# MartijnAB/guacamole

Measured on AMD Instinct MI355X. Metric: pileup loci/sec at 30x WGS; achieved HBM GB/s vs roofline, higher is better.
Workload: dtype u8; 1 GPU; germline-threshold, synthetic 30x chr20-length shard per GPU (configs[1]); genome_loci=63025519, visited_loci_per_gpu=63025483, reads_per_gpu=12612887, contigs_per_gpu=1, read_len=150, threshold=8, parallelism=loci-sharded x1

## Files before the change

guacamole_amd/csrc/gq_germline_common.h:

```cpp
#pragma once

#include "gq_kernels.h"


__device__ __forceinline__ int64_t xcd_tile(int64_t b, int64_t n) {
  const int64_t q = n >> 3, rem = n & 7;
  const int64_t x = b & 7, j = b >> 3;
  return x * q + (x < rem ? x : rem) + j;
}

struct LdsOut {
  unsigned *lds;
  unsigned long long base[2], cap[2];
  __device__ __forceinline__ unsigned long long reserve(int which, unsigned n) {
    return wave_reserve_lds(lds + which, n);
  }
};
struct GlobalOut {
  Counters *ctr;
  int part;
  unsigned long long base[2], cap[2];
  __device__ __forceinline__ unsigned long long reserve(int which, unsigned n) {
    return wave_reserve(&ctr->part[which][part], n);
  }
};

template <int T, bool ZERO = false, class Out>
__device__ __forceinline__ void germline_decide(const uint32_t *cnt, const Tile &tl, int64_t tile_id, bool wide,
                                                int n_samples, int threshold, int emit_ref, int emit_no_call,
                                                CallRec *__restrict__ recs, ComplexItem *__restrict__ cplx,
                                                Out &out, unsigned &visited, unsigned &amb, unsigned &ties,
                                                const uint32_t *reg = nullptr) {
  constexpr int S = T + 2 * kGuard;
  const int32_t L0 = tl.L0;
  const bool multi_sample = n_samples > 1;
  const int nloci = tl.L1 - L0;
  const int64_t thr1 = (int64_t)threshold + 1;
  const bool narrow = thr1 >= 0 && thr1 <= 1001;
  const uint32_t thr1u = (uint32_t)thr1;
  auto passes = [=](uint32_t count, uint32_t depth) {
    return narrow ? count * 100u >= thr1u * depth : (int64_t)count * 100 >= thr1 * (int64_t)depth;
  };
  constexpr uint64_t kAltSym = ((uint64_t)'<' << 8) | ((uint64_t)'A' << 16) | ((uint64_t)'L' << 24) |
                               ((uint64_t)'T' << 32) | ((uint64_t)'>' << 40);
  for (int i0 = 0; i0 < nloci; i0 += blockDim.x) {
    const int i = i0 + threadIdx.x;
    const bool in = i < nloci;
    uint32_t wac = 0, wtg = 0, wox = 0, wnn = 0, eac = 0, etg = 0;
    if (in) {
      wac = cnt[W_AC * S + kGuard + i];
      wtg = cnt[W_TG * S + kGuard + i];
      wox = cnt[W_OX * S + kGuard + i];
      wnn = cnt[W_NN * S + kGuard + i];
      eac = cnt[W_EAC * S + kGuard + i];
      etg = cnt[W_ETG * S + kGuard + i];
    }
    if (ZERO && i < T) {
      uint32_t *z = const_cast<uint32_t *>(cnt) + kGuard + i;
#pragma unroll
      for (int w = 0; w < W_N; ++w) z[w * S] = 0u;
    }
    uint32_t c[5] = {wac & 0xFFFFu, wac >> 16, wtg & 0xFFFFu, wtg >> 16, wnn >> 16};
    if (reg) {
#pragma unroll
      for (int k = 0; k < 5; ++k) c[k] += in ? reg[k] : 0u;
    }
    const uint32_t cx = (wox & 0xFFFFu) + (wox >> 16);
    const uint32_t depth = c[0] + c[1] + c[2] + c[3] + c[4] + cx;
    const uint32_t mask = (wnn & 0xFu) | (c[0] > (eac & 0xFFFFu) ? 1u : 0u) | (c[1] > (eac >> 16) ? 2u : 0u) |
                          (c[2] > (etg & 0xFFFFu) ? 4u : 0u) | (c[3] > (etg >> 16) ? 8u : 0u);
    const bool live = in && depth > 0;
    const bool ambiguous = (mask & (mask - 1)) != 0;
    const uint32_t low = mask & (0u - mask);
    const uint32_t c_ref = low == 1u ? c[0] : low == 2u ? c[1] : low == 4u ? c[2] : low == 8u ? c[3] : c[4];
    const bool cgn = low == 2u && c[3] > 0 && c[4] > 0;
    const bool to_complex = (wide && in) || (live && (ambiguous || cx > 0 || multi_sample || cgn));
    const bool homref = live && !to_complex && !passes(depth - c_ref, depth);
    const bool ref_pass = c_ref > 0 && passes(c_ref, depth);
    const bool emit_hr = homref && (ref_pass ? emit_ref : emit_no_call);
    const bool general = live && !to_complex && !homref;
    visited += (live && !(wide && in)) ? 1u : 0u;
    amb += (live && ambiguous && !wide) ? 1u : 0u;
    if (__ballot(to_complex || emit_hr || general) == 0) continue;
    CallRec out0, out1;
    unsigned nout = 0;
    const uint8_t ref = mask ? bit_base(mask) : (uint8_t)'N';
    const int32_t pos = L0 + i;
    const uint64_t ord = (uint64_t)(tl.ordinal0 + i);
    auto push = [&](const CallRec &rr) {
      if (nout == 0) out0 = rr;
      else out1 = rr;
      ++nout;
    };
    if (emit_hr) {
      CallRec rr;
      rr.key = ord << 12;
      rr.contig = tl.contig;
      rr.pos = pos;
      rr.sample = 0;
      rr.gt0 = rr.gt1 = ref_pass ? GQ_GT_REF : GQ_GT_NOCALL;
      rr.flags = 0;
      rr.ref_len = 1;
      rr.alt_len = 5;
      rr.allele = (uint64_t)ref | kAltSym;
      push(rr);
    }
    if (general) {
      CallRec rr;
      rr.key = ord << 12;
      rr.contig = tl.contig;
      rr.pos = pos;
      rr.sample = 0;
      rr.gt0 = ref;
      rr.gt1 = 0;
      rr.flags = kCandidate;
      rr.ref_len = (uint16_t)c[4];
      rr.alt_len = 0;
      rr.allele = (uint64_t)c[0] | ((uint64_t)c[1] << 16) | ((uint64_t)c[2] << 32) | ((uint64_t)c[3] << 48);
      push(rr);
      rr.flags = kCandidateSlot;
      push(rr);
    }
    const unsigned long long base = out.reserve(0, nout);
    CallRec *prec = recs + out.base[0];
    if (nout > 0 && base < out.cap[0]) prec[base] = out0;
    if (nout > 1 && base + 1 < out.cap[0]) prec[base + 1] = out1;
    const unsigned long long cb = out.reserve(1, to_complex ? 1u : 0u);
    if (to_complex && cb < out.cap[1])
      cplx[out.base[1] + cb] = ComplexItem{(int32_t)tile_id, L0 + i, wide ? 1 : 0};
  }
}

__global__ void germline_expand(CallRec *__restrict__ recs, Counters *ctr, OutGeom og, int threshold,
                                int emit_ref, int emit_no_call, uint64_t dead_key) {
  const unsigned long long n = ctr->n_rec;
  const int64_t thr1 = (int64_t)threshold + 1;
  auto passes = [=](uint32_t count, uint32_t depth) { return (int64_t)count * 100 >= thr1 * (int64_t)depth; };
  constexpr uint64_t kAltSym = ((uint64_t)'<' << 8) | ((uint64_t)'A' << 16) | ((uint64_t)'L' << 24) |
                               ((uint64_t)'T' << 32) | ((uint64_t)'>' << 40);
  unsigned dead = 0, ties = 0;
  (void)n;
  for (int p = blockIdx.x; p < kParts; p += gridDim.x) {
   const unsigned long long cnt = ctr->part_off[0][p + 1] - ctr->part_off[0][p];
   for (unsigned long long k = threadIdx.x; k < cnt; k += blockDim.x) {
    const unsigned long long slot = og.slot(0, p, k);
    const CallRec cand = recs[slot];
    if (cand.flags != kCandidate) continue;
    constexpr int NC = 6;
    const uint32_t c[NC] = {(uint32_t)(cand.allele & 0xFFFFu), (uint32_t)((cand.allele >> 16) & 0xFFFFu),
                            (uint32_t)((cand.allele >> 32) & 0xFFFFu), (uint32_t)(cand.allele >> 48), cand.ref_len,
                            cand.alt_len};
    const uint32_t depth = c[0] + c[1] + c[2] + c[3] + c[4] + c[5];
    const uint8_t ref = cand.gt0;
    int npres = 0;
#pragma unroll
    for (int cat = 0; cat < NC; ++cat) npres += c[cat] > 0 ? 1 : 0;
    uint64_t sk[NC];
#pragma unroll
    for (int cat = 0; cat < NC; ++cat) {
      scala::SeqHasher hr, ha;
      hr.add_byte(ref);
      if (cat < 5) ha.add_byte(cat_base(cat));
      const uint32_t h = scala::allele_hash(hr.result(), ha.result());
      sk[cat] = npres <= 4 ? (uint64_t)(15u - scala::mutable_bucket(h, 4)) : scala::trie_key(h);
    }
    uint32_t k0 = 0, k1 = 0, k2 = 0;
    int npass = 0;
#pragma unroll
    for (int cat = 0; cat < NC; ++cat) {
      const uint32_t cc = c[cat];
      if (cc == 0 || !passes(cc, depth)) continue;
      ++npass;
      int rank = 0;
#pragma unroll
      for (int o = 0; o < NC; ++o)
        if (o != cat && c[o] > 0 && (sk[o] < sk[cat] || (sk[o] == sk[cat] && o < cat))) ++rank;
      uint32_t key = (cc << 16) | ((uint32_t)(255 - rank) << 8) | (uint32_t)cat;
      if (key > k0) { const uint32_t t = k0; k0 = key; key = t; }
      if (key > k1) { const uint32_t t = k1; k1 = key; key = t; }
      if (key > k2) { k2 = key; }
    }
    const bool tie = npass >= 2 && ((k0 >> 16) == (k1 >> 16) || (npass >= 3 && (k1 >> 16) == (k2 >> 16)));
    if (tie) ++ties;
    const uint8_t fl = tie ? GQ_FLAG_TIE : 0;
    const int t0 = (int)(k0 & 0xFFu), t1 = (int)(k1 & 0xFFu);
    auto is_var = [&](int cat) { return cat == 5 || cat_base(cat) != ref; };
    int nout = 0, aa = 0, ab = 0;
    uint8_t ga0 = 0, ga1 = 0, gb0 = 0, gb1 = 0;
    bool syma = false;
    if (npass == 0) {
      if (emit_no_call) nout = 1, ga0 = ga1 = GQ_GT_NOCALL, syma = true;
    } else if (npass == 1 && !is_var(t0)) {
      if (emit_ref) nout = 1, ga0 = ga1 = GQ_GT_REF, syma = true;
    } else if (npass == 1) {
      nout = 1, ga0 = ga1 = GQ_GT_ALT, aa = t0;
    } else {
      const bool v1 = is_var(t0), v2 = is_var(t1);
      if ((!v1 || !v2) && ((t0 == 5) != (t1 == 5))) {
      } else if (v1 != v2) {
        nout = 1, ga0 = GQ_GT_REF, ga1 = GQ_GT_ALT, aa = v1 ? t0 : t1;
      } else if (v1 && v2) {
        nout = 2, ga0 = gb0 = GQ_GT_ALT, ga1 = gb1 = GQ_GT_OTHERALT, aa = t0, ab = t1;
      }
    }
    auto put = [&](unsigned long long at, bool live, int sub, uint8_t g0, uint8_t g1, int cat, bool sym) {
      const uint64_t key = live ? (cand.key | (uint64_t)sub) : dead_key;
      const uint32_t alt_len = sym ? 5u : cat == 5 ? 0u : 1u;
      const uint64_t allele = sym ? ((uint64_t)ref | kAltSym)
                                  : ((uint64_t)ref | (cat == 5 ? 0ull : (uint64_t)cat_base(cat) << 8));
      const uint32_t w3 = (uint32_t)cand.sample | ((uint32_t)g0 << 8) | ((uint32_t)g1 << 16) |
                          ((uint32_t)(live ? fl : 0) << 24);
      const uint32_t w4 = 1u | (alt_len << 16);
      uint4 *d = reinterpret_cast<uint4 *>(recs + at);
      d[0] = make_uint4((uint32_t)key, (uint32_t)(key >> 32), (uint32_t)cand.contig, (uint32_t)cand.pos);
      d[1] = make_uint4(w3, w4, (uint32_t)allele, (uint32_t)(allele >> 32));
    };
    put(slot, nout > 0, 0, ga0, ga1, aa, syma);
    put(slot + 1, nout > 1, 1, gb0, gb1, ab, false);
    dead += nout > 1 ? 0u : nout > 0 ? 1u : 2u;
   }
  }
  for (int d = 32; d >= 1; d >>= 1) {
    dead += __shfl_xor(dead, d, 64);
    ties += __shfl_xor(ties, d, 64);
  }
  if ((threadIdx.x & 63) == 0) {
    const int sl = (int)((blockIdx.x * (blockDim.x >> 6) + (threadIdx.x >> 6)) & (kSpread - 1));
    if (dead) atomicAdd(&ctr->spread[3][sl], (unsigned long long)dead);
    if (ties) atomicAdd(&ctr->spread[2][sl], (unsigned long long)ties);
  }
}

__device__ __forceinline__ void add_run_counters(Counters *ctr, unsigned visited, unsigned amb, unsigned ties,
                                                 int slot) {
  __shared__ unsigned red[3];
  if (threadIdx.x < 3) red[threadIdx.x] = 0;
  __syncthreads();
  if (visited) atomicAdd(&red[0], visited);
  if (amb) atomicAdd(&red[1], amb);
  if (ties) atomicAdd(&red[2], ties);
  __syncthreads();
  if (threadIdx.x == 0) {
    const int sl = slot & (kSpread - 1);
    if (red[0]) atomicAdd(&ctr->spread[0][sl], (unsigned long long)red[0]);
    if (red[1]) atomicAdd(&ctr->spread[1][sl], (unsigned long long)red[1]);
    if (red[2]) atomicAdd(&ctr->spread[2][sl], (unsigned long long)red[2]);
  }
}

template <int T>
__global__ __launch_bounds__(kBlock) __attribute__((amdgpu_waves_per_eu(4))) void germline_walk(const Tile *__restrict__ tiles, const int32_t *__restrict__ slow,
                                                        DevReads R, int threshold, int emit_ref, int emit_no_call,
                                                        CallRec *__restrict__ recs, ComplexItem *__restrict__ cplx,
                                                        OutGeom og,
                                                        Counters *ctr) {
  constexpr int S = T + 2 * kGuard;
  __shared__ __attribute__((aligned(16))) uint32_t cnt[W_N * S];
  const int64_t n = (int64_t)ctr->n_slow;
  const int part = kPartsCols + (int)((blockIdx.x * (blockDim.x >> 6) + (threadIdx.x >> 6)) & (kPartsWalk - 1));
  GlobalOut out{ctr, part, {og.slot(0, part, 0), og.slot(1, part, 0)}, {og.capB[0], og.capB[1]}};
  unsigned visited = 0, amb = 0, ties = 0;
  for (int64_t q = blockIdx.x; q < n; q += gridDim.x) {
    const int64_t tid_tile = slow[q];
    const Tile tl = tiles[tid_tile];
    const bool wide = (tl.re - tl.rb) >= 65535;
    uint4 *c4 = reinterpret_cast<uint4 *>(cnt);
    for (int i = threadIdx.x; i < W_N * S / 4; i += blockDim.x) c4[i] = make_uint4(0u, 0u, 0u, 0u);
    __syncthreads();
    if (!wide) {
      GermSink<T, 0> sink{cnt, tl.L0, &ctr->err, &ctr->err_pos};
      for (int64_t r = tl.rb + threadIdx.x; r < tl.re; r += blockDim.x) walk_read_lane(R, r, tl.L0, tl.L1, sink);
    }
    __syncthreads();
    germline_decide<T>(cnt, tl, tid_tile, wide, R.n_samples, threshold, emit_ref, emit_no_call, recs, cplx, out,
                       visited, amb, ties);
    __syncthreads();
  }
  add_run_counters(ctr, visited, amb, ties, (int)blockIdx.x);
}
```

guacamole_amd/csrc/gq_host.h:

```cpp
#pragma once
#include <hip/hip_runtime.h>

#include <algorithm>
#include <cstddef>
#include <cstring>
#include <condition_variable>
#include <mutex>
#include <thread>
#include <cstdarg>
#include <cstdio>
#include <string>
#include <utility>
#include <vector>

#include "../../include/gqpileup.h"
#include "gq_kernels.h"

namespace gq {

gq_status set_err(gq_status s, const char *fmt, ...);

#define HIP_TRY(expr)                                                                         \
  do {                                                                                        \
    hipError_t _e = (expr);                                                                   \
// ... 688 lines not shown
    if (len && !keep(m)) len = 0;
    {
      const int64_t q0 = m.qoff + (pr.col0 >> 4);
      const int32_t npc = len ? ((pr.col1 - 1) >> 4) - (pr.col0 >> 4) + 1 : 0;
      int64_t g[kReadPieces];
      piece_grows(R, rr, q0, npc < kReadPieces ? npc : kReadPieces, g);
#pragma unroll
      for (int j = 0; j < kReadPieces; ++j) m.grow[j] = g[j];
    }
    if (len) meta[lane] = m;
    const uint32_t incl = wave_incl_scan(len), ex = incl - len;
    const uint32_t tot = (uint32_t)__builtin_amdgcn_readlane((int)incl, 63);
    for (uint32_t w0 = 0; w0 < tot; w0 += 64) {
      owner[lane] = 0;
      __builtin_amdgcn_wave_barrier();
      __builtin_amdgcn_fence(__ATOMIC_SEQ_CST, "wavefront");
      if (len > 0 && ex > w0 && ex < w0 + 64) owner[ex - w0] = (uint32_t)lane + 1;
      __builtin_amdgcn_wave_barrier();
      __builtin_amdgcn_fence(__ATOMIC_SEQ_CST, "wavefront");
      const uint32_t w = w0 + (uint32_t)lane;
      const unsigned long long run = __ballot(len > 0 && ex <= w0);
      const uint32_t k_at = run ? 64u - (uint32_t)__clzll((long long)run) : 0u;
      const uint32_t k1 = max(wave_incl_max(owner[lane]), k_at);
      const bool au = w < tot;
      const int k = au ? (int)k1 - 1 : 0;
      const uint4 *rec = reinterpret_cast<const uint4 *>(meta + k);
      const uint4 a = rec[0], bq = rec[1], c = rec[2], dq = rec[3], eq = rec[4];
      ReadMeta mm;
      mm.p0 = (int64_t)((uint64_t)a.x | ((uint64_t)a.y << 32));
      mm.s = (int32_t)a.z;
      mm.e = (int32_t)a.w;
      mm.info = bq.x;
      mm.mq = bq.y;
      mm.col0 = (int32_t)bq.z;
      mm.evin = bq.w;
      mm.ev01 = eq.z;
      mm.ev23 = eq.w;
      mm.md_off = (int64_t)((uint64_t)c.x | ((uint64_t)c.y << 32));
      mm.qoff = (int64_t)((uint64_t)c.z | ((uint64_t)c.w << 32));
      const int64_t g0 = (int64_t)((uint64_t)dq.x | ((uint64_t)dq.y << 32));
      const int64_t g1 = (int64_t)((uint64_t)dq.z | ((uint64_t)dq.w << 32));
      const int64_t g2 = (int64_t)((uint64_t)eq.x | ((uint64_t)eq.y << 32));
      const uint32_t kex = (uint32_t)__shfl((int)ex, k, 64);
      const int32_t col = mm.col0 + (int32_t)(w - kex);
      const int32_t col1 = (mm.e + 7) >> 3;
      bool act = au && col < col1;
      const int32_t pj = (col >> 4) - (mm.col0 >> 4);
      const int64_t slot = mm.qoff + (col >> 4);
      int64_t grow = pj == 0 ? g0 : pj == 1 ? g1 : pj == 2 ? g2 : -2;
      if (act && grow == -2) grow = piece_grow(R, 64 * b + k, slot);
      act = act && grow >= 0;
      const int64_t pa = mm.p0 + 8 * (int64_t)col;
      const bool fast = src != nullptr && act && (mm.info & kColEligible) && pa >= 0 && pa + 8 <= R.seq_cap;
      const uint64_t pre = src != nullptr && R.seq_cap >= 8 && !(dbg & 1)
                               ? *reinterpret_cast<const gq_u64u *>(src + (fast ? pa : 0))
                               : 0ull;
      decltype(fetch((int64_t)0, mm, (int32_t)0, 0ull, false)) raw{};
      if (act && !(dbg & 1)) raw = fetch(64 * b + k, mm, col, pre, fast);
      emit(act && !(dbg & 2), raw, 64 * b + k, mm, col, grow, slot);
    }
    __builtin_amdgcn_wave_barrier();
    __builtin_amdgcn_fence(__ATOMIC_SEQ_CST, "wavefront");
  }
}

__device__ __forceinline__ unsigned wave_reserve_lds(unsigned *ctr, unsigned n) {
  const uint64_t b1 = __ballot(n & 1u), b2 = __ballot(n & 2u);
  if ((b1 | b2) == 0) return 0;
  const uint64_t lt = __builtin_amdgcn_read_exec() & ((1ull << (threadIdx.x & 63)) - 1ull);
  const unsigned pre = (unsigned)__popcll(b1 & lt) + 2u * (unsigned)__popcll(b2 & lt);
  const unsigned total = (unsigned)__popcll(b1) + 2u * (unsigned)__popcll(b2);
  unsigned base = 0;
  if (lt == 0) base = atomicAdd(ctr, total);
  base = (unsigned)__builtin_amdgcn_readfirstlane((int)base);
  return base + pre;
}

struct Plan {
  int64_t n_tiles = 0;
  int64_t n_loci = 0;
  int T = 0;
  bool aligned = false;
  std::vector<int32_t> rc, rwin;
  std::vector<int64_t> rs, re, rt, rtask;
  struct Win {
    int32_t contig;
    int64_t r0, r1;
  };
  std::vector<Win> wins;
  const int64_t *d_rs = nullptr, *d_re = nullptr, *d_wroff = nullptr;
  const int32_t *d_rwin = nullptr, *d_wcontig = nullptr;
  int64_t range_of_tile(int64_t t) const {
    return (int64_t)(std::upper_bound(rt.begin(), rt.end(), t) - rt.begin()) - 1;
  }
  int64_t tiles_of(int64_t r) const {
    const int64_t s = rs[(size_t)r], e = re[(size_t)r];
    return aligned ? (e - 1) / T - s / T + 1 : (e - s + T - 1) / T;
  }
};

struct AmbItem {
  int32_t tile, pos;
  int64_t item;
};

}

namespace gq {
struct DevBuf {
  void *p = nullptr;
  size_t n = 0;
  hipError_t ensure(size_t bytes) {
    if (bytes <= n) return hipSuccess;
    if (p) (void)hipFree(p);
    p = nullptr;
    n = 0;
    size_t want = std::max(bytes, (size_t)256);
    hipError_t e = hipMalloc(&p, want);
    if (e == hipSuccess) n = want;
    return e;
  }
  void release() {
    if (p) (void)hipFree(p);
    p = nullptr;
    n = 0;
  }
};
}

struct gq_ctx {
  int device = 0;
  hipStream_t stream = nullptr;
  hipEvent_t ev[6] = {};
  hipEvent_t dev_ev[4] = {};
  hipStream_t side = nullptr;
  hipEvent_t side_ev[4] = {};
  gq_timings timings{};
  int germ_tile = gq::kGermT;
  int n_cu = 0;
  int proj_wg_per_cu = 0;
  int dir_wg_per_cu = 0;
  int som_wg_per_cu = 0;
  int somd_wg_per_cu = 0;
  gq::DevBuf mtab;
  int mtab_key = -1;
  int call_wg_per_cu = 0;
  gq::DevBuf ranges, tiles, recs, recs_sorted, keys, keys_sorted, idx, idx_sorted, cplx, pool, counters, sort_tmp, image, tiles2, srecs;
  gq::DevBuf c_depth, c_pos, c_base, c_indel, c_ref, c_rb, c_amb, slow, deep_tiles;
  gq::DevBuf amb, amb_ref, heap_off, heap_reads;
  gq::DevBuf win_meta, win_grp;
  gq::DevBuf deep_list, deep_scratch;
  gq::DevBuf cands;
  gq::DevBuf win_bound;
  gq::DevBuf bkt;
  void *stage[2] = {nullptr, nullptr};
  hipEvent_t stage_done[2] = {};
  bool stage_used[2] = {false, false};
  std::mutex stage_m;
  std::condition_variable stage_cv;
  bool stage_ready = false;
  hipError_t stage_err = hipSuccess;
  std::thread prep;
  hipError_t wait_stage() {
    std::unique_lock<std::mutex> lk(stage_m);
    stage_cv.wait(lk, [this] { return stage_ready; });
    return stage_err;
  }
  void *pin = nullptr;
  size_t pin_n = 0;
  hipError_t pinned(size_t bytes) {
    if (bytes <= pin_n) return hipSuccess;
    if (pin) (void)hipHostFree(pin);
    pin = nullptr;
    pin_n = 0;
    const size_t want = std::max(bytes, (size_t)65536);
    hipError_t e = hipHostMalloc(&pin, want, hipHostMallocDefault);
    if (e == hipSuccess) pin_n = want;
    return e;
  }
};

struct DerivedPool {
  std::vector<std::pair<void *, size_t>> live, spare;
  hipError_t get(void **p, size_t bytes) {
    bytes = std::max(bytes, (size_t)16);
    size_t best = spare.size();
    for (size_t i = 0; i < spare.size(); ++i)
      if (spare[i].second >= bytes && spare[i].second <= bytes + bytes / 4 + 65536 &&
          (best == spare.size() || spare[i].second < spare[best].second))
        best = i;
    if (best < spare.size()) {
      *p = spare[best].first;
      live.push_back(spare[best]);
      spare.erase(spare.begin() + (long)best);
      return hipSuccess;
    }
    *p = nullptr;
    const hipError_t e = hipMalloc(p, bytes);
    if (e == hipSuccess) live.emplace_back(*p, bytes);
    return e;
  }
  void put(void *p) {
    for (size_t i = 0; i < live.size(); ++i)
      if (live[i].first == p) {
        spare.push_back(live[i]);
        live.erase(live.begin() + (long)i);
        return;
      }
  }
  void release_all() {
    spare.insert(spare.end(), live.begin(), live.end());
    live.clear();
  }
  void free_all() {
    for (auto &x : live) (void)hipFree(x.first);
    for (auto &x : spare) (void)hipFree(x.first);
    live.clear();
    spare.clear();
  }
};

struct gq_dev_reads {
  gq_ctx *ctx = nullptr;
  gq::DevReads d{};
  std::vector<int64_t> contig_read_begin;
  std::vector<void *> owned;
  mutable DerivedPool dp;
  int64_t seq_bytes = 0;
  int64_t proj_bytes = 0, pev_count = 0, proj_reads = 0;
  int64_t n_slices = 0;
  int64_t n_rows = 0;
  float h2d_ms = 0, derive_ms = 0;
  bool columns = false;
  bool ev_bases = false;
  bool projected = false;
  void *nnb = nullptr;
  float proj_ms = 0;
  float fill_ms = 0;
  float proj_dev_ms = 0;
  float derive_dev_ms = 0;
  hipEvent_t tev[6] = {};
  unsigned pending = 0;
  unsigned long long *nok = nullptr;
  mutable void *mproj = nullptr;
  mutable int mproj_mapq = -1;
  mutable void *mnb = nullptr;
};

namespace gq {
struct H2DStager {
  static constexpr size_t kChunk = size_t(64) << 20;
  gq_ctx *c;
  hipStream_t stream;
  void **buf = nullptr;
  hipEvent_t *done = nullptr;
  bool *used = nullptr;
  int slot = 0;
  unsigned threads = 1;
  explicit H2DStager(gq_ctx *ctx) : c(ctx), stream(ctx->stream) {
    const unsigned hw = std::max(1u, std::thread::hardware_concurrency());
    threads = std::min(16u, hw);
  }
  ~H2DStager() {
    for (int i = 0; done && i < 2; ++i)
      if (used[i]) (void)hipEventSynchronize(done[i]);
  }
  hipError_t init() {
    const hipError_t e = c->wait_stage();
    if (e != hipSuccess) return e;
    buf = c->stage;
    done = c->stage_done;
    used = c->stage_used;
    return hipSuccess;
  }
  template <class F>
  void fill(uint8_t *out, size_t o, size_t k, const F &src_range) const {
    const unsigned t = (unsigned)std::min<size_t>(threads, std::max<size_t>(1, k >> 22));
    if (t <= 1) {
      src_range(out, o, k);
      return;
    }
    std::vector<std::thread> th;
    const size_t per = (k + t - 1) / t;
    for (unsigned i = 0; i < t; ++i) {
      const size_t a = (size_t)i * per;
      if (a >= k) break;
      th.emplace_back([&, a] { src_range(out + a, o + a, std::min(per, k - a)); });
    }
    for (auto &x : th) x.join();
  }
  template <class F, class G>
  hipError_t copy_from(void *dst, size_t bytes, const F &src_range, const G &landed) {
    for (size_t o = 0; o < bytes; o += kChunk) {
      const size_t k = std::min(kChunk, bytes - o);
      if (used[slot]) {
        hipError_t e = hipEventSynchronize(done[slot]);
        if (e != hipSuccess) return e;
      }
      fill((uint8_t *)buf[slot], o, k, src_range);
      hipError_t e = hipMemcpyAsync((char *)dst + o, buf[slot], k, hipMemcpyHostToDevice, stream);
      if (e == hipSuccess) e = hipEventRecord(done[slot], stream);
      if (e != hipSuccess) return e;
      used[slot] = true;
      slot ^= 1;
      e = landed(o + k);
      if (e != hipSuccess) return e;
    }
    return hipSuccess;
  }
  template <class F>
  hipError_t copy_from(void *dst, size_t bytes, const F &src_range) {
    return copy_from(dst, bytes, src_range, [](size_t) { return hipSuccess; });
  }
  hipError_t copy(void *dst, const void *src, size_t bytes) {
    return copy_from(dst, bytes, [src](uint8_t *out, size_t o, size_t k) { memcpy(out, (const uint8_t *)src + o, k); });
  }
};

gq_status derive_shape(gq_ctx *c, gq_dev_reads *d, int64_t md_len);
gq_status ensure_columns(gq_ctx *c, const gq_dev_reads *d);
gq_status ensure_ev_bases(gq_ctx *c, const gq_dev_reads *d);
gq_status ensure_projection(gq_ctx *c, const gq_dev_reads *d);
hipError_t warm_pileup(hipStream_t s);
hipError_t warm_somatic(hipStream_t s);
hipError_t warm_heapref(hipStream_t s);
hipError_t warm_bamdev(hipStream_t s);

gq_status plan(gq_ctx *c, const gq_dev_reads *rd, const gq_loci *loci, int T, Plan &pl, DevBuf &tiles,
               int stage_cap = 0, int meta_cap = 0, int ev_cap = 0, bool aligned = false);
gq_status check_device_error(gq_ctx *c, const Counters &h);
gq_status heap_ref_bases(gq_ctx *c, const Plan &pl, const DevBuf &tiles_buf,
                         const std::vector<const gq_dev_reads *> &sets, const std::vector<AmbItem> &items,
                         uint8_t *out_ref);

gq_status reads_overlap(gq_ctx *c, const gq_dev_reads *set, int32_t contig,
                        const std::vector<std::pair<int64_t, int64_t>> &ranges, std::vector<char> &out);
}
```

guacamole_amd/csrc/gq_pileup.hip:

```cpp
#include <hip/hip_runtime.h>
#include <hipcub/hipcub.hpp>

#include <algorithm>
#include <chrono>
#include <cstdarg>
#include <cstdlib>
#include <cstdio>
#include <cstring>
#include <string>
#include <thread>
#include <vector>

#include "../../include/gqpileup.h"
#include "gq_host.h"
#include "gq_alleles.h"

using namespace gq;

namespace {
constexpr int kScanT = 256, kScanV = 16, kScanTile = kScanT * kScanV;

__device__ __forceinline__ void scan_load16(const uint32_t *__restrict__ in, int64_t n, int64_t i0, uint32_t (&v)[kScanV]) {
  if (i0 + kScanV <= n) {
    const uint4 *p = reinterpret_cast<const uint4 *>(in + i0);
// ... 1309 lines not shown
      if (((valid4 >> j) & 1u) && i + j >= 0 && i + j < T) elem_i(i + j, K_SNV, (uint8_t)(w >> (8 * j)), 0, false, fl);
  }
  __device__ __forceinline__ void event_i(int i, uint8_t b, uint8_t m, uint8_t) {
    const int bc = base_cat(b);
    if (bc < 4) atomicAdd(&cnt[(K2_EVA + bc) * T + i], 1u);
    const uint32_t bit = std_bit(m);
    if (bit) atomicOr(&cnt[K2_MASK * T + i], bit);
  }
  __device__ __forceinline__ void elem_i(int i, int kind, uint8_t base, uint8_t mdb, bool ev, uint8_t fl) {
    int c;
    switch (kind) {
      case K_SNV: c = base_cat(base); break;
      case K_INS: c = K2_INS; break;
      case K_DEL: c = K2_DEL; break;
      case K_MID: c = K2_MID; break;
      default: c = K2_CLIP; break;
    }
    atomicAdd(&cnt[c * T + i], 1u);
    if (!(fl & 1)) atomicAdd(&cnt[K2_POS * T + i], 1u);
    const uint32_t b = std_bit(mdb);
    if (kind == K_SNV && !ev) return;
    if (kind == K_SNV && ev) {
      const int bc = base_cat(base);
      if (bc < 4) atomicAdd(&cnt[(K2_EVA + bc) * T + i], 1u);
    }
    if (b) atomicOr(&cnt[K2_MASK * T + i], b);
  }
  __device__ __forceinline__ void clip_run(int i0, int i1, uint8_t fl) {
    for (int i = i0; i < i1; ++i) elem_i(i, K_CLIP, 0, (uint8_t)'N', false, fl);
  }
  __device__ __forceinline__ void error(int code, int64_t where) { raise_error(err, (int64_t *)err_pos, code, where); }
};

template <int T>
__global__ __launch_bounds__(kBlock) void counts_tile(const Tile *__restrict__ tiles, DevReads R,
                                                      int32_t *__restrict__ depth, int32_t *__restrict__ pos_depth,
                                                      int32_t *__restrict__ base_counts,
                                                      int32_t *__restrict__ indel_counts,
                                                      int32_t *__restrict__ ref_depth, uint8_t *__restrict__ ref_base,
                                                      uint8_t *__restrict__ ambiguous, Counters *ctr) {
  __shared__ uint32_t cnt[K2_NCAT * T];
  const Tile tl = tiles[blockIdx.x];
  const int32_t L0 = tl.L0, L1 = tl.L1;
  for (int i = threadIdx.x; i < K2_NCAT * T; i += blockDim.x) cnt[i] = 0u;
  __syncthreads();
  CountSink<T> sink{cnt, L0, &ctr->err, &ctr->err_pos};
  for (int64_t r = tl.rb + threadIdx.x; r < tl.re; r += blockDim.x) walk_read_lane(R, r, L0, L1, sink);
  __syncthreads();
  for (int i = threadIdx.x; i < L1 - L0; i += blockDim.x) {
    const int64_t o = tl.ordinal0 + i;
    uint32_t dsum = 0;
    for (int k = 0; k <= K2_CLIP; ++k) dsum += cnt[k * T + i];
    uint32_t mask = cnt[K2_MASK * T + i];
    for (int k = 0; k < 4; ++k)
      if (cnt[k * T + i] > cnt[(K2_EVA + k) * T + i]) mask |= 1u << k;
    const uint8_t rb = mask ? bit_base(mask) : (uint8_t)'N';
    depth[o] = (int32_t)dsum;
    pos_depth[o] = (int32_t)cnt[K2_POS * T + i];
    const int out_order[6] = {K2_A, K2_C, K2_G, K2_T, K2_N, K2_O};
    for (int k = 0; k < 6; ++k) base_counts[o * 6 + k] = (int32_t)cnt[out_order[k] * T + i];
    for (int k = 0; k < 4; ++k) indel_counts[o * 4 + k] = (int32_t)cnt[(K2_INS + k) * T + i];
    ref_depth[o] = (int32_t)cnt[base_cat(rb) * T + i];
    ref_base[o] = rb;
    ambiguous[o] = __popc(mask) > 1 ? 1 : 0;
  }
}

struct VafAmb {
  int32_t depth, base[6];
};
template <int T>
__global__ __launch_bounds__(kBlock) void vaf_tile(const Tile *__restrict__ tiles, DevReads R, int bins,
                                                   int min_depth, int min_vaf, unsigned long long *__restrict__ hist,
                                                   AmbItem *__restrict__ amb, VafAmb *__restrict__ amb_cnt,
                                                   unsigned long long amb_cap, Counters *ctr) {
  __shared__ uint32_t cnt[K2_NCAT * T];
  __shared__ uint32_t h[101];
  const Tile tl = tiles[blockIdx.x];
  const int32_t L0 = tl.L0, L1 = tl.L1;
  for (int i = threadIdx.x; i < K2_NCAT * T; i += blockDim.x) cnt[i] = 0u;
  for (int i = threadIdx.x; i < 101; i += blockDim.x) h[i] = 0u;
  __syncthreads();
  CountSink<T> sink{cnt, L0, &ctr->err, &ctr->err_pos};
  for (int64_t r = tl.rb + threadIdx.x; r < tl.re; r += blockDim.x) walk_read_lane(R, r, L0, L1, sink);
  __syncthreads();
  const int bin_size = 100 / bins;
  unsigned visited = 0, variant = 0;
  for (int i = threadIdx.x; i < L1 - L0; i += blockDim.x) {
    uint32_t dsum = 0;
    for (int k = 0; k <= K2_CLIP; ++k) dsum += cnt[k * T + i];
    if (dsum == 0) continue;
    ++visited;
    uint32_t mask = cnt[K2_MASK * T + i];
    for (int k = 0; k < 4; ++k)
      if (cnt[k * T + i] > cnt[(K2_EVA + k) * T + i]) mask |= 1u << k;
    if (__popc(mask) > 1) {
      const unsigned long long k = atomicAdd(&ctr->n_amb, 1ull);
      if (k < amb_cap) {
        amb[k] = AmbItem{(int32_t)blockIdx.x, L0 + i, (int64_t)k};
        VafAmb v;
        v.depth = (int32_t)dsum;
        const int out_order[6] = {K2_A, K2_C, K2_G, K2_T, K2_N, K2_O};
        for (int q = 0; q < 6; ++q) v.base[q] = (int32_t)cnt[out_order[q] * T + i];
        amb_cnt[k] = v;
      }
      continue;
    }
    const uint8_t rb = mask ? bit_base(mask) : (uint8_t)'N';
    const uint32_t ref = cnt[base_cat(rb) * T + i];
    if (ref == dsum) continue;
    const float vaf = (float)(int32_t)(dsum - ref) / (float)(int32_t)dsum;
    if (!((int32_t)dsum >= min_depth) || !((double)vaf >= (double)min_vaf / 100.0)) continue;
    ++variant;
    const int pct = (int)(vaf * 100.0f);
    atomicAdd(&h[pct - pct % bin_size], 1u);
  }
  __syncthreads();
  unsigned long long *hh = hist + (size_t)(blockIdx.x & 63) * 101;
  for (int i = threadIdx.x; i < 101; i += blockDim.x)
    if (h[i]) atomicAdd(&hh[i], (unsigned long long)h[i]);
  for (int d = 32; d >= 1; d >>= 1) {
    visited += __shfl_xor(visited, d, 64);
    variant += __shfl_xor(variant, d, 64);
  }
  if ((threadIdx.x & 63) == 0) {
    if (visited) atomicAdd(&ctr->spread[0][blockIdx.x & (kSpread - 1)], (unsigned long long)visited);
    if (variant) atomicAdd(&ctr->spread[1][blockIdx.x & (kSpread - 1)], (unsigned long long)variant);
  }
}

struct CallsLayout {
  size_t contig, pos, ref_off, alt_off, ref_len, alt_len, sample, gt0, gt1, flags, pool, bytes;
};
__host__ __device__ inline CallsLayout calls_layout(int64_t n, int64_t dev_pool_used) {
  auto al = [](size_t x) { return (x + 63) & ~(size_t)63; };
  const size_t N = (size_t)n;
  CallsLayout L;
  L.contig = 64;
  L.pos = al(L.contig + 4 * N);
  L.ref_off = al(L.pos + 8 * N);
  L.alt_off = al(L.ref_off + 8 * N);
  L.ref_len = al(L.alt_off + 8 * N);
  L.alt_len = al(L.ref_len + 4 * N);
  L.sample = al(L.alt_len + 4 * N);
  L.gt0 = al(L.sample + N);
  L.gt1 = al(L.gt0 + N);
  L.flags = al(L.gt1 + N);
  L.pool = al(L.flags + N);
  L.bytes = al(L.pool + 8 * N + (size_t)dev_pool_used + 1);
  return L;
}

__global__ __launch_bounds__(1024) void part_scan(Counters *ctr, int which, OutGeom og) {
  constexpr int PER = kParts / 1024;
  __shared__ unsigned long long s[1024];
  __shared__ unsigned long long mx;
  const int t = threadIdx.x;
  unsigned long long v[PER], sum = 0, m = 0;
#pragma unroll
  for (int j = 0; j < PER; ++j) {
    const unsigned long long x = ctr->part[which][t * PER + j];
    const unsigned long long cap = og.cap(which, t * PER + j);
    m = x > cap && x - cap > m ? x - cap : m;
    v[j] = x < cap ? x : cap;
    sum += v[j];
  }
  if (t == 0) mx = 0;
  s[t] = sum;
  __syncthreads();
  if (m) atomicMax(&mx, m);
  for (int d = 1; d < 1024; d <<= 1) {
    const unsigned long long y = t >= d ? s[t - d] : 0ull;
    __syncthreads();
    s[t] += y;
    __syncthreads();
  }
  unsigned long long o = s[t] - sum;
#pragma unroll
  for (int j = 0; j < PER; ++j) {
    ctr->part_off[which][t * PER + j] = o;
    o += v[j];
  }
  if (t == 1023) {
    ctr->part_off[which][kParts] = s[t];
    if (which == 0) ctr->n_rec = s[t];
    else ctr->n_complex = s[t];
    ctr->part_max[which] = mx;
  }
}

__global__ void gather_keys(const CallRec *__restrict__ recs, const Counters *__restrict__ ctr, OutGeom og,
                            int64_t n, uint64_t *__restrict__ keys,
                            int32_t *__restrict__ slot) {
  const int64_t k = (int64_t)blockIdx.x * blockDim.x + threadIdx.x;
  if (k >= n) return;
  const unsigned long long src = part_slot(ctr->part_off[0], (unsigned long long)k, og, 0);
  keys[k] = recs[src].key;
  slot[k] = (int32_t)src;
}

constexpr int kFinBlocks = 1024;
constexpr int kImgBlocks = 512;
__global__ __launch_bounds__(kBlock) void bucket_count(const CallRec *__restrict__ recs, Counters *__restrict__ ctr,
                                                        OutGeom og, uint64_t dead_key, int bshift, int64_t nbk,
                                                        uint64_t *__restrict__ keys, int32_t *__restrict__ slot,
                                                        int64_t *__restrict__ bkt, uint32_t *__restrict__ cnt) {
  const int64_t n_all = (int64_t)ctr->n_rec;
  for (int64_t k = (int64_t)blockIdx.x * blockDim.x + threadIdx.x; k < n_all; k += (int64_t)gridDim.x * blockDim.x) {
    const unsigned long long src = part_slot(ctr->part_off[0], (unsigned long long)k, og, 0);
    const uint64_t key = recs[src].key;
    keys[k] = key;
    slot[k] = (int32_t)src;
    int64_t b = key == dead_key ? -1 : (int64_t)(key >> (12 + bshift));
    if (b >= nbk) {
      if (atomicCAS(&ctr->err, 0, 1 ) == 0) {
        const CallRec r = recs[src];
        ctr->err_pos = (long long)src;
        ctr->prof[0] = key;
        ctr->prof[1] = ((unsigned long long)(uint32_t)r.contig << 32) | (uint32_t)r.pos;
        ctr->prof[2] = ((unsigned long long)r.flags << 24) | ((unsigned long long)r.gt1 << 16) | ((unsigned long long)r.gt0 << 8) | r.sample;
        ctr->prof[3] = (unsigned long long)k;
        ctr->prof[4] = ctr->n_rec;
      }
      b = -1;
    }
    bkt[k] = b;
    if (b >= 0) atomicAdd(&cnt[b], 1u);
  }
}

__global__ void bucket_scatter(const Counters *__restrict__ ctr, const int64_t *__restrict__ bkt,
                               const uint32_t *__restrict__ off, uint32_t *__restrict__ fill,
                               int32_t *__restrict__ members) {
  const int64_t n_all = (int64_t)ctr->n_rec;
  for (int64_t k = (int64_t)blockIdx.x * blockDim.x + threadIdx.x; k < n_all; k += (int64_t)gridDim.x * blockDim.x) {
    const int64_t b = bkt[k];
    if (b >= 0) members[off[b] + atomicAdd(&fill[b], 1u)] = (int32_t)k;
  }
}

__global__ void bucket_rank(int64_t nbk, const uint32_t *__restrict__ off, const int32_t *__restrict__ members,
                            const uint64_t *__restrict__ keys, const int32_t *__restrict__ slot,
                            const int64_t *__restrict__ bkt, int32_t *__restrict__ order) {
  const int64_t n = off[nbk];
  for (int64_t p = (int64_t)blockIdx.x * blockDim.x + threadIdx.x; p < n; p += (int64_t)gridDim.x * blockDim.x) {
    const int32_t k = members[p];
    const int64_t b = bkt[k];
    const uint32_t lo = off[b], hi = off[b + 1];
    const uint64_t key = keys[k];
    uint32_t rank = 0;
    for (uint32_t q = lo; q < hi; ++q) rank += keys[members[q]] < key ? 1u : 0u;
    order[lo + rank] = slot[k];
  }
}

__global__ void zero_u32(uint32_t *__restrict__ v, int64_t n) {
  for (int64_t i = (int64_t)blockIdx.x * blockDim.x + threadIdx.x; i < n; i += (int64_t)gridDim.x * blockDim.x) v[i] = 0u;
}

__global__ void iota_i32(int32_t *__restrict__ v, int64_t n) {
  const int64_t i = (int64_t)blockIdx.x * blockDim.x + threadIdx.x;
  if (i < n) v[i] = (int32_t)i;
}

__device__ __forceinline__ void img_chunk(int64_t n, int64_t &a, int64_t &b) {
  const int64_t per = (n + kImgBlocks - 1) / kImgBlocks;
  a = min(n, (int64_t)blockIdx.x * per);
  b = min(n, a + per);
}
__device__ __forceinline__ uint32_t rec_len(const CallRec &r) { return (uint32_t)r.ref_len + (uint32_t)r.alt_len; }

__global__ __launch_bounds__(kBlock) void img_sums(const CallRec *__restrict__ recs, const int32_t *__restrict__ order,
                                                    const uint32_t *__restrict__ off, int64_t nbk,
                                                    int64_t *__restrict__ bsum) {
  __shared__ unsigned long long red;
  if (threadIdx.x == 0) red = 0;
  __syncthreads();
  int64_t a, b;
  img_chunk((int64_t)off[nbk], a, b);
  unsigned long long s = 0;
  for (int64_t k = a + threadIdx.x; k < b; k += blockDim.x) s += rec_len(recs[order[k]]);
  for (int d = 32; d >= 1; d >>= 1) s += __shfl_xor(s, d, 64);
  if ((threadIdx.x & 63) == 0 && s) atomicAdd(&red, s);
  __syncthreads();
  if (threadIdx.x == 0) bsum[blockIdx.x] = (int64_t)red;
}

__global__ __launch_bounds__(kImgBlocks) void img_scan(int64_t *__restrict__ bsum) {
  __shared__ int64_t s[kImgBlocks];
  const int t = threadIdx.x;
  const int64_t v = bsum[t];
  s[t] = v;
  __syncthreads();
  for (int d = 1; d < kImgBlocks; d <<= 1) {
    const int64_t y = t >= d ? s[t - d] : 0;
    __syncthreads();
    s[t] += y;
    __syncthreads();
  }
  bsum[t] = s[t] - v;
  if (t == kImgBlocks - 1) bsum[kImgBlocks] = s[t];
}

__global__ __launch_bounds__(kBlock) void calls_image(const CallRec *__restrict__ recs, const int32_t *__restrict__ order,
                                                       const uint32_t *__restrict__ off, int64_t nbk,
                                                       const int64_t *__restrict__ bsum, const uint8_t *__restrict__ dpool,
                                                       Counters *__restrict__ ctr, uint8_t *__restrict__ img) {
  __shared__ uint32_t wsum[kBlock / 64];
  const int64_t n = (int64_t)off[nbk];
  const CallsLayout L = calls_layout(n, 0);
  int64_t a, b;
  img_chunk(n, a, b);
  int64_t prefix = bsum[blockIdx.x];
  const int lane = threadIdx.x & 63, wv = threadIdx.x >> 6;
  for (int64_t base = a; base < b; base += blockDim.x) {
    const int64_t k = base + threadIdx.x;
    CallRec r{};
    if (k < b) r = recs[order[k]];
    const uint32_t tot = k < b ? rec_len(r) : 0u;
    const uint32_t inc = wave_incl_scan(tot);
    if (lane == 63) wsum[wv] = inc;
    __syncthreads();
    uint32_t before = 0, all = 0;
#pragma unroll
    for (int w = 0; w < kBlock / 64; ++w) {
      before += w < wv ? wsum[w] : 0u;
      all += wsum[w];
    }
    __syncthreads();
    if (k < b) {
      const int64_t o = prefix + before + inc - tot;
      reinterpret_cast<int32_t *>(img + L.contig)[k] = r.contig;
      reinterpret_cast<int64_t *>(img + L.pos)[k] = r.pos;
      reinterpret_cast<int64_t *>(img + L.ref_off)[k] = o;
      reinterpret_cast<int64_t *>(img + L.alt_off)[k] = o + r.ref_len;
      reinterpret_cast<int32_t *>(img + L.ref_len)[k] = r.ref_len;
      reinterpret_cast<int32_t *>(img + L.alt_len)[k] = r.alt_len;
      img[L.sample + k] = r.sample;
      img[L.gt0 + k] = r.gt0;
      img[L.gt1 + k] = r.gt1;
      img[L.flags + k] = r.flags;
      uint8_t *dst = img + L.pool + o;
      if (tot <= 8) {
        for (uint32_t i = 0; i < tot; ++i) dst[i] = (uint8_t)(r.allele >> (8 * i));
      } else {
        for (uint32_t i = 0; i < tot; ++i) dst[i] = dpool[r.allele + i];
      }
    }
    prefix += all;
  }
  if (blockIdx.x == 0 && threadIdx.x == 0) {
    const int64_t pool_len = bsum[kImgBlocks];
    reinterpret_cast<int64_t *>(img)[0] = pool_len;
    reinterpret_cast<int64_t *>(img)[1] = n;
    ctr->n_out = (unsigned long long)n;
    ctr->out_pool = (unsigned long long)pool_len;
  }
}

}

namespace {
__global__ void warm_k() {}
}
hipError_t gq::warm_pileup(hipStream_t s) {
  hipLaunchKernelGGL(warm_k, dim3(1), dim3(64), 0, s);
  return hipGetLastError();
}

extern "C" {

const char *gq_version(void) { return "guacamole-amd gqpileup 0.1 (gfx950)"; }
const char *gq_last_error(void) { return g_err.c_str(); }

gq_status gq_open(int device, gq_ctx **out) {
  if (!out) return set_err(GQ_E_ARG, "gq_open: null out");
  int n = 0;
  HIP_TRY(hipGetDeviceCount(&n));
  if (device < 0 || device >= n) return set_err(GQ_E_ARG, "gq_open: device %d out of range (%d devices)", device, n);
  HIP_TRY(hipSetDevice(device));
  gq_ctx *c = new gq_ctx();
  c->device = device;
  HIP_TRY(hipStreamCreateWithFlags(&c->stream, hipStreamNonBlocking));
  HIP_TRY(hipStreamCreateWithFlags(&c->side, hipStreamNonBlocking));
  for (auto &e : c->ev) HIP_TRY(hipEventCreate(&e));
  for (auto &e : c->dev_ev) HIP_TRY(hipEventCreate(&e));
  for (auto &e : c->side_ev) HIP_TRY(hipEventCreateWithFlags(&e, hipEventDisableTiming));
  c->prep = std::thread([c] {
    hipError_t e = hipSetDevice(c->device);
    for (int i = 0; i < 2 && e == hipSuccess; ++i) {
      e = hipHostMalloc(&c->stage[i], H2DStager::kChunk, hipHostMallocDefault);
      if (e == hipSuccess) e = hipEventCreateWithFlags(&c->stage_done[i], hipEventDisableTiming);
    }
    {
      std::lock_guard<std::mutex> lk(c->stage_m);
      c->stage_err = e;
      c->stage_ready = true;
    }
    c->stage_cv.notify_all();
    if (e == hipSuccess) e = gq::warm_pileup(c->stream);
    if (e == hipSuccess) e = gq::warm_somatic(c->stream);
    if (e == hipSuccess) e = gq::warm_heapref(c->stream);
    if (e == hipSuccess) e = gq::warm_bamdev(c->stream);
    (void)e;
  });
  *out = c;
  return GQ_OK;
}


void gq_close(gq_ctx *c) {
  if (!c) return;
  if (c->prep.joinable()) c->prep.join();
  (void)hipSetDevice(c->device);
  (void)hipStreamSynchronize(c->stream);
  for (int i = 0; i < 2; ++i) {
    if (c->stage_done[i]) (void)hipEventDestroy(c->stage_done[i]);
    if (c->stage[i]) (void)hipHostFree(c->stage[i]);
  }
  for (DevBuf *b : {&c->ranges, &c->tiles, &c->recs, &c->recs_sorted, &c->keys, &c->keys_sorted, &c->idx,
                    &c->idx_sorted, &c->cplx, &c->pool, &c->counters, &c->sort_tmp, &c->image, &c->tiles2, &c->srecs, &c->c_depth, &c->c_pos,
                    &c->c_base, &c->c_indel, &c->c_ref, &c->c_rb, &c->c_amb, &c->slow, &c->amb, &c->amb_ref,
                    &c->heap_off, &c->heap_reads, &c->win_meta, &c->win_grp, &c->bkt})
    b->release();
  for (auto &e : c->ev) (void)hipEventDestroy(e);
  for (auto &e : c->dev_ev) (void)hipEventDestroy(e);
  for (auto &e : c->side_ev) (void)hipEventDestroy(e);
  if (c->side) {
    (void)hipStreamSynchronize(c->side);
    (void)hipStreamDestroy(c->side);
  }
  if (c->pin) (void)hipHostFree(c->pin);
  (void)hipStreamDestroy(c->stream);
  delete c;
}

gq_status gq_get_timings(const gq_ctx *c, gq_timings *out) {
  if (!c || !out) return set_err(GQ_E_ARG, "gq_get_timings: null argument");
  *out = c->timings;
  return GQ_OK;
}

gq_status gq_set_tile(gq_ctx *c, int32_t t) {
  if (!c) return set_err(GQ_E_ARG, "null ctx");
  if (t == 0) t = kGermT;
  if (t != 512) return set_err(GQ_E_ARG, "tile must be 512 (the germline column kernel's geometry)");
  c->germ_tile = t;
  return GQ_OK;
}

static gq_status validate_reads(const gq_reads *h) {
  if (!h) return set_err(GQ_E_ARG, "null read set");
  if (h->n_reads < 0 || h->n_contigs <= 0) return set_err(GQ_E_ARG, "bad read-set sizes");
  if (h->n_samples < 1 || h->n_samples > 8) return set_err(GQ_E_ARG, "n_samples must be in [1, 8]");
  return GQ_OK;
}

static gq_status settle_stats(gq_dev_reads *d) {
  if (d->pending & 1) {
    HIP_TRY(hipEventSynchronize(d->tev[1]));
    (void)hipEventElapsedTime(&d->derive_dev_ms, d->tev[0], d->tev[1]);
  }
  if (d->pending & 2) {
    HIP_TRY(hipEventSynchronize(d->tev[5]));
    (void)hipEventElapsedTime(&d->fill_ms, d->tev[3], d->tev[4]);
    (void)hipEventElapsedTime(&d->proj_dev_ms, d->tev[2], d->tev[5]);
    std::vector<unsigned long long> hk(kOkSpread);
    HIP_TRY(hipMemcpy(hk.data(), d->nok, sizeof(unsigned long long) * kOkSpread, hipMemcpyDeviceToHost));
    d->proj_reads = 0;
    for (unsigned long long x : hk) d->proj_reads += (int64_t)x;
    d->dp.put(d->nok);
    d->nok = nullptr;
  }
  d->pending = 0;
  return GQ_OK;
}

static gq_status derive_shape_impl(gq_ctx *c, gq_dev_reads *d, int64_t md_len, bool lazy = false) {
  for (hipEvent_t &e : d->tev)
    if (!e) HIP_TRY(hipEventCreate(&e));
  HIP_TRY(hipEventRecord(d->tev[0], c->stream));
  {
    const auto &b = d->contig_read_begin;
    bool ok = !b.empty() && b.front() == 0 && b.back() == d->d.n_reads;
    for (size_t i = 1; i < b.size() && ok; ++i) ok = b[i] >= b[i - 1];
    if (!ok) return set_err(GQ_E_UNSORTED, "contig_read_begin must run from 0 to n_reads, non-decreasing");
  }
  void *p = nullptr;
  HIP_TRY(d->dp.get(&p, sizeof(int16_t) * (size_t)std::max<int64_t>(d->d.n_reads, 1)));
  d->d.lead = (const int16_t *)p;
  d->d.ev_rb = nullptr;
  d->ev_bases = false;
  int unordered = 0;
  const int nc = d->d.n_contigs;
  std::vector<int32_t> last((size_t)nc, 0);
  if (d->d.n_reads > 0) {
    void *flag = nullptr;
    HIP_TRY(d->dp.get(&flag, sizeof(int)));
    HIP_TRY(hipMemsetAsync(flag, 0, sizeof(int), c->stream));
    const unsigned nb = (unsigned)((d->d.n_reads + kBlock - 1) / kBlock);
    hipLaunchKernelGGL(read_prep, dim3(nb), dim3(kBlock), 0, c->stream, d->d, (int *)flag, (int16_t *)p);
    HIP_TRY(hipGetLastError());
    int bad = 0;
    HIP_TRY(hipMemcpyAsync(&bad, flag, sizeof(int), hipMemcpyDeviceToHost, c->stream));
    const auto &crb = d->contig_read_begin;
    for (int k = 0; k < nc; ++k)
      if (crb[(size_t)k + 1] > crb[(size_t)k])
        HIP_TRY(hipMemcpyAsync(&last[(size_t)k], d->d.pmax_end + (crb[(size_t)k + 1] - 1), sizeof(int32_t),
                               hipMemcpyDeviceToHost, c->stream));
    HIP_TRY(hipStreamSynchronize(c->stream));
    if (bad & 1)
      return set_err(GQ_E_UNSORTED, "Regions must be sorted by start locus: reads are not sorted by (contig, start), "
                                    "or pmax_end is not the running maximum of end within each contig");
    if (bad & 2)
      return set_err(GQ_E_ARG, "read set: an offset or length lies outside its pool, or a sample slot >= n_samples");
    unordered = (bad & 4) ? 1 : 0;
  }
  {
    std::vector<int64_t> qoff((size_t)nc + 1, 0);
    for (int k = 0; k < nc; ++k) {
      const int64_t col1 = ((int64_t)std::max(last[(size_t)k], 0) + 7) >> 3;
      qoff[(size_t)k + 1] = qoff[(size_t)k] + 4 * ((col1 + 63) >> 6);
    }
    void *qo = nullptr;
    HIP_TRY(d->dp.get(&qo, sizeof(int64_t) * ((size_t)nc + 1)));
    HIP_TRY(hipMemcpyAsync(qo, qoff.data(), sizeof(int64_t) * ((size_t)nc + 1), hipMemcpyHostToDevice, c->stream));
    d->d.qoff = (const int64_t *)qo;
    d->n_slices = qoff[(size_t)nc];
    const int64_t n_blk = qoff[(size_t)nc] / 4;
    void *bi = nullptr;
    HIP_TRY(d->dp.get(&bi, sizeof(int64_t) * 2 * (size_t)std::max<int64_t>(n_blk, 1)));
    int64_t *brb = (int64_t *)bi, *brs = brb + std::max<int64_t>(n_blk, 1);
    if (n_blk > 0) {
      hipLaunchKernelGGL(block_index, dim3((unsigned)((n_blk + kBlock - 1) / kBlock)), dim3(kBlock), 0, c->stream, d->d,
                         n_blk, brb, brs);
      HIP_TRY(hipGetLastError());
    }
    d->d.blk_rb = brb;
    d->d.blk_rs = brs;
  }
  HIP_TRY(hipEventRecord(d->tev[1], c->stream));
  d->d.pool_ordered = unordered ? 0 : 1;
  if (lazy) {
    d->pending |= 1;
    return GQ_OK;
  }
  HIP_TRY(hipStreamSynchronize(c->stream));
  (void)hipEventElapsedTime(&d->derive_dev_ms, d->tev[0], d->tev[1]);
  return GQ_OK;
}


gq_status gq_reads_upload(gq_ctx *c, const gq_reads *h, gq_dev_reads **out) {
  if (!c || !out) return set_err(GQ_E_ARG, "gq_reads_upload: null argument");
  gq_status st = validate_reads(h);
  if (st) return st;
  HIP_TRY(hipSetDevice(c->device));
  gq_dev_reads *d = new gq_dev_reads();
  d->ctx = c;
  const int64_t n = h->n_reads;
  const auto t0 = std::chrono::steady_clock::now();
  H2DStager stager(c);
  {
    hipError_t e = stager.init();
    if (e != hipSuccess) {
      delete d;
      return set_err(GQ_E_HIP, "upload: pinned staging: %s", hipGetErrorString(e));
    }
  }
  auto up_from = [&](size_t bytes, void **dst, size_t pad, const auto &src_range) -> hipError_t {
    *dst = nullptr;
    hipError_t e = hipMalloc(dst, std::max(bytes + pad, (size_t)16));
    if (e != hipSuccess) return e;
    d->owned.push_back(*dst);
    if (bytes) e = stager.copy_from(*dst, bytes, src_range);
    if (e == hipSuccess && pad) e = hipMemsetAsync((char *)*dst + bytes, 0, pad, c->stream);
    return e;
  };
  auto up = [&](const void *src, size_t bytes, void **dst, size_t pad) -> hipError_t {
    if (bytes >= (size_t(1) << 20) || (!src && bytes))
      return up_from(bytes, dst, pad, [src](uint8_t *out, size_t o, size_t k) {
        if (src) memcpy(out, (const uint8_t *)src + o, k);
        else memset(out, 0, k);
      });
    *dst = nullptr;
    hipError_t e = hipMalloc(dst, std::max(bytes + pad, (size_t)16));
    if (e != hipSuccess) return e;
    d->owned.push_back(*dst);
    if (bytes) e = hipMemcpyAsync(*dst, src, bytes, hipMemcpyHostToDevice, c->stream);
    if (e == hipSuccess && pad) e = hipMemsetAsync((char *)*dst + bytes, 0, pad, c->stream);
    return e;
  };
  void *p;
#define UP_CHECK(field, T, expr)                                                \
  do {                                                                          \
    hipError_t _e = (expr);                                                     \
    if (_e != hipSuccess) {                                                     \
      gq_reads_free(d);                                                         \
      return set_err(GQ_E_HIP, "upload %s: %s", #field, hipGetErrorString(_e)); \
    }                                                                           \
    d->d.field = (const T *)p;                                                  \
  } while (0)
#define UP(field, count, T) UP_CHECK(field, T, up(h->field, (size_t)(count) * sizeof(T), &p, pad_##field))
  enum : size_t { pad_contig_read_begin = 0, pad_start = 0, pad_end = 0, pad_pmax_end = 0, pad_mapq = 0, pad_flags = 0,
                  pad_sample = 0, pad_seq_off = 0, pad_seq_len = 0, pad_cigar_off = 0, pad_n_cigar = 0, pad_md_off = 0,
                  pad_n_md = 0, pad_n_mismatch = 0, pad_seq = kSeqPad, pad_qual = kSeqPad, pad_cigar = 0,
                  pad_md_ev = 0 };
  const gq_reads *h0 = h;
  gq_reads hh = *h;
  std::vector<int64_t> off2;
  bool ordered = true;
  for (int64_t r = 1; r < n && ordered; ++r) ordered = h->seq_off[r] >= h->seq_off[r - 1] + h->seq_len[r - 1];
  if (!ordered) {
    off2.resize((size_t)n);
    int64_t o = 0;
    for (int64_t r = 0; r < n; ++r) {
      off2[(size_t)r] = o;
      o += h->seq_len[r];
    }
    hh.seq_off = off2.data();
    hh.seq_bytes = o;
  }
  auto gather = [&](const uint8_t *src) {
    return [&, src](uint8_t *out, size_t o, size_t k) {
      if (!src) {
        memset(out, 0, k);
        return;
      }
      int64_t r = (int64_t)(std::upper_bound(off2.begin(), off2.end(), (int64_t)o) - off2.begin()) - 1;
      size_t done = 0;
      while (done < k) {
        const size_t a = o + done - (size_t)off2[(size_t)r];
        const size_t m = std::min((size_t)h0->seq_len[r] - a, k - done);
        memcpy(out + done, src + h0->seq_off[r] + a, m);
        done += m;
        ++r;
      }
    };
  };
  h = &hh;
  UP(contig_read_begin, h->n_contigs + 1, int64_t);
  UP(start, n, int32_t);
  UP(end, n, int32_t);
  UP(pmax_end, n, int32_t);
  UP(mapq, n, uint8_t);
  UP(flags, n, uint8_t);
  UP(sample, n, uint8_t);
  UP(seq_off, n, int64_t);
  UP(seq_len, n, int32_t);
  UP(cigar_off, n, int64_t);
  UP(n_cigar, n, int32_t);
  UP(md_off, n, int64_t);
  UP(n_md, n, int32_t);
  UP(n_mismatch, n, uint16_t);
  if (ordered) {
    UP(seq, h->seq_bytes, uint8_t);
    UP(qual, h->seq_bytes, uint8_t);
  } else {
    UP_CHECK(seq, uint8_t, up_from((size_t)h->seq_bytes, &p, pad_seq, gather(h0->seq)));
    UP_CHECK(qual, uint8_t, up_from((size_t)h->seq_bytes, &p, pad_qual, gather(h0->qual)));
  }
  UP(cigar, h->cigar_len, uint32_t);
  UP(md_ev, h->md_len, uint32_t);
#undef UP
#undef UP_CHECK
  d->d.n_reads = n;
  d->d.seq_bytes = h->seq_bytes;
  d->d.seq_cap = h->seq_bytes + kSeqPad;
  d->d.cigar_len = h->cigar_len;
  d->d.md_len = h->md_len;
  d->d.n_contigs = h->n_contigs;
  d->d.n_samples = h->n_samples;
  if (h->sample_hash && h->n_samples > 0) {
    void *sh = nullptr;
    if (hipMalloc(&sh, sizeof(uint32_t) * (size_t)h->n_samples) != hipSuccess ||
        hipMemcpy(sh, h->sample_hash, sizeof(uint32_t) * (size_t)h->n_samples, hipMemcpyHostToDevice) != hipSuccess) {
      if (sh) (void)hipFree(sh);
      gq_reads_free(d);
      return set_err(GQ_E_HIP, "gq_reads_upload: sample hashes");
    }
    d->owned.push_back(sh);
    d->d.sample_hash = (const uint32_t *)sh;
  }
  d->contig_read_begin.assign(h->contig_read_begin, h->contig_read_begin + h->n_contigs + 1);
  d->seq_bytes = h->seq_bytes;
  if (hipStreamSynchronize(c->stream) != hipSuccess) {
    gq_reads_free(d);
    return set_err(GQ_E_HIP, "gq_reads_upload: copies");
  }
  const auto t1 = std::chrono::steady_clock::now();
  d->h2d_ms = std::chrono::duration<float, std::milli>(t1 - t0).count();
  gq_status st2 = derive_shape_impl(c, d, h->md_len);
  d->derive_ms = std::chrono::duration<float, std::milli>(std::chrono::steady_clock::now() - t1).count();
  if (st2) {
    gq_reads_free(d);
    return st2;
  }
  *out = d;
  return GQ_OK;
}

gq_status gq_reads_wrap_device(gq_ctx *c, const gq_reads *h, gq_dev_reads **out) {
  if (!c || !out) return set_err(GQ_E_ARG, "gq_reads_wrap_device: null argument");
  gq_status st = validate_reads(h);
  if (st) return st;
  gq_dev_reads *d = new gq_dev_reads();
  d->ctx = c;
  d->d.n_reads = h->n_reads;
  d->d.seq_bytes = h->seq_bytes;
  d->d.seq_cap = h->seq_bytes;
  d->d.cigar_len = h->cigar_len;
  d->d.md_len = h->md_len;
  d->d.n_contigs = h->n_contigs;
  d->d.n_samples = h->n_samples;
  d->d.contig_read_begin = h->contig_read_begin;
  d->d.start = h->start;
  d->d.end = h->end;
  d->d.pmax_end = h->pmax_end;
  d->d.mapq = h->mapq;
  d->d.flags = h->flags;
  d->d.sample = h->sample;
  d->d.seq_off = h->seq_off;
  d->d.seq_len = h->seq_len;
  d->d.cigar_off = h->cigar_off;
  d->d.n_cigar = h->n_cigar;
  d->d.md_off = h->md_off;
  d->d.n_md = h->n_md;
  d->d.n_mismatch = h->n_mismatch;
  d->d.seq = h->seq;
  d->d.qual = h->qual;
  d->d.cigar = h->cigar;
  d->d.md_ev = h->md_ev;
  d->d.sample_hash = h->sample_hash;
  d->contig_read_begin.resize((size_t)h->n_contigs + 1);
  hipError_t e = hipMemcpy(d->contig_read_begin.data(), h->contig_read_begin,
                           sizeof(int64_t) * ((size_t)h->n_contigs + 1), hipMemcpyDeviceToHost);
  if (e != hipSuccess) {
    delete d;
    return set_err(GQ_E_HIP, "wrap: contig_read_begin D2H: %s", hipGetErrorString(e));
  }
  d->seq_bytes = h->seq_bytes;
  const auto t1 = std::chrono::steady_clock::now();
  gq_status st2 = derive_shape_impl(c, d, h->md_len);
  d->derive_ms = std::chrono::duration<float, std::milli>(std::chrono::steady_clock::now() - t1).count();
  if (st2) {
    gq_reads_free(d);
    return st2;
  }
  *out = d;
  return GQ_OK;
}

gq_status gq_reads_rederive(gq_ctx *c, gq_dev_reads *d) {
  if (!c || !d) return set_err(GQ_E_ARG, "gq_reads_rederive: null argument");
  if (d->ctx != c) return set_err(GQ_E_ARG, "gq_reads_rederive: the read set belongs to another context");
  HIP_TRY(hipSetDevice(c->device));
  HIP_TRY(hipStreamSynchronize(c->stream));
  HIP_TRY(hipStreamSynchronize(c->side));
  d->nok = nullptr;
  d->pending = 0;
  d->dp.release_all();
  DevReads &R = d->d;
  R.lead = nullptr;
  R.ev_rb = R.clean = nullptr;
  R.pool_ordered = 0;
  R.cdesc = nullptr;
  R.cev = nullptr;
  R.caux_off = R.qoff = R.srow = R.pev_off = R.sra = R.soff = R.blk_rb = R.blk_rs = nullptr;
  R.prec = nullptr;
  R.proj = R.pbad = nullptr;
  R.pev = nullptr;
  R.prow = nullptr;
  d->projected = false;
  d->columns = false;
  d->ev_bases = false;
  d->nnb = d->mproj = d->mnb = nullptr;
  d->mproj_mapq = -1;
  d->proj_bytes = d->pev_count = d->proj_reads = d->n_rows = d->n_slices = 0;
  d->proj_ms = d->fill_ms = d->proj_dev_ms = 0;
  const auto t1 = std::chrono::steady_clock::now();
  const gq_status st = derive_shape_impl(c, d, R.md_len, true);
  d->derive_ms = std::chrono::duration<float, std::milli>(std::chrono::steady_clock::now() - t1).count();
  return st;
}

gq_status gq_reads_get_info(const gq_dev_reads *dc, gq_reads_info *out) {
  if (!dc || !out) return set_err(GQ_E_ARG, "gq_reads_get_info: null argument");
  gq_dev_reads *d = const_cast<gq_dev_reads *>(dc);
  if (d->pending) {
    HIP_TRY(hipSetDevice(d->ctx->device));
    const gq_status s0 = settle_stats(d);
    if (s0) return s0;
  }
  out->n_reads = d->d.n_reads;
  out->seq_bytes = d->seq_bytes;
  out->proj_bytes = d->proj_bytes;
  out->pev_count = d->pev_count;
  out->n_rows = d->n_rows;
  out->proj_reads = d->proj_reads;
  out->h2d_ms = d->h2d_ms;
  out->derive_ms = d->derive_ms;
  out->cigar_len = d->d.cigar_len;
  out->md_len = d->d.md_len;
  out->n_contigs = d->d.n_contigs;
  out->n_samples = d->d.n_samples;
  out->proj_ms = d->proj_ms;
  out->projected = d->projected ? 1 : 0;
  out->fill_ms = d->fill_ms;
  out->proj_dev_ms = d->proj_dev_ms;
  out->derive_dev_ms = d->derive_dev_ms;
  return GQ_OK;
}

void gq_reads_free(gq_dev_reads *d) {
  if (!d) return;
  if (d->ctx) (void)hipSetDevice(d->ctx->device);
  for (hipEvent_t e : d->tev)
    if (e) {
      (void)hipEventSynchronize(e);
      (void)hipEventDestroy(e);
    }
  for (void *p : d->owned) (void)hipFree(p);
  d->dp.free_all();
  delete d;
}

}

static int gq_dbg() {
  static const int d = getenv("GQ_DBG") ? atoi(getenv("GQ_DBG")) : 0;
  return d;
}

gq_status gq::plan(gq_ctx *c, const gq_dev_reads *rd, const gq_loci *loci, int T, Plan &pl, DevBuf &tiles_buf,
                   int stage_cap, int meta_cap, int ev_cap, bool aligned) {
  if (!loci || loci->n_ranges < 0) return set_err(GQ_E_ARG, "bad loci");
  const int64_t R = loci->n_ranges;
  pl = Plan{};
  pl.T = T;
  pl.aligned = aligned;
  std::vector<int32_t> &rc = pl.rc;
  std::vector<int64_t> &rs = pl.rs, &re = pl.re, &rt = pl.rt, ro;
  int64_t ord = 0, tiles = 0;
  for (int64_t i = 0; i < R; ++i) {
    const int32_t cc = loci->contig[i];
    const int64_t s = loci->start[i], e = loci->end[i];
    if (cc < 0 || cc >= rd->d.n_contigs) return set_err(GQ_E_ARG, "loci range %lld: contig %d out of range", (long long)i, cc);
    if (s < 0 || e < s || e > INT32_MAX) return set_err(GQ_E_ARG, "loci range %lld: bad interval", (long long)i);
    if (e == s) continue;
    const int64_t task = loci->task ? loci->task[i] : 0;
    if (pl.wins.empty() || pl.rtask.back() != task || rc.back() != cc) {
      pl.wins.push_back(Plan::Win{cc, (int64_t)rc.size(), (int64_t)rc.size()});
    } else if (s < re.back()) {
      return set_err(GQ_E_ARG, "loci range %lld: ranges of one task and contig must be sorted and disjoint",
                     (long long)i);
    }
    pl.wins.back().r1 = (int64_t)rc.size() + 1;
    pl.rwin.push_back((int32_t)(pl.wins.size() - 1));
    pl.rtask.push_back(task);
    rc.push_back(cc);
    rs.push_back(s);
    re.push_back(e);
    ro.push_back(ord);
    rt.push_back(tiles);
    ord += e - s;
    tiles += aligned ? (e - 1) / T - s / T + 1 : (e - s + T - 1) / T;
  }
  pl.n_tiles = tiles;
  pl.n_loci = ord;
  if (tiles == 0) return GQ_OK;
  const size_t nr = rc.size(), nw = pl.wins.size();
  const size_t o_rs = (nr * 4 + 15) & ~(size_t)15, o_wroff = o_rs + 4 * 8 * nr, o_rwin = o_wroff + 8 * (nw + 1),
               o_wc = o_rwin + ((4 * nr + 15) & ~(size_t)15), bytes = o_wc + 4 * nw;
  HIP_TRY(c->ranges.ensure(bytes + 64));
  char *base = (char *)c->ranges.p;
  int32_t *d_rc = (int32_t *)base;
  int64_t *d_rs = (int64_t *)(base + o_rs);
  int64_t *d_re = d_rs + nr, *d_ro = d_re + nr, *d_rt = d_ro + nr;
  {
    HIP_TRY(c->pinned(bytes));
    char *hb = (char *)c->pin;
    memcpy(hb, rc.data(), nr * 4);
    memcpy(hb + o_rs, rs.data(), nr * 8);
    memcpy(hb + o_rs + 8 * nr, re.data(), nr * 8);
    memcpy(hb + o_rs + 16 * nr, ro.data(), nr * 8);
    memcpy(hb + o_rs + 24 * nr, rt.data(), nr * 8);
    int64_t *wroff = (int64_t *)(hb + o_wroff);
    int32_t *wc = (int32_t *)(hb + o_wc);
    for (size_t w = 0; w < nw; ++w) {
      wroff[w] = pl.wins[w].r0;
      wc[w] = pl.wins[w].contig;
    }
    wroff[nw] = (int64_t)nr;
    memcpy(hb + o_rwin, pl.rwin.data(), nr * 4);
    HIP_TRY(hipMemcpyAsync(base, hb, bytes, hipMemcpyHostToDevice, c->stream));
  }
  pl.d_rs = d_rs;
  pl.d_re = d_re;
  pl.d_wroff = (const int64_t *)(base + o_wroff);
  pl.d_rwin = (const int32_t *)(base + o_rwin);
  pl.d_wcontig = (const int32_t *)(base + o_wc);
  const bool with_x = aligned && T == 512 && rd->d.srow != nullptr;
  HIP_TRY(tiles_buf.ensure((size_t)tiles * (sizeof(Tile) + (with_x ? sizeof(TileX) : 0))));
  const int nb = (int)((tiles + kBlock - 1) / kBlock);
  hipLaunchKernelGGL(plan_tiles, dim3(nb), dim3(kBlock), 0, c->stream, d_rc, d_rs, d_re, d_ro, d_rt, (int64_t)nr,
                     tiles, T, rd->d, (Tile *)tiles_buf.p, stage_cap, meta_cap, ev_cap, aligned ? 1 : 0,
                     with_x ? (TileX *)((Tile *)tiles_buf.p + tiles) : (TileX *)nullptr);
  HIP_TRY(hipGetLastError());
  return GQ_OK;
}

gq_status gq::check_device_error(gq_ctx *c, const Counters &h) {
  if (h.err == 1 && h.prof[4])
    fprintf(stderr, "gq: record slot %lld (k %llu of %llu): key %llx contig %d pos %d flags/gt %llx\n",
            (long long)h.err_pos, h.prof[3], h.prof[4], h.prof[0], (int)(h.prof[1] >> 32), (int)(uint32_t)h.prof[1],
            h.prof[2]);
  if (h.err) {
    static const char *names[] = {"ok", "assertion", "invalid cigar element", "CIGAR / MD tag mismatch",
                                  "read without MD tag", "multiple reference bases", "unsorted", "argument", "hip",
                                  "nomem", "allele table capacity"};
    const char *nm = (h.err >= 0 && h.err <= 10) ? names[h.err] : "?";
    return set_err((gq_status)h.err, "device error: %s near position %lld", nm, (long long)h.err_pos);
  }
  return GQ_OK;
}

extern "C" {

static bool germline_direct_mode(const DevReads &R) {
  static const char *m = getenv("GQ_GERM");
  static const bool proj = m && strcmp(m, "proj") == 0;
  return !proj && R.seq_cap >= 8;
}

static unsigned germline_grid(gq_ctx *c, int64_t tiles, bool direct) {
  if (c->n_cu <= 0 && hipDeviceGetAttribute(&c->n_cu, hipDeviceAttributeMultiprocessorCount, c->device) != hipSuccess)
    c->n_cu = 256;
  int &per_cu = direct ? c->dir_wg_per_cu : c->proj_wg_per_cu;
  if (per_cu <= 0) {
    int nb = 0;
    const hipError_t e = direct ? hipOccupancyMaxActiveBlocksPerMultiprocessor(&nb, germline_direct<false>, DirCfg::kThreads, 0)
                                : hipOccupancyMaxActiveBlocksPerMultiprocessor(&nb, germline_proj, ProjCfg::kThreads, 0);
    if (e != hipSuccess || nb <= 0) nb = 2;
    per_cu = nb;
  }
  const int64_t want = (tiles + ProjCfg::kWaves - 1) / ProjCfg::kWaves;
  return (unsigned)std::max<int64_t>(1, std::min<int64_t>({want, (int64_t)per_cu * c->n_cu, (int64_t)kPartsCols}));
}

static gq_status launch_germline(gq_ctx *c, int64_t tiles, const DevReads &R, const gq_germline_params *p,
                                 CallRec *recs, ComplexItem *cplx, const OutGeom &og, Counters *ctr, bool direct) {
  static const int dbg = getenv("GQ_DBG") ? atoi(getenv("GQ_DBG")) : 0;
  HIP_TRY(c->slow.ensure((size_t)tiles * sizeof(int32_t)));
  if (tiles >= (int64_t)1 << 24) return set_err(GQ_E_ARG, "%lld tiles in one call (at most 2^24)", (long long)tiles);
  if (direct) {
    HIP_TRY(c->deep_tiles.ensure((size_t)tiles * sizeof(int32_t)));
    hipLaunchKernelGGL(germline_direct<false>, dim3((unsigned)og.ncols), dim3(DirCfg::kThreads), 0, c->stream,
                       (const Tile *)c->tiles.p, tiles, R, p->threshold, p->emit_ref, p->emit_no_call, recs, cplx, og, ctr,
                       (int32_t *)c->slow.p, (int32_t *)c->deep_tiles.p, dbg);
    HIP_TRY(hipGetLastError());
    hipLaunchKernelGGL(germline_direct<true>, dim3((unsigned)std::min<int64_t>((tiles + DirCfg::kWaves - 1) / DirCfg::kWaves, 512)),
                       dim3(DirCfg::kThreads), 0, c->stream, (const Tile *)c->tiles.p, tiles, R, p->threshold,
                       p->emit_ref, p->emit_no_call, recs, cplx, og, ctr, (int32_t *)c->slow.p,
                       (int32_t *)c->deep_tiles.p, dbg);
  } else {
    hipLaunchKernelGGL(germline_proj, dim3((unsigned)og.ncols), dim3(ProjCfg::kThreads), 0, c->stream,
                       (const Tile *)c->tiles.p, (const TileX *)((const Tile *)c->tiles.p + tiles), tiles, R.proj,
                       R.pev, R.n_samples,
                       p->threshold, p->emit_ref, p->emit_no_call, recs, cplx, og, ctr, (int32_t *)c->slow.p, dbg);
  }
  HIP_TRY(hipGetLastError());
  HIP_TRY(hipEventRecord(c->ev[5], c->stream));
  const unsigned wblocks = (unsigned)std::min<int64_t>(tiles, 2048);
  hipLaunchKernelGGL((germline_walk<ProjCfg::kT>), dim3(wblocks), dim3(kBlock), 0, c->stream,
                     (const Tile *)c->tiles.p, (const int32_t *)c->slow.p, R, p->threshold, p->emit_ref,
                     p->emit_no_call, recs, cplx, og, ctr);
  HIP_TRY(hipGetLastError());
  return GQ_OK;
}

static gq_status germline_run(gq_ctx *c, const gq_dev_reads *rd, const gq_loci *loci, const gq_germline_params *p,
                              gq_calls **out, gq_calls_device *dev) {
  if (!c || !rd || !loci || !p || !out) return set_err(GQ_E_ARG, "gq_germline_threshold: null argument");
  HIP_TRY(hipSetDevice(c->device));
  const int T = c->germ_tile;
  c->timings = gq_timings{};
  const auto h0 = std::chrono::steady_clock::now();
  HIP_TRY(hipEventRecord(c->ev[0], c->stream));
  Plan pl;
  const bool direct = germline_direct_mode(rd->d);
  gq_status st = direct ? GQ_OK : ensure_projection(c, rd);
  if (st) return st;
  st = plan(c, rd, loci, T, pl, c->tiles, 0, 0, 0, true);
  if (st) return st;
  HIP_TRY(hipEventRecord(c->ev[1], c->stream));
  gq_calls *res = (gq_calls *)calloc(1, sizeof(gq_calls));
  if (!res) return set_err(GQ_E_NOMEM, "calloc");
  if (pl.n_tiles == 0) {
    *out = res;
    return GQ_OK;
  }
  const int ns = rd->d.n_samples;
  OutGeom og{};
  og.ncols = (int)germline_grid(c, pl.n_tiles, direct);
  const bool dense = p->emit_ref || p->emit_no_call;
  const unsigned long long wg_loci = (unsigned long long)((pl.n_tiles + og.ncols - 1) / og.ncols) * T;
  og.capA[0] = dense ? 2ull * ns * wg_loci + 64 : wg_loci / 32 + 256;
  og.capA[1] = wg_loci / 32 + 256;
  og.capB[0] = dense ? 2ull * ns * (unsigned long long)pl.n_loci / 8192 + 256 : (unsigned long long)pl.n_loci / 16384 + 256;
  og.capB[1] = (unsigned long long)pl.n_loci / 16384 + 256;
  unsigned long long pool_cap = 1 << 22, amb_cap = 4096;
  unsigned long long gdeep_cap = 1024;
  Counters hc{};
  const int bshift = dense ? 0 : 9;
  const uint64_t dead_key = ((uint64_t)pl.n_loci << 12) | 0xFFFu;
  const int64_t nbk = (pl.n_loci >> bshift) + 1;
  size_t scan_tmp = 0;
  HIP_TRY(hipcub::DeviceScan::ExclusiveSum(nullptr, scan_tmp, (const uint32_t *)nullptr, (uint32_t *)nullptr,
                                           (int)(nbk + 1), c->stream));
  auto finalize = [&](Counters *ctr, size_t cap_rec) -> gq_status {
    uint32_t *cnt = (uint32_t *)c->bkt.p, *off = cnt + (nbk + 1), *fill = off + (nbk + 1);
    hipLaunchKernelGGL(zero_u32, dim3((unsigned)std::min<int64_t>((3 * (nbk + 1) + kBlock - 1) / kBlock, 1024)),
                       dim3(kBlock), 0, c->stream, cnt, 3 * (nbk + 1));
    const unsigned gb = (unsigned)std::max<int64_t>(1, std::min<int64_t>(((int64_t)cap_rec + kBlock - 1) / kBlock, kFinBlocks));
    hipLaunchKernelGGL(bucket_count, dim3(gb), dim3(kBlock), 0, c->stream, (const CallRec *)c->recs.p,
                       ctr, og, dead_key, bshift, nbk, (uint64_t *)c->keys.p, (int32_t *)c->idx_sorted.p,
                       (int64_t *)c->idx.p, cnt);
    HIP_TRY(hipGetLastError());
    HIP_TRY(hipcub::DeviceScan::ExclusiveSum(c->sort_tmp.p, scan_tmp, cnt, off, (int)(nbk + 1), c->stream));
    hipLaunchKernelGGL(bucket_scatter, dim3(gb), dim3(kBlock), 0, c->stream, (const Counters *)ctr,
                       (const int64_t *)c->idx.p, (const uint32_t *)off, fill, (int32_t *)c->keys_sorted.p);
    HIP_TRY(hipGetLastError());
    hipLaunchKernelGGL(bucket_rank, dim3(gb), dim3(kBlock), 0, c->stream, nbk, (const uint32_t *)off,
                       (const int32_t *)c->keys_sorted.p, (const uint64_t *)c->keys.p, (const int32_t *)c->idx_sorted.p,
                       (const int64_t *)c->idx.p, (int32_t *)c->recs_sorted.p);
    HIP_TRY(hipGetLastError());
    int64_t *bsum = (int64_t *)c->keys_sorted.p + (cap_rec + 1) / 2 + 1;
    hipLaunchKernelGGL(img_sums, dim3(kImgBlocks), dim3(kBlock), 0, c->stream, (const CallRec *)c->recs.p,
                       (const int32_t *)c->recs_sorted.p, (const uint32_t *)off, nbk, bsum);
    hipLaunchKernelGGL(img_scan, dim3(1), dim3(kImgBlocks), 0, c->stream, bsum);
    hipLaunchKernelGGL(calls_image, dim3(kImgBlocks), dim3(kBlock), 0, c->stream, (const CallRec *)c->recs.p,
                       (const int32_t *)c->recs_sorted.p, (const uint32_t *)off, nbk, (const int64_t *)bsum,
                       (const uint8_t *)c->pool.p, ctr, (uint8_t *)c->image.p);
    HIP_TRY(hipGetLastError());
    return GQ_OK;
  };
  auto read_counters = [&](Counters *ctr) -> gq_status {
    HIP_TRY(c->pinned(kCountersHead));
    HIP_TRY(hipMemcpyAsync(c->pin, ctr, kCountersHead, hipMemcpyDeviceToHost, c->stream));
    HIP_TRY(hipStreamSynchronize(c->stream));
    memcpy(&hc, c->pin, kCountersHead);
    return GQ_OK;
  };
  for (int attempt = 0; attempt < 3; ++attempt) {
    HIP_TRY(c->amb.ensure(2 * amb_cap * sizeof(AmbItem)));
    const size_t cap_rec = (size_t)og.total(0);
    HIP_TRY(c->recs.ensure(cap_rec * sizeof(CallRec)));
    HIP_TRY(c->cplx.ensure(og.total(1) * sizeof(ComplexItem)));
    HIP_TRY(c->pool.ensure(pool_cap));
    HIP_TRY(c->counters.ensure(sizeof(Counters)));
    HIP_TRY(c->keys.ensure((cap_rec + 1) * 8));
    HIP_TRY(c->keys_sorted.ensure((cap_rec + 1) * 4 + 8 * (kImgBlocks + 2) + 16));
    HIP_TRY(c->idx.ensure((cap_rec + 1) * 8));
    HIP_TRY(c->idx_sorted.ensure((cap_rec + 1) * 4));
    HIP_TRY(c->recs_sorted.ensure((cap_rec + 1) * 4));
    HIP_TRY(c->bkt.ensure(sizeof(uint32_t) * (size_t)(3 * (nbk + 1))));
    HIP_TRY(c->sort_tmp.ensure(std::max<size_t>(scan_tmp, 16)));
    HIP_TRY(c->image.ensure(calls_layout((int64_t)cap_rec, (int64_t)pool_cap).bytes));
    Counters *ctr = (Counters *)c->counters.p;
    HIP_TRY(hipMemsetAsync(ctr, 0, sizeof(Counters), c->stream));
    if (attempt == 0) HIP_TRY(hipEventRecord(c->ev[1], c->stream));
    st = launch_germline(c, pl.n_tiles, rd->d, p, (CallRec *)c->recs.p, (ComplexItem *)c->cplx.p, og, ctr, direct);
    if (st) {
      free(res);
      return st;
    }
    HIP_TRY(hipEventRecord(c->ev[2], c->stream));
#ifndef GQ_CPLX_BLOCKS
#define GQ_CPLX_BLOCKS 4096
#endif
    const int cblocks = (int)std::min<int64_t>(std::max<int64_t>(pl.n_tiles, 1), GQ_CPLX_BLOCKS);
    SomWin wb{};
    st = window_bounds(c, pl, rd, wb);
    if (st) {
      free(res);
      return st;
    }
    hipLaunchKernelGGL(part_scan, dim3(1), dim3(1024), 0, c->stream, ctr, 1, og);
    HIP_TRY(c->deep_list.ensure(3 * sizeof(int64_t) * (size_t)gdeep_cap));
    auto complex_pair = [&](int blocks, int which, AmbItem *amb_out, unsigned long long acap, const AmbItem *amb_in,
                            const uint8_t *amb_ref, int64_t n_amb_in, const SomWin &sw_) -> gq_status {
      int64_t *region = (int64_t *)c->deep_list.p + (size_t)which * gdeep_cap;
      const DeepList fast{region, &ctr->n_gdeep[which], nullptr, nullptr, gdeep_cap};
      const DeepList wide{nullptr, nullptr, region, &ctr->n_gdeep[which], gdeep_cap};
      hipLaunchKernelGGL(germline_complex<2>, dim3(blocks), dim3(kBlock), 0, c->stream, (const Tile *)c->tiles.p,
                         (const ComplexItem *)c->cplx.p, rd->d, p->threshold, p->emit_ref, p->emit_no_call,
                         (CallRec *)c->recs.p, og, (uint8_t *)c->pool.p, pool_cap, ctr, amb_out, acap, amb_in, amb_ref,
                         n_amb_in, gq_dbg(), sw_, fast);
      HIP_TRY(hipGetLastError());
      hipLaunchKernelGGL(germline_complex<16>, dim3(64), dim3(kBlock), 0, c->stream, (const Tile *)c->tiles.p,
                         (const ComplexItem *)c->cplx.p, rd->d, p->threshold, p->emit_ref, p->emit_no_call,
                         (CallRec *)c->recs.p, og, (uint8_t *)c->pool.p, pool_cap, ctr, amb_out, acap, amb_in, amb_ref,
                         n_amb_in, gq_dbg(), sw_, wide);
      HIP_TRY(hipGetLastError());
      return GQ_OK;
    };
    st = complex_pair(cblocks, 0, (AmbItem *)c->amb.p, amb_cap, (const AmbItem *)nullptr, (const uint8_t *)nullptr,
                      (int64_t)0, wb);
    if (st) {
      free(res);
      return st;
    }
    hipLaunchKernelGGL(part_scan, dim3(1), dim3(1024), 0, c->stream, ctr, 0, og);
    {
#ifndef GQ_EXPAND_BLOCKS
#define GQ_EXPAND_BLOCKS 1024
#endif
      hipLaunchKernelGGL(germline_expand, dim3(GQ_EXPAND_BLOCKS), dim3(kBlock), 0, c->stream, (CallRec *)c->recs.p, ctr, og,
                         p->threshold, p->emit_ref, p->emit_no_call, dead_key);
      HIP_TRY(hipGetLastError());
    }
    HIP_TRY(hipEventRecord(c->ev[3], c->stream));
    st = finalize(ctr, cap_rec);
    if (st) {
      free(res);
      return st;
    }
    HIP_TRY(hipEventRecord(c->ev[4], c->stream));
    st = read_counters(ctr);
    if (st) {
      free(res);
      return st;
    }
    bool retry = false;
    for (int w = 0; w < 2; ++w)
      if (hc.part_max[w]) {
        og.capA[w] += hc.part_max[w] + 64;
        og.capB[w] += hc.part_max[w] + 64;
        retry = true;
      }
    if (hc.pool_used > pool_cap) {
      pool_cap = hc.pool_used + 4096;
      retry = true;
    }
    if (hc.n_amb > amb_cap || hc.n_ord > amb_cap) {
      amb_cap = std::max(hc.n_amb, hc.n_ord) + 1024;
      retry = true;
    }
    if (hc.n_gdeep[0] > gdeep_cap) {
      gdeep_cap = hc.n_gdeep[0] + 1024;
      retry = true;
    }
    SomWin sw{};
    const bool rerun = !retry && (hc.n_amb > 0 || hc.n_ord > 0) && !hc.err;
    if (rerun) {
      st = build_somwin(c, pl, rd, rd, sw);
      if (st) {
        free(res);
        return st;
      }
    }
    if (rerun && hc.n_ord > 0) {
      const int oblocks = (int)std::min<int64_t>(((int64_t)hc.n_ord + 3) / 4, 4096);
      st = complex_pair(oblocks, 1, (AmbItem *)nullptr, (unsigned long long)0, (const AmbItem *)c->amb.p + amb_cap,
                        (const uint8_t *)nullptr, (int64_t)hc.n_ord, sw);
      if (st) {
        free(res);
        return st;
      }
      hipLaunchKernelGGL(part_scan, dim3(1), dim3(1024), 0, c->stream, ctr, 0, og);
    }
    if (rerun && hc.n_amb > 0) {
      std::vector<AmbItem> amb((size_t)hc.n_amb);
      HIP_TRY(hipMemcpyAsync(amb.data(), c->amb.p, amb.size() * sizeof(AmbItem), hipMemcpyDeviceToHost, c->stream));
      HIP_TRY(hipStreamSynchronize(c->stream));
      HIP_TRY(c->amb_ref.ensure(amb.size()));
      st = heap_ref_bases(c, pl, c->tiles, {rd}, amb, (uint8_t *)c->amb_ref.p);
      if (st) {
        free(res);
        return st;
      }
      const int ablocks = (int)std::min<int64_t>(((int64_t)amb.size() + 3) / 4, 4096);
      st = complex_pair(ablocks, 2, (AmbItem *)nullptr, (unsigned long long)0, (const AmbItem *)c->amb.p,
                        (const uint8_t *)c->amb_ref.p, (int64_t)amb.size(), sw);
      if (st) {
        free(res);
        return st;
      }
      hipLaunchKernelGGL(part_scan, dim3(1), dim3(1024), 0, c->stream, ctr, 0, og);
    }
    if (rerun) {
      HIP_TRY(hipEventRecord(c->ev[3], c->stream));
      st = read_counters(ctr);
      if (st) {
        free(res);
        return st;
      }
      if (hc.part_max[0]) {
        og.capA[0] += hc.part_max[0] + 64;
        og.capB[0] += hc.part_max[0] + 64;
        retry = true;
      }
      if (hc.pool_used > pool_cap) {
        pool_cap = hc.pool_used + 4096;
        retry = true;
      }
      if (std::max(hc.n_gdeep[1], hc.n_gdeep[2]) > gdeep_cap) {
        gdeep_cap = std::max(hc.n_gdeep[1], hc.n_gdeep[2]) + 1024;
        retry = true;
      }
      if (!retry) {
        st = finalize(ctr, cap_rec);
        if (!st) {
          HIP_TRY(hipEventRecord(c->ev[4], c->stream));
          st = read_counters(ctr);
        }
        if (st) {
          free(res);
          return st;
        }
      }
    }
    if (!retry) break;
    if (attempt == 2) {
      free(res);
      return set_err(GQ_E_CAPACITY, "output capacity retries exhausted");
    }
  }
  if ((gq_dbg() & 32) && hc.prof[4])
    fprintf(stderr, "gq germline_complex prof (cycles/item/wave): cover %.0f reference-base %.0f elements %.0f "
            "map-order %.0f decision %.0f (%llu items)\n", (double)hc.prof[0] / hc.prof[4],
            (double)hc.prof[1] / hc.prof[4], (double)hc.prof[2] / hc.prof[4], (double)hc.prof[5] / hc.prof[4],
            (double)hc.prof[3] / hc.prof[4], hc.prof[4]);
  if ((gq_dbg() & 16) && hc.prof[5])
    fprintf(stderr,
            "gq prof (cycles/tile/wave): setup %.0f chunks %.0f (runs %.0f [fields %.0f slots %.0f] counting %.0f) "
            "decision %.0f (%llu)\n",
            (double)hc.prof[0] / hc.prof[5], (double)hc.prof[1] / hc.prof[5], (double)hc.prof[2] / hc.prof[5],
            (double)hc.prof[6] / hc.prof[5], (double)hc.prof[7] / hc.prof[5], (double)hc.prof[3] / hc.prof[5],
            (double)hc.prof[4] / hc.prof[5], hc.prof[5]);
  for (int k = 0; k < kSpread; ++k) {
    hc.visited += hc.spread[0][k];
    hc.ambiguous += hc.spread[1][k];
    hc.ties += hc.spread[2][k];
    hc.n_dead += hc.spread[3][k];
  }
  st = check_device_error(c, hc);
  if (st) {
    free(res);
    return st;
  }
  const int64_t n = (int64_t)hc.n_out;
  const CallsLayout lay = calls_layout(n, (int64_t)hc.out_pool);
  const int64_t pool_len = (int64_t)hc.out_pool;
  uint8_t *blk = nullptr;
  if (dev) {
    blk = (uint8_t *)c->image.p;
    dev->image = c->image.p;
    dev->image_bytes = (int64_t)lay.pool + pool_len;
  } else {
    const size_t nbytes = (size_t)lay.pool + (size_t)pool_len;
    blk = (uint8_t *)malloc(std::max<size_t>(nbytes, 64));
    if (!blk) {
      free(res);
      return set_err(GQ_E_NOMEM, "result block of %zu bytes", nbytes);
    }
    HIP_TRY(hipMemcpyAsync(blk, c->image.p, nbytes, hipMemcpyDeviceToHost, c->stream));
    HIP_TRY(hipStreamSynchronize(c->stream));
  }
  const auto h1 = std::chrono::steady_clock::now();
  res->n = n;
  res->block_ = dev ? nullptr : blk;
  res->contig = (int32_t *)(blk + lay.contig);
  res->pos = (int64_t *)(blk + lay.pos);
  res->ref_off = (int64_t *)(blk + lay.ref_off);
  res->alt_off = (int64_t *)(blk + lay.alt_off);
  res->ref_len = (int32_t *)(blk + lay.ref_len);
  res->alt_len = (int32_t *)(blk + lay.alt_len);
  res->sample = blk + lay.sample;
  res->gt0 = blk + lay.gt0;
  res->gt1 = blk + lay.gt1;
  res->flags = blk + lay.flags;
  res->allele_pool = blk + lay.pool;
  res->pool_len = pool_len;
  res->visited_loci = (int64_t)hc.visited;
  res->complex_loci = (int64_t)hc.n_complex;
  res->ambiguous_loci = (int64_t)hc.ambiguous;
  res->tie_loci = (int64_t)hc.ties;
  float ms = 0;
  (void)hipEventElapsedTime(&ms, c->ev[0], c->ev[1]);
  c->timings.plan_ms = ms;
  (void)hipEventElapsedTime(&ms, c->ev[1], c->ev[5]);
  c->timings.pileup_ms = ms;
  (void)hipEventElapsedTime(&ms, c->ev[5], c->ev[2]);
  c->timings.walk_ms = ms;
  c->timings.walk_tiles = (int64_t)hc.n_slow;
  c->timings.order_loci = (int64_t)hc.n_ord;
  (void)hipEventElapsedTime(&ms, c->ev[2], c->ev[3]);
  c->timings.complex_ms = ms;
  (void)hipEventElapsedTime(&ms, c->ev[3], c->ev[4]);
  c->timings.finalize_ms = ms;
  (void)hipEventElapsedTime(&ms, c->ev[0], c->ev[4]);
  c->timings.total_ms = ms;
  c->timings.pileup_launches = 1;
  c->timings.tiles = pl.n_tiles;
  const auto h2 = std::chrono::steady_clock::now();
  c->timings.host_ms = std::chrono::duration<float, std::milli>(h2 - h0).count();
  c->timings.marshal_ms = std::chrono::duration<float, std::milli>(h2 - h1).count();
  *out = res;
  return GQ_OK;
}

gq_status gq_germline_threshold(gq_ctx *c, const gq_dev_reads *rd, const gq_loci *loci,
                                const gq_germline_params *p, gq_calls **out) {
  return germline_run(c, rd, loci, p, out, nullptr);
}

gq_status gq_germline_threshold_device(gq_ctx *c, const gq_dev_reads *rd, const gq_loci *loci,
                                       const gq_germline_params *p, gq_calls_device *out) {
  if (!out) return set_err(GQ_E_ARG, "gq_germline_threshold_device: null argument");
  memset(out, 0, sizeof(*out));
  gq_calls *r = nullptr;
  const gq_status st = germline_run(c, rd, loci, p, &r, out);
  if (st) return st;
  out->calls = *r;
  out->calls.block_ = nullptr;
  free(r);
  return GQ_OK;
}

gq_status gq_write_vcf_germline(const char *path, const char *header, int64_t n, const int32_t *contig,
                                const int64_t *pos, const uint8_t *gt0, const uint8_t *gt1, const int64_t *ref_off,
                                const int32_t *ref_len, const int64_t *alt_off, const int32_t *alt_len,
                                const uint8_t *pool, int32_t n_contigs, const char *const *contig_names) {
  if (!path || !header || (n > 0 && (!contig || !pos || !gt0 || !gt1 || !ref_off || !ref_len || !alt_off || !alt_len ||
                                      !contig_names)))
    return set_err(GQ_E_ARG, "gq_write_vcf_germline: null argument");
  FILE *f = fopen(path, "wb");
  if (!f) return set_err(GQ_E_ARG, "cannot write %s", path);
  std::string buf(header);
  buf.reserve((size_t)n * 48 + buf.size() + 64);
  static const char kGt[4] = {'0', '1', '.', '.'};
  std::vector<size_t> clen((size_t)std::max(n_contigs, 0));
  for (int32_t k = 0; k < n_contigs; ++k) clen[(size_t)k] = contig_names[k] ? strlen(contig_names[k]) : 0;
  char num[24];
  bool ok = true;
  for (int64_t i = 0; i < n && ok; ++i) {
    const int32_t c = contig[i];
    if (c < 0 || c >= n_contigs || !contig_names[c]) {
      fclose(f);
      return set_err(GQ_E_ARG, "gq_write_vcf_germline: record %lld has contig %d", (long long)i, c);
    }
    buf.append(contig_names[c], clen[(size_t)c]);
    buf += '\t';
    const int k = snprintf(num, sizeof num, "%lld", (long long)(pos[i] + 1));
    buf.append(num, (size_t)k);
    buf.append("\t.\t", 3);
    buf.append((const char *)pool + ref_off[i], (size_t)ref_len[i]);
    buf += '\t';
    buf.append((const char *)pool + alt_off[i], (size_t)alt_len[i]);
    buf.append("\t.\t.\t.\tGT\t", 10);
    buf += kGt[gt0[i] & 3];
    buf += '/';
    buf += kGt[gt1[i] & 3];
    buf += '\n';
    if (buf.size() > (size_t)(64 << 20)) {
      ok = fwrite(buf.data(), 1, buf.size(), f) == buf.size();
      buf.clear();
    }
  }
  if (ok && !buf.empty()) ok = fwrite(buf.data(), 1, buf.size(), f) == buf.size();
  if (fclose(f) != 0) ok = false;
  return ok ? GQ_OK : set_err(GQ_E_ARG, "write to %s failed", path);
}

void gq_free_calls(gq_calls *r) {
  if (!r) return;
  free(r->block_);
  free(r);
}

gq_status gq_pileup_counts(gq_ctx *c, const gq_dev_reads *rd, const gq_loci *loci, gq_counts **out) {
  if (!c || !rd || !loci || !out) return set_err(GQ_E_ARG, "gq_pileup_counts: null argument");
  HIP_TRY(hipSetDevice(c->device));
  Plan pl;
  gq_status st = ensure_columns(c, rd);
  if (st) return st;
  st = plan(c, rd, loci, kCountT, pl, c->tiles);
  if (st) return st;
  gq_counts *res = (gq_counts *)calloc(1, sizeof(gq_counts));
  const int64_t n = pl.n_loci;
  res->n_loci = n;
  const size_t nn = (size_t)std::max<int64_t>(n, 1);
  res->depth = (int32_t *)malloc(nn * 4);
  res->pos_depth = (int32_t *)malloc(nn * 4);
  res->base_counts = (int32_t *)malloc(nn * 24);
  res->indel_counts = (int32_t *)malloc(nn * 16);
  res->ref_depth = (int32_t *)malloc(nn * 4);
  res->ref_base = (uint8_t *)malloc(nn);
  res->ambiguous = (uint8_t *)malloc(nn);
  if (n == 0) {
    *out = res;
    return GQ_OK;
  }
  HIP_TRY(c->c_depth.ensure(nn * 4));
  HIP_TRY(c->c_pos.ensure(nn * 4));
  HIP_TRY(c->c_base.ensure(nn * 24));
  HIP_TRY(c->c_indel.ensure(nn * 16));
  HIP_TRY(c->c_ref.ensure(nn * 4));
  HIP_TRY(c->c_rb.ensure(nn));
  HIP_TRY(c->c_amb.ensure(nn));
  HIP_TRY(c->counters.ensure(sizeof(Counters)));
  Counters *ctr = (Counters *)c->counters.p;
  HIP_TRY(hipMemsetAsync(ctr, 0, sizeof(Counters), c->stream));
  hipLaunchKernelGGL((counts_tile<kCountT>), dim3((unsigned)pl.n_tiles), dim3(kBlock), 0, c->stream,
                     (const Tile *)c->tiles.p, rd->d, (int32_t *)c->c_depth.p, (int32_t *)c->c_pos.p,
                     (int32_t *)c->c_base.p, (int32_t *)c->c_indel.p, (int32_t *)c->c_ref.p, (uint8_t *)c->c_rb.p,
                     (uint8_t *)c->c_amb.p, ctr);
  HIP_TRY(hipGetLastError());
  Counters hc{};
  HIP_TRY(hipMemcpyAsync(&hc, ctr, sizeof(Counters), hipMemcpyDeviceToHost, c->stream));
  HIP_TRY(hipMemcpyAsync(res->depth, c->c_depth.p, nn * 4, hipMemcpyDeviceToHost, c->stream));
  HIP_TRY(hipMemcpyAsync(res->pos_depth, c->c_pos.p, nn * 4, hipMemcpyDeviceToHost, c->stream));
  HIP_TRY(hipMemcpyAsync(res->base_counts, c->c_base.p, nn * 24, hipMemcpyDeviceToHost, c->stream));
  HIP_TRY(hipMemcpyAsync(res->indel_counts, c->c_indel.p, nn * 16, hipMemcpyDeviceToHost, c->stream));
  HIP_TRY(hipMemcpyAsync(res->ref_depth, c->c_ref.p, nn * 4, hipMemcpyDeviceToHost, c->stream));
  HIP_TRY(hipMemcpyAsync(res->ref_base, c->c_rb.p, nn, hipMemcpyDeviceToHost, c->stream));
  HIP_TRY(hipMemcpyAsync(res->ambiguous, c->c_amb.p, nn, hipMemcpyDeviceToHost, c->stream));
  HIP_TRY(hipStreamSynchronize(c->stream));
  st = check_device_error(c, hc);
  if (st) {
    gq_free_counts(res);
    return st;
  }
  {
    std::vector<AmbItem> amb;
    std::vector<int64_t> ords;
    int64_t o = 0;
    for (size_t r = 0; r < pl.rs.size(); ++r) {
      const int64_t len = pl.re[r] - pl.rs[r];
      for (int64_t i = 0; i < len; ++i)
        if (res->ambiguous[o + i]) {
          amb.push_back(AmbItem{(int32_t)(pl.rt[r] + i / kCountT), (int32_t)(pl.rs[r] + i), (int64_t)amb.size()});
          ords.push_back(o + i);
        }
      o += len;
    }
    if (!amb.empty()) {
      HIP_TRY(c->amb_ref.ensure(amb.size()));
      st = heap_ref_bases(c, pl, c->tiles, {rd}, amb, (uint8_t *)c->amb_ref.p);
      if (st) {
        gq_free_counts(res);
        return st;
      }
      std::vector<uint8_t> rb(amb.size());
      HIP_TRY(hipMemcpy(rb.data(), c->amb_ref.p, rb.size(), hipMemcpyDeviceToHost));
      HIP_TRY(hipMemcpy(&hc, ctr, sizeof(Counters), hipMemcpyDeviceToHost));
      st = check_device_error(c, hc);
      if (st) {
        gq_free_counts(res);
        return st;
      }
      for (size_t k = 0; k < amb.size(); ++k) {
        const int64_t x = ords[k];
        const uint8_t b = rb[k];
        const int cat = b == 'A' ? 0 : b == 'C' ? 1 : b == 'G' ? 2 : b == 'T' ? 3 : 4;
        res->ref_base[x] = b;
        res->ref_depth[x] = res->base_counts[x * 6 + cat];
      }
    }
  }
  *out = res;
  return GQ_OK;
}

gq_status gq_vaf_histogram(gq_ctx *c, const gq_dev_reads *rd, const gq_loci *loci, const gq_vaf_params *p,
                           gq_vaf_hist *out) {
  if (!c || !rd || !loci || !p || !out) return set_err(GQ_E_ARG, "gq_vaf_histogram: null argument");
  if (p->bins < 1 || p->bins > 100) return set_err(GQ_E_ASSERT, "assumption failed: Bins should be between 1 and 100");
  HIP_TRY(hipSetDevice(c->device));
  memset(out, 0, sizeof(*out));
  Plan pl;
  gq_status st = ensure_columns(c, rd);
  if (st) return st;
  st = plan(c, rd, loci, kCountT, pl, c->tiles);
  if (st) return st;
  if (pl.n_tiles == 0) return GQ_OK;
  unsigned long long amb_cap = 4096;
  Counters hc{};
  for (int attempt = 0;; ++attempt) {
    HIP_TRY(c->counters.ensure(sizeof(Counters)));
    HIP_TRY(c->c_depth.ensure(sizeof(unsigned long long) * 64 * 101));
    HIP_TRY(c->amb.ensure(amb_cap * sizeof(AmbItem)));
    HIP_TRY(c->c_base.ensure(amb_cap * sizeof(VafAmb)));
    Counters *ctr = (Counters *)c->counters.p;
    HIP_TRY(hipMemsetAsync(ctr, 0, sizeof(Counters), c->stream));
    HIP_TRY(hipMemsetAsync(c->c_depth.p, 0, sizeof(unsigned long long) * 64 * 101, c->stream));
    hipLaunchKernelGGL((vaf_tile<kCountT>), dim3((unsigned)pl.n_tiles), dim3(kBlock), 0, c->stream,
                       (const Tile *)c->tiles.p, rd->d, (int)p->bins, (int)p->min_read_depth, (int)p->min_vaf,
                       (unsigned long long *)c->c_depth.p, (AmbItem *)c->amb.p, (VafAmb *)c->c_base.p, amb_cap, ctr);
    HIP_TRY(hipGetLastError());
    HIP_TRY(hipMemcpyAsync(&hc, ctr, sizeof(Counters), hipMemcpyDeviceToHost, c->stream));
    HIP_TRY(hipStreamSynchronize(c->stream));
    if (hc.n_amb <= amb_cap || hc.err) break;
    if (attempt == 2) return set_err(GQ_E_CAPACITY, "vaf-histogram: listed-locus capacity retries exhausted");
    amb_cap = hc.n_amb + 1024;
  }
  st = check_device_error(c, hc);
  if (st) return st;
  std::vector<unsigned long long> h(64 * 101);
  HIP_TRY(hipMemcpy(h.data(), c->c_depth.p, sizeof(unsigned long long) * h.size(), hipMemcpyDeviceToHost));
  for (int k = 0; k < 64; ++k)
    for (int b = 0; b < 101; ++b) out->counts[b] += (int64_t)h[(size_t)k * 101 + (size_t)b];
  for (int k = 0; k < kSpread; ++k) {
    out->visited_loci += (int64_t)hc.spread[0][k];
    out->variant_loci += (int64_t)hc.spread[1][k];
  }
  if (hc.n_amb > 0) {
    std::vector<AmbItem> amb((size_t)hc.n_amb);
    std::vector<VafAmb> cnt((size_t)hc.n_amb);
    HIP_TRY(hipMemcpy(amb.data(), c->amb.p, amb.size() * sizeof(AmbItem), hipMemcpyDeviceToHost));
    HIP_TRY(hipMemcpy(cnt.data(), c->c_base.p, cnt.size() * sizeof(VafAmb), hipMemcpyDeviceToHost));
    HIP_TRY(c->amb_ref.ensure(amb.size()));
    st = heap_ref_bases(c, pl, c->tiles, {rd}, amb, (uint8_t *)c->amb_ref.p);
    if (st) return st;
    std::vector<uint8_t> rb(amb.size());
    HIP_TRY(hipMemcpy(rb.data(), c->amb_ref.p, rb.size(), hipMemcpyDeviceToHost));
    HIP_TRY(hipMemcpy(&hc, c->counters.p, sizeof(Counters), hipMemcpyDeviceToHost));
    st = check_device_error(c, hc);
    if (st) return st;
    const int bin_size = 100 / p->bins;
    for (size_t k = 0; k < amb.size(); ++k) {
      const uint8_t b = rb[k];
      const int cat = b == 'A' ? 0 : b == 'C' ? 1 : b == 'G' ? 2 : b == 'T' ? 3 : b == 'N' ? 4 : 5;
      const int32_t depth = cnt[k].depth, ref = cnt[k].base[cat];
      if (ref == depth) continue;
      const float vaf = (float)(depth - ref) / (float)depth;
      if (!(depth >= p->min_read_depth) || !((double)vaf >= (double)p->min_vaf / 100.0)) continue;
      const int pct = (int)(vaf * 100.0f);
      out->counts[pct - pct % bin_size] += 1;
      out->variant_loci += 1;
    }
  }
  return GQ_OK;
}

void gq_free_counts(gq_counts *r) {
  if (!r) return;
  free(r->depth);
  free(r->pos_depth);
  free(r->base_counts);
  free(r->indel_counts);
  free(r->ref_depth);
  free(r->ref_base);
  free(r->ambiguous);
  free(r);
}



}

gq_status gq::derive_shape(gq_ctx *c, gq_dev_reads *d, int64_t md_len) { return derive_shape_impl(c, d, md_len); }

gq_status gq::ensure_ev_bases(gq_ctx *c, const gq_dev_reads *cd) {
  gq_dev_reads *d = const_cast<gq_dev_reads *>(cd);
  if (d->ev_bases) return GQ_OK;
  void *q = nullptr;
  HIP_TRY(d->dp.get(&q, (size_t)std::max<int64_t>(d->d.md_len, 16)));
  if (d->d.n_reads > 0) {
    hipLaunchKernelGGL(ev_bases, dim3((unsigned)((d->d.n_reads + kBlock - 1) / kBlock)), dim3(kBlock), 0, c->stream,
                       d->d, (uint8_t *)q);
    HIP_TRY(hipGetLastError());
  }
  d->d.ev_rb = (const uint8_t *)q;
  d->ev_bases = true;
  return GQ_OK;
}

gq_status gq::ensure_columns(gq_ctx *c, const gq_dev_reads *cd) {
  gq_dev_reads *d = const_cast<gq_dev_reads *>(cd);
  if (d->columns) return GQ_OK;
  {
    const gq_status se = ensure_ev_bases(c, d);
    if (se) return se;
  }
  const int64_t n = d->d.n_reads;
  void *cl = nullptr, *nnb = nullptr;
  HIP_TRY(d->dp.get(&cl, (size_t)std::max<int64_t>(n, 1)));
  HIP_TRY(d->dp.get(&nnb, sizeof(uint32_t) * (size_t)std::max<int64_t>(n, 1)));
  HIP_TRY(hipMemsetAsync(nnb, 0, sizeof(uint32_t) * (size_t)std::max<int64_t>(n, 1), c->stream));
  if (n > 0) {
    if (d->d.pool_ordered) {
      HIP_TRY(hipMemsetAsync(cl, 1, (size_t)n, c->stream));
      const int64_t chunks = (d->d.seq_bytes + 15) / 16;
      if (chunks > 0)
        hipLaunchKernelGGL(pool_clean, dim3((unsigned)((chunks + 2 * kBlock - 1) / (2 * kBlock))), dim3(kBlock), 0,
                           c->stream, d->d, (uint8_t *)cl, (uint32_t *)nnb);
    } else {
      hipLaunchKernelGGL(read_clean, dim3((unsigned)((n + kBlock - 1) / kBlock)), dim3(kBlock), 0, c->stream, d->d,
                         (uint8_t *)cl, (uint32_t *)nnb);
    }
    HIP_TRY(hipGetLastError());
  }
  d->d.clean = (const uint8_t *)cl;
  d->nnb = nnb;
  void *cdp = nullptr, *ce = nullptr, *ao = nullptr, *na = nullptr;
  const size_t ncd = sizeof(ColDesc) * (size_t)std::max<int64_t>(n, 1) + 1024;
  HIP_TRY(d->dp.get(&cdp, ncd));
  HIP_TRY(hipMemsetAsync(cdp, 0, ncd, c->stream));
  HIP_TRY(d->dp.get(&ao, sizeof(int64_t) * (size_t)(n + 1)));
  HIP_TRY(d->dp.get((void **)&na, sizeof(uint32_t) * (size_t)(n + 1)));
  const unsigned nb = (unsigned)((n + 1 + kBlock - 1) / kBlock);
  hipLaunchKernelGGL(col_count, dim3(nb), dim3(kBlock), 0, c->stream, d->d, (uint32_t *)na);
  HIP_TRY(hipGetLastError());
  HIP_TRY(scan_u32_to_i64(d->dp, (const uint32_t *)na, (int64_t *)ao, n + 1, c->stream));
  d->dp.put(na);
  const int64_t aux_bound = std::max<int64_t>(d->d.md_len, 0) + 6 * std::max<int64_t>(d->d.cigar_len, 0);
  const size_t nce = sizeof(uint32_t) * (size_t)std::max<int64_t>(aux_bound, 1) + 1024;
  HIP_TRY(d->dp.get(&ce, nce));
  d->d.cdesc = (const ColDesc *)cdp;
  d->d.cev = (const uint32_t *)ce;
  d->d.caux_off = (const int64_t *)ao;
  if (n > 0) {
    hipLaunchKernelGGL(col_derive, dim3((unsigned)((n + kBlock - 1) / kBlock)), dim3(kBlock), 0, c->stream, d->d,
                       (const int64_t *)ao, (ColDesc *)cdp, (uint32_t *)ce, aux_bound);
    HIP_TRY(hipGetLastError());
  }
  d->columns = true;
  return GQ_OK;
}

gq_status gq::ensure_projection(gq_ctx *c, const gq_dev_reads *cd) {
// ... 120 lines not shown
```

guacamole_amd/csrc/gq_somatic.hip:

```cpp
#include <hip/hip_runtime.h>

#include <algorithm>
#include <chrono>
#include <cmath>
#include <cstdio>
#include <cstdlib>
#include <cstring>
#include <vector>

#include "gq_alleles.h"
#include <hipcub/hipcub.hpp>

#include "gq_host.h"
#include "gq_strictmath.h"
#include "gq_scala_order.h"

#pragma clang fp contract(off)

using namespace gq;

namespace {

#include "gq_winorder.h"

// ... 1173 lines not shown
  img[L.sample + k] = (uint8_t)((r.key >> 4) & 0xFFu);
  ((int64_t *)(img + L.ref_off))[k] = at;
  ((int32_t *)(img + L.ref_len))[k] = r.ref_len;
  ((int64_t *)(img + L.alt_off))[k] = at + r.ref_len;
  ((int32_t *)(img + L.alt_len))[k] = r.alt_len;
  ((double *)(img + L.log_odds))[k] = r.log_odds;
  ((int32_t *)(img + L.gq))[k] = r.gq;
  ((gq_evidence *)(img + L.tumor))[k] = r.tumor;
  ((gq_evidence *)(img + L.normal))[k] = r.normal;
  img[L.flags + k] = r.flags;
  uint8_t *o = img + L.pool + at;
  if (tot <= 8)
    for (int i = 0; i < tot; ++i) o[i] = (uint8_t)(r.allele >> (8 * i));
  else
    for (int i = 0; i < tot; ++i) o[i] = dpool[r.allele + (uint64_t)i];
  if (k == n - 1) *(int64_t *)img = at + tot;
}

gq_status fetch_somatic_records(gq_ctx *c, const Counters &hc, unsigned long long pool_cap, uint64_t key_bound,
                                gq_somatic_calls *res) {
  const int64_t n = (int64_t)hc.n_rec;
  const size_t nn = (size_t)std::max<int64_t>(n, 1);
  const SomLayout lay = som_layout(n, (int64_t)std::min<unsigned long long>(hc.pool_used, pool_cap));
  HIP_TRY(c->image.ensure(lay.bytes));
  if (n > 0) {
    HIP_TRY(c->keys.ensure(nn * 8));
    HIP_TRY(c->keys_sorted.ensure(nn * 8));
    HIP_TRY(c->idx.ensure(nn * 8));
    HIP_TRY(c->idx_sorted.ensure(nn * 8));
    const unsigned nb = (unsigned)((n + kBlock - 1) / kBlock);
    uint64_t *keys = (uint64_t *)c->keys.p, *keys2 = (uint64_t *)c->keys_sorted.p;
    uint32_t *slot = (uint32_t *)c->idx.p, *order = (uint32_t *)c->idx_sorted.p;
    int64_t *len = (int64_t *)c->keys.p, *off = (int64_t *)c->idx.p;
    hipLaunchKernelGGL(som_keys, dim3(nb), dim3(kBlock), 0, c->stream, (const SomRec *)c->srecs.p, n, keys, slot);
    HIP_TRY(hipGetLastError());
    const int end_bit = key_bound ? 64 - __builtin_clzll(key_bound) : 64;
    size_t tmp = 0, tmp2 = 0;
    HIP_TRY(hipcub::DeviceRadixSort::SortPairs(nullptr, tmp, keys, keys2, slot, order, (int)n, 0, end_bit, c->stream));
    HIP_TRY(hipcub::DeviceScan::ExclusiveSum(nullptr, tmp2, len, off, (int)n, c->stream));
    HIP_TRY(c->sort_tmp.ensure(std::max(tmp, tmp2)));
    HIP_TRY(hipcub::DeviceRadixSort::SortPairs(c->sort_tmp.p, tmp, keys, keys2, slot, order, (int)n, 0, end_bit,
                                               c->stream));
    hipLaunchKernelGGL(som_lengths, dim3(nb), dim3(kBlock), 0, c->stream, (const SomRec *)c->srecs.p,
                       (const uint32_t *)order, n, len);
    HIP_TRY(hipGetLastError());
    HIP_TRY(hipcub::DeviceScan::ExclusiveSum(c->sort_tmp.p, tmp2, len, off, (int)n, c->stream));
    hipLaunchKernelGGL(som_image, dim3(nb), dim3(kBlock), 0, c->stream, (const SomRec *)c->srecs.p,
                       (const uint32_t *)order, (const int64_t *)off, (const uint8_t *)c->pool.p, n, lay,
                       (uint8_t *)c->image.p);
    HIP_TRY(hipGetLastError());
  } else {
    HIP_TRY(hipMemsetAsync(c->image.p, 0, 64, c->stream));
  }
  uint8_t *blk = (uint8_t *)malloc(lay.bytes);
  if (!blk) return set_err(GQ_E_NOMEM, "somatic result block of %zu bytes", lay.bytes);
  const hipError_t e = hipMemcpyAsync(blk, c->image.p, lay.bytes, hipMemcpyDeviceToHost, c->stream);
  if (e == hipSuccess) (void)hipEventRecord(c->ev[4], c->stream);
  if (e != hipSuccess || hipStreamSynchronize(c->stream) != hipSuccess) {
    free(blk);
    return set_err(GQ_E_HIP, "somatic result image D2H");
  }
  const auto m0 = std::chrono::steady_clock::now();
  res->n = n;
  res->block_ = blk;
  res->contig = (int32_t *)(blk + lay.contig);
  res->pos = (int64_t *)(blk + lay.pos);
  res->sample = blk + lay.sample;
  res->ref_off = (int64_t *)(blk + lay.ref_off);
  res->ref_len = (int32_t *)(blk + lay.ref_len);
  res->alt_off = (int64_t *)(blk + lay.alt_off);
  res->alt_len = (int32_t *)(blk + lay.alt_len);
  res->log_odds = (double *)(blk + lay.log_odds);
  res->gq = (int32_t *)(blk + lay.gq);
  res->tumor = (gq_evidence *)(blk + lay.tumor);
  res->normal = (gq_evidence *)(blk + lay.normal);
  res->flags = blk + lay.flags;
  res->allele_pool = blk + lay.pool;
  res->pool_len = n > 0 ? *(const int64_t *)blk : 0;
  c->timings.marshal_ms = std::chrono::duration<float, std::milli>(std::chrono::steady_clock::now() - m0).count();
  return GQ_OK;
}

}

struct gq_reference {
  int device = 0;
  int32_t n_contigs = 0;
  void *bytes = nullptr;
  int64_t *d_off = nullptr;
  std::vector<int64_t> off, len;
};

extern "C" {

gq_status gq_reference_upload(gq_ctx *c, int32_t n_contigs, const uint8_t *const *bases, const int64_t *lengths,
                              gq_reference **out) {
  if (!c || n_contigs < 0 || (n_contigs > 0 && (!bases || !lengths)) || !out)
    return set_err(GQ_E_ARG, "gq_reference_upload: bad argument");
  HIP_TRY(hipSetDevice(c->device));
  gq_reference *r = new gq_reference();
  r->device = c->device;
  r->n_contigs = n_contigs;
  r->off.assign((size_t)n_contigs, -1);
  r->len.assign((size_t)n_contigs, -1);
  int64_t tot = 0;
  for (int32_t k = 0; k < n_contigs; ++k) {
    if (!bases[k] || lengths[k] < 0) continue;
    r->off[(size_t)k] = tot;
    r->len[(size_t)k] = lengths[k];
    tot += (lengths[k] + 1023) / 512 * 512;
  }
  auto fail = [&](gq_status st) {
    gq_reference_free(r);
    return st;
  };
  if (hipMalloc(&r->bytes, (size_t)std::max<int64_t>(tot, 512)) != hipSuccess ||
      hipMalloc((void **)&r->d_off, sizeof(int64_t) * (size_t)std::max(n_contigs, 1)) != hipSuccess)
    return fail(set_err(GQ_E_HIP, "gq_reference_upload: hipMalloc of %lld bytes failed", (long long)tot));
  if (hipMemsetAsync(r->bytes, 'N', (size_t)std::max<int64_t>(tot, 512), c->stream) != hipSuccess)
    return fail(set_err(GQ_E_HIP, "gq_reference_upload: memset failed"));
  for (int32_t k = 0; k < n_contigs; ++k)
    if (r->off[(size_t)k] >= 0 && lengths[k] > 0 &&
        hipMemcpyAsync((uint8_t *)r->bytes + r->off[(size_t)k], bases[k], (size_t)lengths[k], hipMemcpyHostToDevice,
                       c->stream) != hipSuccess)
      return fail(set_err(GQ_E_HIP, "gq_reference_upload: copy of contig %d failed", k));
  if (n_contigs > 0 && hipMemcpyAsync(r->d_off, r->off.data(), sizeof(int64_t) * (size_t)n_contigs,
                                      hipMemcpyHostToDevice, c->stream) != hipSuccess)
    return fail(set_err(GQ_E_HIP, "gq_reference_upload: offsets copy failed"));
  if (hipStreamSynchronize(c->stream) != hipSuccess) return fail(set_err(GQ_E_HIP, "gq_reference_upload: sync failed"));
  *out = r;
  return GQ_OK;
}

void gq_reference_free(gq_reference *r) {
  if (!r) return;
  (void)hipSetDevice(r->device);
  if (r->bytes) (void)hipFree(r->bytes);
  if (r->d_off) (void)hipFree(r->d_off);
  delete r;
}

gq_status gq_somatic_standard(gq_ctx *c, const gq_dev_reads *t, const gq_dev_reads *n, const gq_loci *loci,
                              const gq_somatic_params *p, gq_somatic_calls **out) {
  return gq_somatic_standard_ref(c, t, n, loci, nullptr, p, out);
}

gq_status gq_somatic_standard_ref(gq_ctx *c, const gq_dev_reads *t, const gq_dev_reads *n, const gq_loci *loci,
                                  const gq_reference *ref, const gq_somatic_params *p, gq_somatic_calls **out) {
  if (!c || !t || !n || !loci || !p || !out) return set_err(GQ_E_ARG, "gq_somatic_standard: null argument");
  if (t->d.n_contigs != n->d.n_contigs)
    return set_err(GQ_E_ARG, "tumor and normal read sets must share the contig list (%d vs %d contigs)",
                   t->d.n_contigs, n->d.n_contigs);
  const int dbg = getenv("GQ_DBG") ? atoi(getenv("GQ_DBG")) : 0;
  RefView rv{nullptr, nullptr};
  std::vector<int32_t> lc;
  std::vector<int64_t> ls, le, lt;
  gq_loci trimmed{};
  if (ref) {
    if (ref->n_contigs != t->d.n_contigs)
      return set_err(GQ_E_ARG, "reference covers %d contigs, the read sets %d", ref->n_contigs, t->d.n_contigs);
    if (ref->device != c->device) return set_err(GQ_E_ARG, "reference uploaded to another device");
    HIP_TRY(hipSetDevice(c->device));
    auto covered = [&](int32_t ci, int64_t a, int64_t b, bool *hit) -> gq_status {
      *hit = false;
      for (const gq_dev_reads *sr : {t, n}) {
        std::vector<char> o;
        const gq_status s2 = reads_overlap(c, sr, ci, {{a, b}}, o);
        if (s2) return s2;
        if (o[0]) *hit = true;
      }
      return GQ_OK;
    };
    for (int64_t k = 0; k < loci->n_ranges; ++k) {
      const int32_t ci = loci->contig[k];
      const int64_t s0 = loci->start[k];
      int64_t e0 = loci->end[k];
      if (e0 <= s0) continue;
      if (ci < 0 || ci >= ref->n_contigs) return set_err(GQ_E_ARG, "loci range on contig %d: no such contig", ci);
      bool hit = false;
      if (ref->off[(size_t)ci] < 0) {
        const gq_status s2 = covered(ci, s0, e0, &hit);
        if (s2) return s2;
        if (hit) return set_err(GQ_E_ARG, "contig %d does not exist in the current reference", ci);
        continue;
      }
      const int64_t len = ref->len[(size_t)ci];
      if (e0 > len) {
        const gq_status s2 = covered(ci, std::max(len, s0), e0, &hit);
        if (s2) return s2;
        if (hit)
          return set_err(GQ_E_ARG, "locus %lld of contig %d is past the end of the reference contig (length %lld)",
                         (long long)std::max(len, s0), ci, (long long)len);
        e0 = len;
        if (e0 <= s0) continue;
      }
      lc.push_back(ci);
      ls.push_back(s0);
      le.push_back(e0);
      lt.push_back(loci->task ? loci->task[k] : 0);
    }
    trimmed = gq_loci{(int64_t)lc.size(), lc.data(), ls.data(), le.data(), loci->task ? lt.data() : nullptr};
    loci = &trimmed;
    rv = RefView{(const uint8_t *)ref->bytes, ref->d_off};
  }
  HIP_TRY(hipSetDevice(c->device));
  const auto h0 = std::chrono::steady_clock::now();
  c->timings = gq_timings{};
  HIP_TRY(hipEventRecord(c->ev[0], c->stream));
  Plan pt, pn;
  static const bool som_proj = getenv("GQ_SOM") && strcmp(getenv("GQ_SOM"), "proj") == 0;
  const bool direct = !som_proj && t->d.seq_cap >= 8;
  gq_status st = direct ? GQ_OK : ensure_projection(c, t);
  if (st) return st;
  st = plan(c, t, loci, SomProjCfg::kT, pt, c->tiles, 0, 0, 0, true);
  if (st) return st;
  st = plan(c, n, loci, SomProjCfg::kT, pn, c->tiles2, 0, 0, 0, true);
  if (st) return st;
  gq_somatic_calls *res = (gq_somatic_calls *)calloc(1, sizeof(gq_somatic_calls));
  if (!res) return set_err(GQ_E_NOMEM, "calloc");
  if (pt.n_tiles == 0) {
    *out = res;
    return GQ_OK;
  }
  {
    static_assert(sizeof(double) == 8, "FP64");
    double succ[256];
    for (int q = 0; q < 256; ++q) succ[q] = 1.0 - std::pow(10.0, -q / 10.0);
    HIP_TRY(hipMemcpyToSymbolAsync(HIP_SYMBOL(g_succ), succ, sizeof succ, 0, hipMemcpyHostToDevice, c->stream));
    HIP_TRY(hipStreamSynchronize(c->stream));
  }
  SomWin sw{};
  st = build_somwin(c, pt, t, n, sw);
  if (st) {
    free(res);
    return st;
  }
  if (direct) {
    if (c->mtab_key != 1) {
      HIP_TRY(c->mtab.ensure(256 * 256));
      hipLaunchKernelGGL(margin_table, dim3(256), dim3(256), 0, c->stream, 1, (uint8_t *)c->mtab.p);
      HIP_TRY(hipGetLastError());
      c->mtab_key = 1;
    }
  } else {
    st = ensure_margin_projection(c, t, (int)p->min_mapq);
  }
  if (st) {
    free(res);
    return st;
  }
  OutGeom og{};
  {
    if (c->n_cu <= 0 &&
        hipDeviceGetAttribute(&c->n_cu, hipDeviceAttributeMultiprocessorCount, c->device) != hipSuccess)
      c->n_cu = 256;
    int &wg_cu = direct ? c->somd_wg_per_cu : c->som_wg_per_cu;
    if (wg_cu <= 0) {
      int nb = 0;
      const hipError_t e =
          direct ? hipOccupancyMaxActiveBlocksPerMultiprocessor(&nb, somatic_direct<false>, SomDirCfg::kThreads, 0)
                 : hipOccupancyMaxActiveBlocksPerMultiprocessor(&nb, somatic_proj<false>, SomProjCfg::kThreads, 0);
      if (e != hipSuccess || nb <= 0) nb = direct ? 2 : 4;
      wg_cu = nb;
    }
    og.ncols = (int)std::max<int64_t>(1, std::min<int64_t>({(pt.n_tiles + SomProjCfg::kWaves - 1) / SomProjCfg::kWaves,
                                                           (int64_t)wg_cu * c->n_cu, (int64_t)kPartsCols}));
    const unsigned long long wg_loci = (unsigned long long)((pt.n_tiles + og.ncols - 1) / og.ncols) * SomProjCfg::kT;
    og.capA[1] = wg_loci / 16 + 256;
    og.capB[1] = (unsigned long long)pt.n_loci / 65536 + 1024;
  }
  unsigned long long rec_cap = 1 << 16, pool_cap = 1 << 20, amb_cap = 4096, deep_cap = 4096;
  Counters hc{};
  float call_ms = 0, deep_ms = 0;
  for (int attempt = 0; attempt < 3; ++attempt) {
    HIP_TRY(c->amb.ensure(amb_cap * sizeof(AmbItem)));
    HIP_TRY(c->cplx.ensure(og.total(1) * sizeof(ComplexItem)));
    HIP_TRY(c->srecs.ensure(rec_cap * sizeof(SomRec)));
    HIP_TRY(c->pool.ensure(pool_cap));
    HIP_TRY(c->slow.ensure((size_t)pt.n_tiles * sizeof(int32_t)));
    HIP_TRY(c->counters.ensure(sizeof(Counters)));
    Counters *ctr = (Counters *)c->counters.p;
    HIP_TRY(hipMemsetAsync(ctr, 0, sizeof(Counters), c->stream));
    HIP_TRY(hipEventRecord(c->ev[1], c->stream));
    if (direct) {
      if (rv.b)
        hipLaunchKernelGGL(somatic_direct<true>, dim3((unsigned)og.ncols), dim3(SomDirCfg::kThreads), 0, c->stream,
                           (const Tile *)c->tiles.p, (const Tile *)c->tiles2.p, pt.n_tiles, t->d, n->d.start, n->d.end,
                           (const uint8_t *)c->mtab.p, (int)p->min_mapq, (ComplexItem *)c->cplx.p, og, ctr,
                           (int32_t *)c->slow.p, rv, 0, (dbg >> 16) & 0xFF);
      else
        hipLaunchKernelGGL(somatic_direct<false>, dim3((unsigned)og.ncols), dim3(SomDirCfg::kThreads), 0, c->stream,
                           (const Tile *)c->tiles.p, (const Tile *)c->tiles2.p, pt.n_tiles, t->d, n->d.start, n->d.end,
                           (const uint8_t *)c->mtab.p, (int)p->min_mapq, (ComplexItem *)c->cplx.p, og, ctr,
                           (int32_t *)c->slow.p, rv, 0, (dbg >> 16) & 0xFF);
    } else if (rv.b)
      hipLaunchKernelGGL(somatic_proj<true>, dim3((unsigned)og.ncols), dim3(SomProjCfg::kThreads), 0, c->stream,
                         (const Tile *)c->tiles.p, (const Tile *)c->tiles2.p, pt.n_tiles, t->d,
                         (const uint8_t *)t->mproj, (const uint8_t *)t->mnb, n->d.start, n->d.end, (ComplexItem *)c->cplx.p, og, ctr,
                         (int32_t *)c->slow.p, rv);
    else
      hipLaunchKernelGGL(somatic_proj<false>, dim3((unsigned)og.ncols), dim3(SomProjCfg::kThreads), 0, c->stream,
                         (const Tile *)c->tiles.p, (const Tile *)c->tiles2.p, pt.n_tiles, t->d,
                         (const uint8_t *)t->mproj, (const uint8_t *)t->mnb, n->d.start, n->d.end, (ComplexItem *)c->cplx.p, og, ctr,
                         (int32_t *)c->slow.p, rv);
    HIP_TRY(hipGetLastError());
    hipLaunchKernelGGL((somatic_tile<SomProjCfg::kT>), dim3((unsigned)std::min<int64_t>(pt.n_tiles, 2048)), dim3(kBlock), 0,
// ... 53 lines not shown
    auto run_deep = [&](int64_t n_items, const AmbItem *ain, const uint8_t *aref) -> gq_status {
      const int scap = (int)std::max<unsigned long long>(hc.deep_max, (unsigned long long)kFastCap);
      const int64_t nw = std::min<int64_t>(n_items, 4096);
      const size_t wb = deep_wave_bytes(scap, kMaxG);
      HIP_TRY(c->deep_scratch.ensure((size_t)nw * wb + 256));
      HIP_TRY(hipEventRecord(c->ev[5], c->stream));
      const unsigned blocks = (unsigned)((nw + kSomWaves - 1) / kSomWaves);
      hipLaunchKernelGGL(somatic_call_k<true>, dim3(blocks), dim3(kBlock), 0, c->stream,
                         (const CandRec *)c->cands.p, t->d, n->d, *p,
                         (SomRec *)c->srecs.p, rec_cap, (uint8_t *)c->pool.p, pool_cap, og, ctr, sw,
                         (AmbItem *)(ain ? nullptr : c->amb.p), ain ? (unsigned long long)0 : amb_cap, ain, aref,
                         ain ? n_items : (int64_t)0, ain ? RefView{nullptr, nullptr} : rv, dbg,
                         DeepIO{(int64_t *)c->deep_list.p, 0, ain ? 0 : n_items, (uint8_t *)c->deep_scratch.p, scap,
                                kMaxG, (int64_t *)c->deep_list.p + deep_cap, deep_cap});
      HIP_TRY(hipGetLastError());
      HIP_TRY(hipEventRecord(c->ev[3], c->stream));
      HIP_TRY(hipMemcpyAsync(&hc, ctr, sizeof(Counters), hipMemcpyDeviceToHost, c->stream));
      HIP_TRY(hipStreamSynchronize(c->stream));
      float ms = 0;
      (void)hipEventElapsedTime(&ms, c->ev[5], c->ev[3]);
      deep_ms += ms;
      return GQ_OK;
    };
    if (!retry && hc.n_deep > 0 && !hc.err) {
      st = run_deep((int64_t)hc.n_deep, nullptr, nullptr);
      if (st) {
        free(res);
        return st;
      }
    }
    if (hc.n_wide > deep_cap) {
      deep_cap = hc.n_wide + 1024;
      retry = true;
    }
    auto run_wide = [&](int64_t n_items, const AmbItem *ain, const uint8_t *aref, int64_t n_ain) -> gq_status {
      const int scap = (int)std::max<unsigned long long>(hc.deep_max, (unsigned long long)kFastCap);
      const int maxg = 64 * kWideNS * (64 * kWideNS + 1) / 2;
      const int64_t nw = std::min<int64_t>(n_items, 16);
      const size_t wb = deep_wave_bytes(scap, maxg, kWideNS);
      HIP_TRY(c->deep_scratch.ensure((size_t)nw * wb + 256));
      HIP_TRY(hipEventRecord(c->ev[5], c->stream));
      hipLaunchKernelGGL((somatic_call_k<true, kWideNS>), dim3((unsigned)((nw + kSomWaves - 1) / kSomWaves)),
                         dim3(kBlock), 0, c->stream, (const CandRec *)c->cands.p, t->d, n->d, *p, (SomRec *)c->srecs.p,
                         rec_cap, (uint8_t *)c->pool.p, pool_cap, og, ctr, sw, (AmbItem *)(ain ? nullptr : c->amb.p),
                         ain ? (unsigned long long)0 : amb_cap, ain, aref, ain ? n_ain : (int64_t)0,
                         ain ? RefView{nullptr, nullptr} : rv, dbg,
                         DeepIO{(int64_t *)c->deep_list.p + deep_cap, 0, n_items, (uint8_t *)c->deep_scratch.p,
                                scap, maxg, nullptr, 0});
      HIP_TRY(hipGetLastError());
      HIP_TRY(hipEventRecord(c->ev[3], c->stream));
      HIP_TRY(hipMemcpyAsync(&hc, ctr, sizeof(Counters), hipMemcpyDeviceToHost, c->stream));
      HIP_TRY(hipStreamSynchronize(c->stream));
      float ms = 0;
      (void)hipEventElapsedTime(&ms, c->ev[5], c->ev[3]);
      deep_ms += ms;
      return GQ_OK;
    };
    if (!retry && hc.n_wide > 0 && !hc.err) {
      st = run_wide((int64_t)hc.n_wide, nullptr, nullptr, 0);
      if (st) {
        free(res);
        return st;
      }
    }
    if (hc.n_amb > amb_cap) {
      amb_cap = hc.n_amb + 1024;
      retry = true;
    }
    if (!retry && hc.n_amb > 0 && !hc.err) {
      std::vector<AmbItem> amb((size_t)hc.n_amb);
      HIP_TRY(hipMemcpyAsync(amb.data(), c->amb.p, amb.size() * sizeof(AmbItem), hipMemcpyDeviceToHost, c->stream));
      HIP_TRY(hipStreamSynchronize(c->stream));
      HIP_TRY(c->amb_ref.ensure(2 * amb.size()));
      st = heap_ref_bases(c, pt, c->tiles, {t, n}, amb, (uint8_t *)c->amb_ref.p);
      if (st) {
        free(res);
        return st;
      }
      HIP_TRY(hipMemsetAsync(&ctr->n_wide, 0, sizeof(ctr->n_wide), c->stream));
      st = run_deep((int64_t)amb.size(), (const AmbItem *)c->amb.p, (const uint8_t *)c->amb_ref.p);
      if (st) {
        free(res);
        return st;
      }
      if (hc.n_wide > deep_cap) {
        deep_cap = hc.n_wide + 1024;
        retry = true;
      }
      if (!retry && hc.n_wide > 0 && !hc.err) {
        st = run_wide((int64_t)hc.n_wide, (const AmbItem *)c->amb.p, (const uint8_t *)c->amb_ref.p, (int64_t)amb.size());
        if (st) {
          free(res);
          return st;
        }
      }
    }
    if (hc.n_rec > rec_cap) {
      rec_cap = hc.n_rec + 1024;
      retry = true;
    }
    if (hc.pool_used > pool_cap) {
      pool_cap = hc.pool_used + 4096;
      retry = true;
    }
    if (!retry) break;
    if (attempt == 2) {
      free(res);
      return set_err(GQ_E_CAPACITY, "output capacity retries exhausted");
    }
  }
  for (int k = 0; k < kSpread; ++k) hc.visited += hc.spread[0][k];
  if ((dbg & 16) && hc.prof[5])
    fprintf(stderr, "gq somatic_call prof (cycles/candidate/wave): front %.0f (tumor fold %.0f) tables %.0f "
            "tumor-genotypes %.0f normal-genotypes+evidence %.0f (%llu candidates reached)\n", (double)hc.prof[0] / hc.prof[5],
            (double)hc.prof[1] / hc.prof[5], (double)hc.prof[2] / hc.prof[5], (double)hc.prof[3] / hc.prof[5],
            (double)hc.prof[4] / hc.prof[5], hc.prof[5]);
  st = check_device_error(c, hc);
  if (st) {
    free(res);
    return st;
  }
  st = fetch_somatic_records(c, hc, pool_cap, (uint64_t)std::max<int64_t>(pt.n_loci, 1) << 12, res);
  if (st) {
    free(res);
    return st;
  }
  res->visited_loci = (int64_t)hc.visited;
  res->candidate_loci = (int64_t)hc.n_complex;
  float ms = 0;
  (void)hipEventElapsedTime(&ms, c->ev[1], c->ev[2]);
  c->timings.pileup_ms = ms;
  (void)hipEventElapsedTime(&ms, c->ev[2], c->ev[3]);
  c->timings.complex_ms = ms;
  (void)hipEventElapsedTime(&ms, c->ev[3], c->ev[4]);
  c->timings.finalize_ms = ms;
  (void)hipEventElapsedTime(&ms, c->ev[0], c->ev[4]);
  c->timings.total_ms = ms;
  c->timings.pileup_launches = 1;
  c->timings.tiles = pt.n_tiles;
  c->timings.walk_tiles = (int64_t)hc.n_slow;
  c->timings.deep_loci = (int64_t)hc.n_deep;
  c->timings.deep_max = (int64_t)hc.deep_max;
  c->timings.call_ms = call_ms;
  c->timings.deep_ms = deep_ms;
  c->timings.front_ms = 0;
  c->timings.host_ms = std::chrono::duration<float, std::milli>(std::chrono::steady_clock::now() - h0).count();
  *out = res;
  return GQ_OK;
}

gq_status gq_variant_support(gq_ctx *c, const gq_dev_reads *rd, const gq_loci *loci, gq_allele_counts **out) {
  if (!c || !rd || !loci || !out) return set_err(GQ_E_ARG, "gq_variant_support: null argument");
  HIP_TRY(hipSetDevice(c->device));
  const auto h0 = std::chrono::steady_clock::now();
  c->timings = gq_timings{};
  HIP_TRY(hipEventRecord(c->ev[0], c->stream));
  Plan pl;
  gq_status st = ensure_columns(c, rd);
  if (st) return st;
  st = plan(c, rd, loci, 512, pl, c->tiles);
  if (st) return st;
  gq_allele_counts *res = (gq_allele_counts *)calloc(1, sizeof(gq_allele_counts));
  if (!res) return set_err(GQ_E_NOMEM, "calloc");
  auto fail = [&](gq_status e) {
    gq_free_allele_counts(res);
    return e;
  };
  unsigned long long rec_cap = (unsigned long long)std::max<int64_t>(pl.n_loci * 2, 1024), pool_cap = 1 << 16,
                     amb_cap = 4096, deep_cap = 1024;
  Counters hc{};
  const int blocks = (int)std::min<int64_t>(std::max<int64_t>((pl.n_loci + kSomWaves - 1) / kSomWaves, 1), 8192);
  for (int attempt = 0; pl.n_tiles > 0; ++attempt) {
    HIP_TRY(c->amb.ensure(amb_cap * sizeof(AmbItem)));
    HIP_TRY(c->srecs.ensure(rec_cap * sizeof(VsRec)));
    HIP_TRY(c->pool.ensure(pool_cap));
    HIP_TRY(c->counters.ensure(sizeof(Counters)));
    HIP_TRY(c->deep_list.ensure(deep_cap * sizeof(int64_t)));
    Counters *ctr = (Counters *)c->counters.p;
    HIP_TRY(hipMemsetAsync(ctr, 0, sizeof(Counters), c->stream));
    HIP_TRY(hipEventRecord(c->ev[1], c->stream));
    int64_t *dl = (int64_t *)c->deep_list.p;
    const DeepSel fast{dl, deep_cap, nullptr, 0, nullptr, 0, 0};
    auto run_deep = [&](int64_t from, const AmbItem *ain, const uint8_t *aref, int64_t n_ain) -> gq_status {
      HIP_TRY(hipMemcpyAsync(&hc, ctr, sizeof(Counters), hipMemcpyDeviceToHost, c->stream));
      HIP_TRY(hipStreamSynchronize(c->stream));
      const int64_t nd = (int64_t)std::min<unsigned long long>(hc.n_deep, deep_cap) - from;
      if (nd <= 0 || hc.err) return GQ_OK;
      const DeepSel deep{nullptr, deep_cap, dl + from, nd, nullptr, 0, 0};
      const int db = (int)std::min<int64_t>((nd + kSomWaves - 1) / kSomWaves, 64);
      hipLaunchKernelGGL(variant_support_call<true>, dim3((unsigned)db), dim3(kBlock), 0, c->stream,
                         (const Tile *)c->tiles.p, pl.n_tiles, pl.n_loci, rd->d, (VsRec *)c->srecs.p, rec_cap,
                         (uint8_t *)c->pool.p, pool_cap, ctr, ain ? (AmbItem *)nullptr : (AmbItem *)c->amb.p,
                         ain ? (unsigned long long)0 : amb_cap, ain, aref, n_ain, deep);
      HIP_TRY(hipGetLastError());
      HIP_TRY(hipMemcpyAsync(&hc, ctr, sizeof(Counters), hipMemcpyDeviceToHost, c->stream));
      HIP_TRY(hipStreamSynchronize(c->stream));
      return GQ_OK;
    };
    hipLaunchKernelGGL(variant_support_call<false>, dim3((unsigned)blocks), dim3(kBlock), 0, c->stream,
                       (const Tile *)c->tiles.p, pl.n_tiles, pl.n_loci, rd->d, (VsRec *)c->srecs.p, rec_cap,
                       (uint8_t *)c->pool.p, pool_cap, ctr, (AmbItem *)c->amb.p, amb_cap, (const AmbItem *)nullptr,
                       (const uint8_t *)nullptr, (int64_t)0, fast);
    HIP_TRY(hipGetLastError());
    st = run_deep(0, nullptr, nullptr, 0);
    if (st) return fail(st);
    bool retry = false;
    if (hc.n_amb > amb_cap) {
      amb_cap = hc.n_amb + 1024;
      retry = true;
    }
    if (hc.n_deep > deep_cap) {
      deep_cap = hc.n_deep + 1024;
      retry = true;
    }
    if (!retry && hc.n_amb > 0 && !hc.err) {
      std::vector<AmbItem> amb((size_t)hc.n_amb);
      HIP_TRY(hipMemcpyAsync(amb.data(), c->amb.p, amb.size() * sizeof(AmbItem), hipMemcpyDeviceToHost, c->stream));
      HIP_TRY(hipStreamSynchronize(c->stream));
      HIP_TRY(c->amb_ref.ensure(amb.size()));
      st = heap_ref_bases(c, pl, c->tiles, {rd}, amb, (uint8_t *)c->amb_ref.p);
      if (st) return fail(st);
      const int ab = (int)std::min<int64_t>(((int64_t)amb.size() + kSomWaves - 1) / kSomWaves, 8192);
      const int64_t from = (int64_t)hc.n_deep;
      hipLaunchKernelGGL(variant_support_call<false>, dim3((unsigned)ab), dim3(kBlock), 0, c->stream,
                         (const Tile *)c->tiles.p, pl.n_tiles, pl.n_loci, rd->d, (VsRec *)c->srecs.p, rec_cap,
                         (uint8_t *)c->pool.p, pool_cap, ctr, (AmbItem *)nullptr, (unsigned long long)0,
                         (const AmbItem *)c->amb.p, (const uint8_t *)c->amb_ref.p, (int64_t)amb.size(), fast);
      HIP_TRY(hipGetLastError());
      st = run_deep(from, (const AmbItem *)c->amb.p, (const uint8_t *)c->amb_ref.p, (int64_t)amb.size());
      if (st) return fail(st);
      if (hc.n_deep > deep_cap) {
        deep_cap = hc.n_deep + 1024;
        retry = true;
      }
    }
    if (hc.n_rec > rec_cap) {
      rec_cap = hc.n_rec + 1024;
      retry = true;
    }
    if (hc.pool_used > pool_cap) {
      pool_cap = hc.pool_used + 4096;
      retry = true;
    }
    if (!retry || hc.err) break;
    if (attempt == 2) return fail(set_err(GQ_E_CAPACITY, "variant-support output capacity retries exhausted"));
  }
  HIP_TRY(hipEventRecord(c->ev[2], c->stream));
  st = check_device_error(c, hc);
  if (st) return fail(st);
  const int64_t nr = pl.n_tiles > 0 ? (int64_t)hc.n_rec : 0;
  std::vector<VsRec> recs((size_t)nr);
  std::vector<uint8_t> hpool((size_t)std::min<unsigned long long>(hc.pool_used, pool_cap));
  if (nr) HIP_TRY(hipMemcpyAsync(recs.data(), c->srecs.p, (size_t)nr * sizeof(VsRec), hipMemcpyDeviceToHost, c->stream));
  if (!hpool.empty()) HIP_TRY(hipMemcpyAsync(hpool.data(), c->pool.p, hpool.size(), hipMemcpyDeviceToHost, c->stream));
  HIP_TRY(hipStreamSynchronize(c->stream));
  auto bytes = [&](const VsRec &r) {
    std::string b((size_t)(r.ref_len + r.alt_len), '\0');
    for (int i = 0; i < r.ref_len + r.alt_len; ++i)
      b[(size_t)i] = (char)(r.ref_len + r.alt_len <= 8 ? (uint8_t)(r.allele >> (8 * i)) : hpool[(size_t)r.allele + (size_t)i]);
    return b;
  };
  std::vector<std::string> ab((size_t)nr);
  for (int64_t k = 0; k < nr; ++k) ab[(size_t)k] = bytes(recs[(size_t)k]);
  std::vector<int64_t> ord((size_t)nr);
  for (int64_t k = 0; k < nr; ++k) ord[(size_t)k] = k;
  std::sort(ord.begin(), ord.end(), [&](int64_t x, int64_t y) {
    const VsRec &a = recs[(size_t)x], &b = recs[(size_t)y];
    if (a.key != b.key) return a.key < b.key;
    const std::string ra = ab[(size_t)x].substr(0, a.ref_len), rb2 = ab[(size_t)y].substr(0, b.ref_len);
    if (ra != rb2) return ra < rb2;
    return ab[(size_t)x].substr(a.ref_len) < ab[(size_t)y].substr(b.ref_len);
  });
  const size_t N = (size_t)std::max<int64_t>(nr, 1);
  res->n = nr;
  res->contig = (int32_t *)malloc(N * 4);
  res->pos = (int64_t *)malloc(N * 8);
  res->sample = (int32_t *)malloc(N * 4);
  res->count = (int32_t *)malloc(N * 4);
  res->ref_off = (int64_t *)malloc(N * 8);
  res->alt_off = (int64_t *)malloc(N * 8);
  res->ref_len = (int32_t *)malloc(N * 4);
  res->alt_len = (int32_t *)malloc(N * 4);
  res->flags = (uint8_t *)malloc(N);
  std::string apool;
  for (int64_t q = 0; q < nr; ++q) {
    const int64_t k = ord[(size_t)q];
    const VsRec &r = recs[(size_t)k];
    res->contig[q] = r.contig;
    res->pos[q] = r.pos;
    res->sample[q] = r.sample;
    res->count[q] = r.count;
    res->ref_len[q] = r.ref_len;
    res->alt_len[q] = r.alt_len;
    res->ref_off[q] = (int64_t)apool.size();
    res->alt_off[q] = (int64_t)apool.size() + r.ref_len;
    res->flags[q] = r.flags;
    apool += ab[(size_t)k];
  }
  res->pool_len = (int64_t)apool.size();
  res->allele_pool = (uint8_t *)malloc(std::max<size_t>(apool.size(), 1));
  if (!apool.empty()) memcpy(res->allele_pool, apool.data(), apool.size());
  float ms = 0;
  (void)hipEventElapsedTime(&ms, c->ev[1], c->ev[2]);
  c->timings.pileup_ms = ms;
  (void)hipEventElapsedTime(&ms, c->ev[0], c->ev[2]);
  c->timings.total_ms = ms;
  c->timings.tiles = pl.n_tiles;
  c->timings.host_ms = std::chrono::duration<float, std::milli>(std::chrono::steady_clock::now() - h0).count();
  *out = res;
  return GQ_OK;
}

void gq_free_allele_counts(gq_allele_counts *r) {
  if (!r) return;
  free(r->contig);
  free(r->pos);
  free(r->sample);
  free(r->count);
  free(r->ref_off);
  free(r->alt_off);
  free(r->ref_len);
  free(r->alt_len);
  free(r->allele_pool);
  free(r->flags);
  free(r);
}

gq_status gq_germline_standard(gq_ctx *c, const gq_dev_reads *rd, const gq_loci *loci, const gq_germline_std_params *p,
                               gq_somatic_calls **out) {
  if (!c || !rd || !loci || !p || !out) return set_err(GQ_E_ARG, "gq_germline_standard: null argument");
  HIP_TRY(hipSetDevice(c->device));
  const auto h0 = std::chrono::steady_clock::now();
  c->timings = gq_timings{};
  HIP_TRY(hipEventRecord(c->ev[0], c->stream));
  Plan pt;
  gq_status st = ensure_projection(c, rd);
  if (st) return st;
  st = plan(c, rd, loci, SomProjCfg::kT, pt, c->tiles, 0, 0, 0, true);
  if (st) return st;
  gq_somatic_calls *res = (gq_somatic_calls *)calloc(1, sizeof(gq_somatic_calls));
  if (!res) return set_err(GQ_E_NOMEM, "calloc");
  auto fail = [&](gq_status e) {
    free(res);
    return e;
  };
  if (pt.n_tiles == 0) {
    *out = res;
    return GQ_OK;
  }
  {
    double succ[256];
    for (int q = 0; q < 256; ++q) succ[q] = 1.0 - std::pow(10.0, -q / 10.0);
    HIP_TRY(hipMemcpyToSymbolAsync(HIP_SYMBOL(g_succ), succ, sizeof succ, 0, hipMemcpyHostToDevice, c->stream));
    HIP_TRY(hipStreamSynchronize(c->stream));
  }
  SomWin sw{};
  st = build_somwin(c, pt, rd, rd, sw);
  if (st) return fail(st);
  st = ensure_margin_projection(c, rd, (int)p->min_mapq, false);
  if (st) return fail(st);
  const int no_bound = rd->d.n_samples > 1 ? 1 : 0;
  const bool direct = false;
  OutGeom og{};
  {
    if (c->n_cu <= 0 &&
        hipDeviceGetAttribute(&c->n_cu, hipDeviceAttributeMultiprocessorCount, c->device) != hipSuccess)
      c->n_cu = 256;
    int &wg_cu = direct ? c->somd_wg_per_cu : c->som_wg_per_cu;
    if (wg_cu <= 0) {
      int nb = 0;
      const hipError_t e =
          direct ? hipOccupancyMaxActiveBlocksPerMultiprocessor(&nb, somatic_direct<false>, SomDirCfg::kThreads, 0)
                 : hipOccupancyMaxActiveBlocksPerMultiprocessor(&nb, somatic_proj<false>, SomProjCfg::kThreads, 0);
      if (e != hipSuccess || nb <= 0) nb = direct ? 2 : 4;
      wg_cu = nb;
    }
    og.ncols = (int)std::max<int64_t>(1, std::min<int64_t>({(pt.n_tiles + SomProjCfg::kWaves - 1) / SomProjCfg::kWaves,
                                                           (int64_t)wg_cu * c->n_cu, (int64_t)kPartsCols}));
    const unsigned long long wg_loci = (unsigned long long)((pt.n_tiles + og.ncols - 1) / og.ncols) * SomProjCfg::kT;
    og.capA[1] = wg_loci / 16 + 256;
    og.capB[1] = (unsigned long long)pt.n_loci / 65536 + 1024;
  }
  unsigned long long rec_cap = 1 << 16, pool_cap = 1 << 20, amb_cap = 4096, deep_cap = 4096;
  Counters hc{};
  for (int attempt = 0; attempt < 3; ++attempt) {
    HIP_TRY(c->amb.ensure(amb_cap * sizeof(AmbItem)));
    HIP_TRY(c->cplx.ensure(og.total(1) * sizeof(ComplexItem)));
    HIP_TRY(c->srecs.ensure(rec_cap * sizeof(SomRec)));
    HIP_TRY(c->pool.ensure(pool_cap));
    HIP_TRY(c->slow.ensure((size_t)pt.n_tiles * sizeof(int32_t)));
    HIP_TRY(c->counters.ensure(sizeof(Counters)));
    Counters *ctr = (Counters *)c->counters.p;
    HIP_TRY(hipMemsetAsync(ctr, 0, sizeof(Counters), c->stream));
    HIP_TRY(hipEventRecord(c->ev[1], c->stream));
    hipLaunchKernelGGL(somatic_proj<false>, dim3((unsigned)og.ncols), dim3(SomProjCfg::kThreads), 0, c->stream,
                       (const Tile *)c->tiles.p, (const Tile *)c->tiles.p, pt.n_tiles, rd->d, (const uint8_t *)rd->mproj, (const uint8_t *)rd->mnb,
                       rd->d.start, rd->d.end, (ComplexItem *)c->cplx.p, og, ctr, (int32_t *)c->slow.p,
                       RefView{nullptr, nullptr}, no_bound);
    HIP_TRY(hipGetLastError());
    hipLaunchKernelGGL((somatic_tile<SomProjCfg::kT>), dim3((unsigned)std::min<int64_t>(pt.n_tiles, 2048)), dim3(kBlock), 0,
                       c->stream, (const Tile *)c->tiles.p, (const Tile *)c->tiles.p, rd->d, rd->d, (ComplexItem *)c->cplx.p,
                       og, (const int32_t *)c->slow.p, (int)p->min_mapq, ctr, RefView{nullptr, nullptr}, 1);
    HIP_TRY(hipGetLastError());
    hipLaunchKernelGGL(part_scan_som, dim3(1), dim3(1024), 0, c->stream, ctr, og);
    HIP_TRY(hipGetLastError());
    HIP_TRY(hipEventRecord(c->ev[2], c->stream));
    {
      unsigned long long pm = 0;
      HIP_TRY(hipMemcpyAsync(&pm, &ctr->part_max[1], sizeof(pm), hipMemcpyDeviceToHost, c->stream));
      HIP_TRY(hipStreamSynchronize(c->stream));
      if (pm) {
        og.capA[1] += pm + 64;
        og.capB[1] += pm + 64;
        if (attempt == 2) return fail(set_err(GQ_E_CAPACITY, "candidate capacity retries exhausted"));
        continue;
      }
    }
    const int cblocks = (int)std::min<int64_t>(std::max<int64_t>(pt.n_tiles, 1), 8192);
    HIP_TRY(c->deep_list.ensure(deep_cap * sizeof(int64_t)));
    int64_t *dl = (int64_t *)c->deep_list.p;
    const DeepSel fast{dl, deep_cap, nullptr, 0, nullptr, 0, 0};
    auto run_deep = [&](int64_t from, AmbItem *aout, unsigned long long acap, const AmbItem *ain, const uint8_t *aref,
                        int64_t n_ain) -> gq_status {
      HIP_TRY(hipMemcpyAsync(&hc, ctr, sizeof(Counters), hipMemcpyDeviceToHost, c->stream));
      HIP_TRY(hipStreamSynchronize(c->stream));
      const int64_t nd = (int64_t)std::min<unsigned long long>(hc.n_deep, deep_cap) - from;
      if (nd <= 0 || hc.err) return GQ_OK;
      const int scap = (int)std::max<unsigned long long>(hc.deep_max, 64);
      const int64_t nt = (int64_t)std::min<unsigned long long>(std::max<unsigned long long>(hc.deep_nt, 2), 64 * kDeepNS);
      const int maxG = (int)std::max<int64_t>(nt * (nt + 1) / 2, 16);
      const int64_t waves = std::min<int64_t>(nd, 256);
      HIP_TRY(c->deep_scratch.ensure((size_t)waves * gs_wave_bytes(scap, maxG) + 256));
      const DeepSel deep{nullptr, deep_cap, dl + from, nd, (uint8_t *)c->deep_scratch.p, scap, maxG};
      hipLaunchKernelGGL(germline_standard_call<true>, dim3((unsigned)((waves + kSomWaves - 1) / kSomWaves)),
                         dim3(kBlock), 0, c->stream, (const Tile *)c->tiles.p, (const ComplexItem *)c->cplx.p, rd->d, *p,
                         (SomRec *)c->srecs.p, rec_cap, (uint8_t *)c->pool.p, pool_cap, og, ctr, sw, aout, acap, ain,
                         aref, n_ain, deep);
      HIP_TRY(hipGetLastError());
      HIP_TRY(hipMemcpyAsync(&hc, ctr, sizeof(Counters), hipMemcpyDeviceToHost, c->stream));
      HIP_TRY(hipStreamSynchronize(c->stream));
      return GQ_OK;
    };
    hipLaunchKernelGGL(germline_standard_call<false>, dim3(cblocks), dim3(kBlock), 0, c->stream, (const Tile *)c->tiles.p,
                       (const ComplexItem *)c->cplx.p, rd->d, *p, (SomRec *)c->srecs.p, rec_cap, (uint8_t *)c->pool.p,
                       pool_cap, og, ctr, sw, (AmbItem *)c->amb.p, amb_cap, (const AmbItem *)nullptr,
                       (const uint8_t *)nullptr, (int64_t)0, fast);
    HIP_TRY(hipGetLastError());
    st = run_deep(0, (AmbItem *)c->amb.p, amb_cap, nullptr, nullptr, 0);
    if (st) return fail(st);
    HIP_TRY(hipEventRecord(c->ev[3], c->stream));
    bool retry = false;
    if (hc.n_amb > amb_cap) {
      amb_cap = hc.n_amb + 1024;
      retry = true;
    }
    if (hc.n_deep > deep_cap) {
      deep_cap = hc.n_deep + 1024;
      retry = true;
    }
    if (!retry && hc.n_amb > 0 && !hc.err) {
      std::vector<AmbItem> amb((size_t)hc.n_amb);
      HIP_TRY(hipMemcpyAsync(amb.data(), c->amb.p, amb.size() * sizeof(AmbItem), hipMemcpyDeviceToHost, c->stream));
      HIP_TRY(hipStreamSynchronize(c->stream));
      HIP_TRY(c->amb_ref.ensure(amb.size()));
      st = heap_ref_bases(c, pt, c->tiles, {rd}, amb, (uint8_t *)c->amb_ref.p);
      if (st) return fail(st);
      const int ablocks = (int)std::min<int64_t>(((int64_t)amb.size() + 3) / 4, 8192);
      const int64_t from = (int64_t)hc.n_deep;
      hipLaunchKernelGGL(germline_standard_call<false>, dim3(ablocks), dim3(kBlock), 0, c->stream,
                         (const Tile *)c->tiles.p, (const ComplexItem *)c->cplx.p, rd->d, *p, (SomRec *)c->srecs.p,
                         rec_cap, (uint8_t *)c->pool.p, pool_cap, og, ctr, sw, (AmbItem *)nullptr,
                         (unsigned long long)0, (const AmbItem *)c->amb.p, (const uint8_t *)c->amb_ref.p,
                         (int64_t)amb.size(), fast);
      HIP_TRY(hipGetLastError());
      st = run_deep(from, (AmbItem *)nullptr, (unsigned long long)0, (const AmbItem *)c->amb.p,
                    (const uint8_t *)c->amb_ref.p, (int64_t)amb.size());
      if (st) return fail(st);
      HIP_TRY(hipEventRecord(c->ev[3], c->stream));
      if (hc.n_deep > deep_cap) {
        deep_cap = hc.n_deep + 1024;
        retry = true;
      }
    }
    if (hc.n_rec > rec_cap) {
      rec_cap = hc.n_rec + 1024;
      retry = true;
    }
    if (hc.pool_used > pool_cap) {
      pool_cap = hc.pool_used + 4096;
      retry = true;
    }
    if (!retry) break;
    if (attempt == 2) return fail(set_err(GQ_E_CAPACITY, "output capacity retries exhausted"));
  }
  for (int k = 0; k < kSpread; ++k) hc.visited += hc.spread[0][k];
  st = check_device_error(c, hc);
  if (st) return fail(st);
  st = fetch_somatic_records(c, hc, pool_cap, (uint64_t)std::max<int64_t>(pt.n_loci, 1) << 12, res);
  if (st) return fail(st);
  res->visited_loci = (int64_t)hc.visited;
  res->candidate_loci = (int64_t)hc.n_complex;
  float ms = 0;
  (void)hipEventElapsedTime(&ms, c->ev[1], c->ev[2]);
  c->timings.pileup_ms = ms;
  (void)hipEventElapsedTime(&ms, c->ev[2], c->ev[3]);
  c->timings.complex_ms = ms;
  (void)hipEventElapsedTime(&ms, c->ev[3], c->ev[4]);
  c->timings.finalize_ms = ms;
  (void)hipEventElapsedTime(&ms, c->ev[0], c->ev[4]);
  c->timings.total_ms = ms;
  c->timings.tiles = pt.n_tiles;
  c->timings.host_ms = std::chrono::duration<float, std::milli>(std::chrono::steady_clock::now() - h0).count();
  *out = res;
  return GQ_OK;
}

gq_status gq_allele_evidence(gq_ctx *c, const gq_dev_reads *rd, const gq_loci *loci,
                             const gq_allele_evidence_params *p, gq_allele_evidence_rows **out) {
  if (!c || !rd || !loci || !p || !out) return set_err(GQ_E_ARG, "gq_allele_evidence: null argument");
  HIP_TRY(hipSetDevice(c->device));
  const auto h0 = std::chrono::steady_clock::now();
  c->timings = gq_timings{};
  HIP_TRY(hipEventRecord(c->ev[0], c->stream));
  Plan pl;
  gq_status st = ensure_columns(c, rd);
  if (st) return st;
  st = plan(c, rd, loci, kAeT, pl, c->tiles);
  if (st) return st;
  gq_allele_evidence_rows *res = (gq_allele_evidence_rows *)calloc(1, sizeof(gq_allele_evidence_rows));
  if (!res) return set_err(GQ_E_NOMEM, "calloc");
  auto fail = [&](gq_status e) {
    gq_free_allele_evidence(res);
    return e;
  };
  if (pl.n_tiles == 0) {
    *out = res;
    return GQ_OK;
  }
  SomWin sw{};
  st = build_somwin(c, pl, rd, rd, sw);
  if (st) return fail(st);
  if (c->n_cu <= 0 && hipDeviceGetAttribute(&c->n_cu, hipDeviceAttributeMultiprocessorCount, c->device) != hipSuccess)
    c->n_cu = 256;
  unsigned long long item_cap = (unsigned long long)std::min<int64_t>(
                         pl.n_loci, std::max<int64_t>(pl.n_loci / 8, 1 << 16)),
                     rec_cap = 1 << 16, pool_cap = 1 << 16, amb_cap = 4096, deep_cap = 4096;
  Counters hc{};
  int64_t n_items = 0;
  for (int attempt = 0;; ++attempt) {
    HIP_TRY(c->amb.ensure(amb_cap * sizeof(AmbItem)));
    HIP_TRY(c->cplx.ensure(item_cap * sizeof(ComplexItem)));
    HIP_TRY(c->srecs.ensure(rec_cap * sizeof(AeRec)));
    HIP_TRY(c->pool.ensure(pool_cap));
    HIP_TRY(c->counters.ensure(sizeof(Counters)));
    HIP_TRY(c->deep_list.ensure(deep_cap * sizeof(int64_t)));
    Counters *ctr = (Counters *)c->counters.p;
    HIP_TRY(hipMemsetAsync(ctr, 0, sizeof(Counters), c->stream));
    HIP_TRY(hipEventRecord(c->ev[1], c->stream));
    hipLaunchKernelGGL((allele_evidence_list<kAeT>), dim3((unsigned)std::min<int64_t>(pl.n_tiles, (int64_t)4 * c->n_cu)),
                       dim3(kBlock), 0, c->stream, (const Tile *)c->tiles.p, pl.n_tiles, rd->d, (int)p->min_mapq,
                       (int)p->variants_only, (ComplexItem *)c->cplx.p, item_cap, ctr);
    HIP_TRY(hipGetLastError());
    HIP_TRY(hipEventRecord(c->ev[2], c->stream));
    HIP_TRY(hipEventRecord(c->ev[3], c->stream));
    HIP_TRY(hipMemcpyAsync(&hc, ctr, kCountersHead, hipMemcpyDeviceToHost, c->stream));
    HIP_TRY(hipStreamSynchronize(c->stream));
    if (hc.err) break;
    if (hc.n_complex > item_cap) {
      if (attempt == 2) return fail(set_err(GQ_E_CAPACITY, "allele-evidence: locus list capacity retries exhausted"));
      item_cap = hc.n_complex + 1024;
      continue;
    }
    n_items = (int64_t)hc.n_complex;
    if (n_items == 0) break;
    int64_t *dl = (int64_t *)c->deep_list.p;
    const DeepSel fast{dl, deep_cap, nullptr, 0, nullptr, 0, 0};
    auto run_deep = [&](int64_t from, AmbItem *aout, unsigned long long acap, const AmbItem *ain, const uint8_t *aref,
                        int64_t n_ain) -> gq_status {
      HIP_TRY(hipMemcpyAsync(&hc, ctr, kCountersHead, hipMemcpyDeviceToHost, c->stream));
      HIP_TRY(hipStreamSynchronize(c->stream));
      const int64_t nd = (int64_t)std::min<unsigned long long>(hc.n_deep, deep_cap) - from;
      if (nd <= 0 || hc.err) return GQ_OK;
      const int scap = (int)std::max<unsigned long long>(hc.deep_max, 64);
      const int64_t waves = std::min<int64_t>(nd, 256);
      HIP_TRY(c->deep_scratch.ensure((size_t)waves * gs_wave_bytes(scap, 16) + 256));
      const DeepSel deep{nullptr, deep_cap, dl + from, nd, (uint8_t *)c->deep_scratch.p, scap, 16};
      hipLaunchKernelGGL(allele_evidence_call<true>, dim3((unsigned)((waves + kSomWaves - 1) / kSomWaves)), dim3(kBlock),
                         0, c->stream, (const Tile *)c->tiles.p, (const ComplexItem *)c->cplx.p, n_items, rd->d, *p,
                         (AeRec *)c->srecs.p, rec_cap, (uint8_t *)c->pool.p, pool_cap, ctr, sw, aout, acap, ain, aref,
                         n_ain, deep);
      HIP_TRY(hipGetLastError());
      HIP_TRY(hipMemcpyAsync(&hc, ctr, kCountersHead, hipMemcpyDeviceToHost, c->stream));
      HIP_TRY(hipStreamSynchronize(c->stream));
      return GQ_OK;
    };
    const int cblocks = (int)std::min<int64_t>((n_items + kSomWaves - 1) / kSomWaves, 8192);
    hipLaunchKernelGGL(allele_evidence_call<false>, dim3((unsigned)cblocks), dim3(kBlock), 0, c->stream,
                       (const Tile *)c->tiles.p, (const ComplexItem *)c->cplx.p, n_items, rd->d, *p, (AeRec *)c->srecs.p,
                       rec_cap, (uint8_t *)c->pool.p, pool_cap, ctr, sw, (AmbItem *)c->amb.p, amb_cap,
                       (const AmbItem *)nullptr, (const uint8_t *)nullptr, (int64_t)0, fast);
    HIP_TRY(hipGetLastError());
    st = run_deep(0, (AmbItem *)c->amb.p, amb_cap, nullptr, nullptr, 0);
    if (st) return fail(st);
    HIP_TRY(hipEventRecord(c->ev[3], c->stream));
    bool retry = false;
    if (hc.n_amb > amb_cap) {
      amb_cap = hc.n_amb + 1024;
      retry = true;
    }
    if (hc.n_deep > deep_cap) {
      deep_cap = hc.n_deep + 1024;
      retry = true;
    }
    if (!retry && hc.n_amb > 0 && !hc.err) {
      std::vector<AmbItem> amb((size_t)hc.n_amb);
      HIP_TRY(hipMemcpyAsync(amb.data(), c->amb.p, amb.size() * sizeof(AmbItem), hipMemcpyDeviceToHost, c->stream));
      HIP_TRY(hipStreamSynchronize(c->stream));
      HIP_TRY(c->amb_ref.ensure(amb.size()));
      st = heap_ref_bases(c, pl, c->tiles, {rd}, amb, (uint8_t *)c->amb_ref.p);
      if (st) return fail(st);
      const int ablocks = (int)std::min<int64_t>(((int64_t)amb.size() + kSomWaves - 1) / kSomWaves, 8192);
      const int64_t from = (int64_t)hc.n_deep;
      hipLaunchKernelGGL(allele_evidence_call<false>, dim3((unsigned)ablocks), dim3(kBlock), 0, c->stream,
                         (const Tile *)c->tiles.p, (const ComplexItem *)c->cplx.p, n_items, rd->d, *p,
                         (AeRec *)c->srecs.p, rec_cap, (uint8_t *)c->pool.p, pool_cap, ctr, sw, (AmbItem *)nullptr,
                         (unsigned long long)0, (const AmbItem *)c->amb.p, (const uint8_t *)c->amb_ref.p,
                         (int64_t)amb.size(), fast);
      HIP_TRY(hipGetLastError());
      st = run_deep(from, (AmbItem *)nullptr, (unsigned long long)0, (const AmbItem *)c->amb.p,
                    (const uint8_t *)c->amb_ref.p, (int64_t)amb.size());
      if (st) return fail(st);
      HIP_TRY(hipEventRecord(c->ev[3], c->stream));
      if (hc.n_deep > deep_cap) {
        deep_cap = hc.n_deep + 1024;
        retry = true;
      }
    }
    if (hc.n_rec > rec_cap) {
      rec_cap = hc.n_rec + 1024;
      retry = true;
    }
    if (hc.pool_used > pool_cap) {
      pool_cap = hc.pool_used + 4096;
      retry = true;
    }
    if (!retry || hc.err) break;
    if (attempt == 2) return fail(set_err(GQ_E_CAPACITY, "allele-evidence: output capacity retries exhausted"));
  }
  for (int k = 0; k < kSpread; ++k) hc.visited += hc.spread[0][k];
  st = check_device_error(c, hc);
  if (st) return fail(st);
  const int64_t nr = n_items > 0 ? (int64_t)hc.n_rec : 0;
  std::vector<AeRec> recs((size_t)nr);
  std::vector<uint8_t> hpool((size_t)std::min<unsigned long long>(hc.pool_used, pool_cap));
  if (nr) HIP_TRY(hipMemcpyAsync(recs.data(), c->srecs.p, (size_t)nr * sizeof(AeRec), hipMemcpyDeviceToHost, c->stream));
  if (!hpool.empty()) HIP_TRY(hipMemcpyAsync(hpool.data(), c->pool.p, hpool.size(), hipMemcpyDeviceToHost, c->stream));
  HIP_TRY(hipEventRecord(c->ev[4], c->stream));
  HIP_TRY(hipStreamSynchronize(c->stream));
  const auto m0 = std::chrono::steady_clock::now();
  std::vector<uint32_t> ord((size_t)nr);
  for (int64_t k = 0; k < nr; ++k) ord[(size_t)k] = (uint32_t)k;
  std::sort(ord.begin(), ord.end(), [&](uint32_t x, uint32_t y) { return recs[x].key < recs[y].key; });
  const size_t N = (size_t)std::max<int64_t>(nr, 1);
  size_t pool_len = 0;
  for (const AeRec &r : recs) pool_len += (size_t)r.ref_len + r.alt_len;
  res->contig = (int32_t *)malloc(N * 4);
  res->pos = (int64_t *)malloc(N * 8);
  res->sample = (int32_t *)malloc(N * 4);
  res->ref_off = (int64_t *)malloc(N * 8);
  res->alt_off = (int64_t *)malloc(N * 8);
  res->ref_len = (int32_t *)malloc(N * 4);
  res->alt_len = (int32_t *)malloc(N * 4);
  res->evidence = (gq_evidence *)malloc(N * sizeof(gq_evidence));
// ... 93 lines not shown
```

Measured before the change: 36.20 billion loci/s.

## Fold part_scan and img_scan into consumers; defer read validation sync on reuse

The partition prefix scan now runs inside block 0 of germline_expand, and each expand block reads its partition count directly from the clamped counter instead of a separate part_scan launch. The img_scan kernel is removed: each calls_image block recomputes its own prefix and the total from the block sums. The finalize scratch moves into the counters buffer so one memset clears it and the separate zero launch is skipped on the first pass. When derive_shape runs again on a read set it has already seen, it reuses the cached qoff/shape and copies the validation flag asynchronously into pinned memory, checking it later instead of doing a blocking stream sync. This trades fewer launches and host syncs for redundant per-block prefix work, a serialized scan in block 0, and errors that are reported later.

```diff
diff --git a/guacamole_amd/csrc/gq_germline_common.h b/guacamole_amd/csrc/gq_germline_common.h
--- a/guacamole_amd/csrc/gq_germline_common.h
+++ b/guacamole_amd/csrc/gq_germline_common.h
@@ -131,17 +131,57 @@
   }
 }
 
-__global__ void germline_expand(CallRec *__restrict__ recs, Counters *ctr, OutGeom og, int threshold,
-                                int emit_ref, int emit_no_call, uint64_t dead_key) {
-  const unsigned long long n = ctr->n_rec;
+template <int NT>
+__device__ __forceinline__ void part_scan_block(Counters *ctr, int which, const OutGeom &og) {
+  static_assert(kParts % NT == 0, "partitions per thread");
+  constexpr int PER = kParts / NT;
+  __shared__ unsigned long long s[NT];
+  __shared__ unsigned long long mx;
+  const int t = threadIdx.x;
+  unsigned long long v[PER], sum = 0, m = 0;
+#pragma unroll
+  for (int j = 0; j < PER; ++j) {
+    const unsigned long long x = ctr->part[which][t * PER + j];
+    const unsigned long long cap = og.cap(which, t * PER + j);
+    m = x > cap && x - cap > m ? x - cap : m;
+    v[j] = x < cap ? x : cap;
+    sum += v[j];
+  }
+  if (t == 0) mx = 0;
+  s[t] = sum;
+  __syncthreads();
+  if (m) atomicMax(&mx, m);
+  for (int d = 1; d < NT; d <<= 1) {
+    const unsigned long long y = t >= d ? s[t - d] : 0ull;
+    __syncthreads();
+    s[t] += y;
+    __syncthreads();
+  }
+  unsigned long long o = s[t] - sum;
+#pragma unroll
+  for (int j = 0; j < PER; ++j) {
+    ctr->part_off[which][t * PER + j] = o;
+    o += v[j];
+  }
+  if (t == NT - 1) {
+    ctr->part_off[which][kParts] = s[t];
+    if (which == 0) ctr->n_rec = s[t];
+    else ctr->n_complex = s[t];
+    ctr->part_max[which] = mx;
+  }
+}
+
+__global__ __launch_bounds__(kBlock) void germline_expand(CallRec *__restrict__ recs, Counters *ctr, OutGeom og,
+                                                          int threshold, int emit_ref, int emit_no_call,
+                                                          uint64_t dead_key) {
+  if (blockIdx.x == 0) part_scan_block<kBlock>(ctr, 0, og);
   const int64_t thr1 = (int64_t)threshold + 1;
   auto passes = [=](uint32_t count, uint32_t depth) { return (int64_t)count * 100 >= thr1 * (int64_t)depth; };
   constexpr uint64_t kAltSym = ((uint64_t)'<' << 8) | ((uint64_t)'A' << 16) | ((uint64_t)'L' << 24) |
                                ((uint64_t)'T' << 32) | ((uint64_t)'>' << 40);
   unsigned dead = 0, ties = 0;
-  (void)n;
   for (int p = blockIdx.x; p < kParts; p += gridDim.x) {
-   const unsigned long long cnt = ctr->part_off[0][p + 1] - ctr->part_off[0][p];
+   const unsigned long long cnt = min(ctr->part[0][p], og.cap(0, p));
    for (unsigned long long k = threadIdx.x; k < cnt; k += blockDim.x) {
     const unsigned long long slot = og.slot(0, p, k);
     const CallRec cand = recs[slot];
diff --git a/guacamole_amd/csrc/gq_host.h b/guacamole_amd/csrc/gq_host.h
--- a/guacamole_amd/csrc/gq_host.h
+++ b/guacamole_amd/csrc/gq_host.h
@@ -864,7 +864,6 @@
   gq::DevBuf deep_list, deep_scratch;
   gq::DevBuf cands;
   gq::DevBuf win_bound;
-  gq::DevBuf bkt;
   void *stage[2] = {nullptr, nullptr};
   hipEvent_t stage_done[2] = {};
   bool stage_used[2] = {false, false};
@@ -954,6 +953,12 @@
   hipEvent_t tev[6] = {};
   unsigned pending = 0;
   unsigned long long *nok = nullptr;
+  bool shape_kept = false;
+  int64_t *qoff_dev = nullptr;
+  int64_t n_slices_kept = 0;
+  int pool_ordered_kept = 0;
+  int *vflag = nullptr;
+  bool vflag_pending = false;
   mutable void *mproj = nullptr;
   mutable int mproj_mapq = -1;
   mutable void *mnb = nullptr;
@@ -1030,6 +1035,8 @@
 };
 
 gq_status derive_shape(gq_ctx *c, gq_dev_reads *d, int64_t md_len);
+gq_status validation_settled(const gq_dev_reads *d);
+gq_status validation_wait(const gq_dev_reads *d);
 gq_status ensure_columns(gq_ctx *c, const gq_dev_reads *d);
 gq_status ensure_ev_bases(gq_ctx *c, const gq_dev_reads *d);
 gq_status ensure_projection(gq_ctx *c, const gq_dev_reads *d);
diff --git a/guacamole_amd/csrc/gq_pileup.hip b/guacamole_amd/csrc/gq_pileup.hip
--- a/guacamole_amd/csrc/gq_pileup.hip
+++ b/guacamole_amd/csrc/gq_pileup.hip
@@ -1485,41 +1485,7 @@
 }
 
 __global__ __launch_bounds__(1024) void part_scan(Counters *ctr, int which, OutGeom og) {
-  constexpr int PER = kParts / 1024;
-  __shared__ unsigned long long s[1024];
-  __shared__ unsigned long long mx;
-  const int t = threadIdx.x;
-  unsigned long long v[PER], sum = 0, m = 0;
-#pragma unroll
-  for (int j = 0; j < PER; ++j) {
-    const unsigned long long x = ctr->part[which][t * PER + j];
-    const unsigned long long cap = og.cap(which, t * PER + j);
-    m = x > cap && x - cap > m ? x - cap : m;
-    v[j] = x < cap ? x : cap;
-    sum += v[j];
-  }
-  if (t == 0) mx = 0;
-  s[t] = sum;
-  __syncthreads();
-  if (m) atomicMax(&mx, m);
-  for (int d = 1; d < 1024; d <<= 1) {
-    const unsigned long long y = t >= d ? s[t - d] : 0ull;
-    __syncthreads();
-    s[t] += y;
-    __syncthreads();
-  }
-  unsigned long long o = s[t] - sum;
-#pragma unroll
-  for (int j = 0; j < PER; ++j) {
-    ctr->part_off[which][t * PER + j] = o;
-    o += v[j];
-  }
-  if (t == 1023) {
-    ctr->part_off[which][kParts] = s[t];
-    if (which == 0) ctr->n_rec = s[t];
-    else ctr->n_complex = s[t];
-    ctr->part_max[which] = mx;
-  }
+  part_scan_block<1024>(ctr, which, og);
 }
 
 __global__ void gather_keys(const CallRec *__restrict__ recs, const Counters *__restrict__ ctr, OutGeom og,
@@ -1572,6 +1538,13 @@
   }
 }
 
+__device__ __forceinline__ void img_chunk(int64_t n, int64_t &a, int64_t &b) {
+  const int64_t per = (n + kImgBlocks - 1) / kImgBlocks;
+  a = min(n, (int64_t)blockIdx.x * per);
+  b = min(n, a + per);
+}
+__device__ __forceinline__ uint32_t rec_len(const CallRec &r) { return (uint32_t)r.ref_len + (uint32_t)r.alt_len; }
+
 __global__ void bucket_rank(int64_t nbk, const uint32_t *__restrict__ off, const int32_t *__restrict__ members,
                             const uint64_t *__restrict__ keys, const int32_t *__restrict__ slot,
                             const int64_t *__restrict__ bkt, int32_t *__restrict__ order) {
@@ -1596,16 +1569,9 @@
   if (i < n) v[i] = (int32_t)i;
 }
 
-__device__ __forceinline__ void img_chunk(int64_t n, int64_t &a, int64_t &b) {
-  const int64_t per = (n + kImgBlocks - 1) / kImgBlocks;
-  a = min(n, (int64_t)blockIdx.x * per);
-  b = min(n, a + per);
-}
-__device__ __forceinline__ uint32_t rec_len(const CallRec &r) { return (uint32_t)r.ref_len + (uint32_t)r.alt_len; }
-
 __global__ __launch_bounds__(kBlock) void img_sums(const CallRec *__restrict__ recs, const int32_t *__restrict__ order,
                                                     const uint32_t *__restrict__ off, int64_t nbk,
-                                                    int64_t *__restrict__ bsum) {
+                                                    unsigned long long *__restrict__ bsum) {
   __shared__ unsigned long long red;
   if (threadIdx.x == 0) red = 0;
   __syncthreads();
@@ -1616,36 +1582,38 @@
   for (int d = 32; d >= 1; d >>= 1) s += __shfl_xor(s, d, 64);
   if ((threadIdx.x & 63) == 0 && s) atomicAdd(&red, s);
   __syncthreads();
-  if (threadIdx.x == 0) bsum[blockIdx.x] = (int64_t)red;
-}
-
-__global__ __launch_bounds__(kImgBlocks) void img_scan(int64_t *__restrict__ bsum) {
-  __shared__ int64_t s[kImgBlocks];
-  const int t = threadIdx.x;
-  const int64_t v = bsum[t];
-  s[t] = v;
-  __syncthreads();
-  for (int d = 1; d < kImgBlocks; d <<= 1) {
-    const int64_t y = t >= d ? s[t - d] : 0;
-    __syncthreads();
-    s[t] += y;
-    __syncthreads();
-  }
-  bsum[t] = s[t] - v;
-  if (t == kImgBlocks - 1) bsum[kImgBlocks] = s[t];
+  if (threadIdx.x == 0) bsum[blockIdx.x] = red;
 }
 
 __global__ __launch_bounds__(kBlock) void calls_image(const CallRec *__restrict__ recs, const int32_t *__restrict__ order,
                                                        const uint32_t *__restrict__ off, int64_t nbk,
-                                                       const int64_t *__restrict__ bsum, const uint8_t *__restrict__ dpool,
+                                                       const unsigned long long *__restrict__ bsum, const uint8_t *__restrict__ dpool,
                                                        Counters *__restrict__ ctr, uint8_t *__restrict__ img) {
   __shared__ uint32_t wsum[kBlock / 64];
+  __shared__ unsigned long long before_all[2];
   const int64_t n = (int64_t)off[nbk];
   const CallsLayout L = calls_layout(n, 0);
   int64_t a, b;
   img_chunk(n, a, b);
-  int64_t prefix = bsum[blockIdx.x];
   const int lane = threadIdx.x & 63, wv = threadIdx.x >> 6;
+  if (threadIdx.x < 2) before_all[threadIdx.x] = 0;
+  __syncthreads();
+  {
+    unsigned long long sb = 0, sa = 0;
+    for (int q = threadIdx.x; q < kImgBlocks; q += blockDim.x) {
+      const unsigned long long v = bsum[q];
+      sa += v;
+      sb += q < (int)blockIdx.x ? v : 0ull;
+    }
+    for (int d = 32; d >= 1; d >>= 1) {
+      sa += __shfl_xor(sa, d, 64);
+      sb += __shfl_xor(sb, d, 64);
+    }
+    if (lane == 0 && sb) atomicAdd(&before_all[0], sb);
+    if (lane == 0 && sa) atomicAdd(&before_all[1], sa);
+  }
+  __syncthreads();
+  int64_t prefix = (int64_t)before_all[0];
   for (int64_t base = a; base < b; base += blockDim.x) {
     const int64_t k = base + threadIdx.x;
     CallRec r{};
@@ -1683,7 +1651,7 @@
     prefix += all;
   }
   if (blockIdx.x == 0 && threadIdx.x == 0) {
-    const int64_t pool_len = bsum[kImgBlocks];
+    const int64_t pool_len = (int64_t)before_all[1];
     reinterpret_cast<int64_t *>(img)[0] = pool_len;
     reinterpret_cast<int64_t *>(img)[1] = n;
     ctr->n_out = (unsigned long long)n;
@@ -1699,6 +1667,34 @@
 hipError_t gq::warm_pileup(hipStream_t s) {
   hipLaunchKernelGGL(warm_k, dim3(1), dim3(64), 0, s);
   return hipGetLastError();
+}
+
+static gq_status validation_status(int bad) {
+  if (bad & 1)
+    return set_err(GQ_E_UNSORTED, "Regions must be sorted by start locus: reads are not sorted by (contig, start), "
+                                  "or pmax_end is not the running maximum of end within each contig");
+  if (bad & 2)
+    return set_err(GQ_E_ARG, "read set: an offset or length lies outside its pool, or a sample slot >= n_samples");
+  return GQ_OK;
+}
+
+gq_status gq::validation_settled(const gq_dev_reads *dc) {
+  gq_dev_reads *d = const_cast<gq_dev_reads *>(dc);
+  if (!d->vflag_pending) return GQ_OK;
+  const int bad = *(volatile int *)d->vflag;
+  const gq_status vs = validation_status(bad);
+  if (vs) return vs;
+  if (((bad & 4) ? 0 : 1) != d->pool_ordered_kept)
+    return set_err(GQ_E_ARG, "read set: the sequence pool's order changed since the first derivation");
+  d->vflag_pending = false;
+  return GQ_OK;
+}
+
+gq_status gq::validation_wait(const gq_dev_reads *d) {
+  if (!d || !d->vflag_pending) return GQ_OK;
+  HIP_TRY(hipSetDevice(d->ctx->device));
+  HIP_TRY(hipEventSynchronize(d->tev[1]));
+  return validation_settled(d);
 }
 
 extern "C" {
@@ -1754,7 +1750,7 @@
   for (DevBuf *b : {&c->ranges, &c->tiles, &c->recs, &c->recs_sorted, &c->keys, &c->keys_sorted, &c->idx,
                     &c->idx_sorted, &c->cplx, &c->pool, &c->counters, &c->sort_tmp, &c->image, &c->tiles2, &c->srecs, &c->c_depth, &c->c_pos,
                     &c->c_base, &c->c_indel, &c->c_ref, &c->c_rb, &c->c_amb, &c->slow, &c->amb, &c->amb_ref,
-                    &c->heap_off, &c->heap_reads, &c->win_meta, &c->win_grp, &c->bkt})
+                    &c->heap_off, &c->heap_reads, &c->win_meta, &c->win_grp})
     b->release();
   for (auto &e : c->ev) (void)hipEventDestroy(e);
   for (auto &e : c->dev_ev) (void)hipEventDestroy(e);
@@ -1793,6 +1789,8 @@
   if (d->pending & 1) {
     HIP_TRY(hipEventSynchronize(d->tev[1]));
     (void)hipEventElapsedTime(&d->derive_dev_ms, d->tev[0], d->tev[1]);
+    const gq_status vs = gq::validation_settled(d);
+    if (vs) return vs;
   }
   if (d->pending & 2) {
     HIP_TRY(hipEventSynchronize(d->tev[5]));
@@ -1826,6 +1824,7 @@
   d->ev_bases = false;
   int unordered = 0;
   const int nc = d->d.n_contigs;
+  const bool reuse = lazy && d->shape_kept;
   std::vector<int32_t> last((size_t)nc, 0);
   if (d->d.n_reads > 0) {
     void *flag = nullptr;
@@ -1834,33 +1833,49 @@
     const unsigned nb = (unsigned)((d->d.n_reads + kBlock - 1) / kBlock);
     hipLaunchKernelGGL(read_prep, dim3(nb), dim3(kBlock), 0, c->stream, d->d, (int *)flag, (int16_t *)p);
     HIP_TRY(hipGetLastError());
-    int bad = 0;
-    HIP_TRY(hipMemcpyAsync(&bad, flag, sizeof(int), hipMemcpyDeviceToHost, c->stream));
-    const auto &crb = d->contig_read_begin;
-    for (int k = 0; k < nc; ++k)
-      if (crb[(size_t)k + 1] > crb[(size_t)k])
-        HIP_TRY(hipMemcpyAsync(&last[(size_t)k], d->d.pmax_end + (crb[(size_t)k + 1] - 1), sizeof(int32_t),
-                               hipMemcpyDeviceToHost, c->stream));
-    HIP_TRY(hipStreamSynchronize(c->stream));
-    if (bad & 1)
-      return set_err(GQ_E_UNSORTED, "Regions must be sorted by start locus: reads are not sorted by (contig, start), "
-                                    "or pmax_end is not the running maximum of end within each contig");
-    if (bad & 2)
-      return set_err(GQ_E_ARG, "read set: an offset or length lies outside its pool, or a sample slot >= n_samples");
-    unordered = (bad & 4) ? 1 : 0;
+    if (reuse) {
+      if (!d->vflag) HIP_TRY(hipHostMalloc((void **)&d->vflag, sizeof(int), hipHostMallocDefault));
+      *d->vflag = 0;
+      HIP_TRY(hipMemcpyAsync(d->vflag, flag, sizeof(int), hipMemcpyDeviceToHost, c->stream));
+      d->vflag_pending = true;
+      unordered = d->pool_ordered_kept ? 0 : 1;
+    } else {
+      int bad = 0;
+      HIP_TRY(hipMemcpyAsync(&bad, flag, sizeof(int), hipMemcpyDeviceToHost, c->stream));
+      const auto &crb = d->contig_read_begin;
+      for (int k = 0; k < nc; ++k)
+        if (crb[(size_t)k + 1] > crb[(size_t)k])
+          HIP_TRY(hipMemcpyAsync(&last[(size_t)k], d->d.pmax_end + (crb[(size_t)k + 1] - 1), sizeof(int32_t),
+                                 hipMemcpyDeviceToHost, c->stream));
+      HIP_TRY(hipStreamSynchronize(c->stream));
+      const gq_status vs = validation_status(bad);
+      if (vs) return vs;
+      unordered = (bad & 4) ? 1 : 0;
+    }
   }
   {
-    std::vector<int64_t> qoff((size_t)nc + 1, 0);
-    for (int k = 0; k < nc; ++k) {
-      const int64_t col1 = ((int64_t)std::max(last[(size_t)k], 0) + 7) >> 3;
-      qoff[(size_t)k + 1] = qoff[(size_t)k] + 4 * ((col1 + 63) >> 6);
-    }
-    void *qo = nullptr;
-    HIP_TRY(d->dp.get(&qo, sizeof(int64_t) * ((size_t)nc + 1)));
-    HIP_TRY(hipMemcpyAsync(qo, qoff.data(), sizeof(int64_t) * ((size_t)nc + 1), hipMemcpyHostToDevice, c->stream));
-    d->d.qoff = (const int64_t *)qo;
-    d->n_slices = qoff[(size_t)nc];
-    const int64_t n_blk = qoff[(size_t)nc] / 4;
+    if (!reuse) {
+      std::vector<int64_t> qoff((size_t)nc + 1, 0);
+      for (int k = 0; k < nc; ++k) {
+        const int64_t col1 = ((int64_t)std::max(last[(size_t)k], 0) + 7) >> 3;
+        qoff[(size_t)k + 1] = qoff[(size_t)k] + 4 * ((col1 + 63) >> 6);
+      }
+      if (!d->qoff_dev) {
+        void *qo = nullptr;
+        HIP_TRY(hipMalloc(&qo, sizeof(int64_t) * ((size_t)nc + 1)));
+        d->owned.push_back(qo);
+        d->qoff_dev = (int64_t *)qo;
+      }
+      HIP_TRY(hipMemcpyAsync(d->qoff_dev, qoff.data(), sizeof(int64_t) * ((size_t)nc + 1), hipMemcpyHostToDevice,
+                             c->stream));
+      if (lazy) HIP_TRY(hipStreamSynchronize(c->stream));
+      d->n_slices_kept = qoff[(size_t)nc];
+      d->pool_ordered_kept = unordered ? 0 : 1;
+      d->shape_kept = true;
+    }
+    d->d.qoff = d->qoff_dev;
+    d->n_slices = d->n_slices_kept;
+    const int64_t n_blk = d->n_slices_kept / 4;
     void *bi = nullptr;
     HIP_TRY(d->dp.get(&bi, sizeof(int64_t) * 2 * (size_t)std::max<int64_t>(n_blk, 1)));
     int64_t *brb = (int64_t *)bi, *brs = brb + std::max<int64_t>(n_blk, 1);
@@ -2154,6 +2169,7 @@
       (void)hipEventDestroy(e);
     }
   for (void *p : d->owned) (void)hipFree(p);
+  if (d->vflag) (void)hipHostFree(d->vflag);
   d->dp.free_all();
   delete d;
 }
@@ -2330,6 +2346,11 @@
   gq_calls *res = (gq_calls *)calloc(1, sizeof(gq_calls));
   if (!res) return set_err(GQ_E_NOMEM, "calloc");
   if (pl.n_tiles == 0) {
+    st = validation_wait(rd);
+    if (st) {
+      free(res);
+      return st;
+    }
     *out = res;
     return GQ_OK;
   }
@@ -2351,10 +2372,14 @@
   size_t scan_tmp = 0;
   HIP_TRY(hipcub::DeviceScan::ExclusiveSum(nullptr, scan_tmp, (const uint32_t *)nullptr, (uint32_t *)nullptr,
                                            (int)(nbk + 1), c->stream));
-  auto finalize = [&](Counters *ctr, size_t cap_rec) -> gq_status {
-    uint32_t *cnt = (uint32_t *)c->bkt.p, *off = cnt + (nbk + 1), *fill = off + (nbk + 1);
-    hipLaunchKernelGGL(zero_u32, dim3((unsigned)std::min<int64_t>((3 * (nbk + 1) + kBlock - 1) / kBlock, 1024)),
-                       dim3(kBlock), 0, c->stream, cnt, 3 * (nbk + 1));
+  const size_t fin_off = (sizeof(Counters) + 15) & ~(size_t)15;
+  const size_t fin_words = 2 * (size_t)kImgBlocks + 3 * (size_t)(nbk + 1);
+  auto finalize = [&](Counters *ctr, size_t cap_rec, bool cleared) -> gq_status {
+    unsigned long long *bsum = (unsigned long long *)((char *)ctr + fin_off);
+    uint32_t *cnt = (uint32_t *)(bsum + kImgBlocks), *off = cnt + (nbk + 1), *fill = off + (nbk + 1);
+    if (!cleared)
+      hipLaunchKernelGGL(zero_u32, dim3((unsigned)std::min<int64_t>(((int64_t)fin_words + kBlock - 1) / kBlock, 1024)),
+                         dim3(kBlock), 0, c->stream, (uint32_t *)bsum, (int64_t)fin_words);
     const unsigned gb = (unsigned)std::max<int64_t>(1, std::min<int64_t>(((int64_t)cap_rec + kBlock - 1) / kBlock, kFinBlocks));
     hipLaunchKernelGGL(bucket_count, dim3(gb), dim3(kBlock), 0, c->stream, (const CallRec *)c->recs.p,
                        ctr, og, dead_key, bshift, nbk, (uint64_t *)c->keys.p, (int32_t *)c->idx_sorted.p,
@@ -2368,12 +2393,10 @@
                        (const int32_t *)c->keys_sorted.p, (const uint64_t *)c->keys.p, (const int32_t *)c->idx_sorted.p,
                        (const int64_t *)c->idx.p, (int32_t *)c->recs_sorted.p);
     HIP_TRY(hipGetLastError());
-    int64_t *bsum = (int64_t *)c->keys_sorted.p + (cap_rec + 1) / 2 + 1;
     hipLaunchKernelGGL(img_sums, dim3(kImgBlocks), dim3(kBlock), 0, c->stream, (const CallRec *)c->recs.p,
                        (const int32_t *)c->recs_sorted.p, (const uint32_t *)off, nbk, bsum);
-    hipLaunchKernelGGL(img_scan, dim3(1), dim3(kImgBlocks), 0, c->stream, bsum);
     hipLaunchKernelGGL(calls_image, dim3(kImgBlocks), dim3(kBlock), 0, c->stream, (const CallRec *)c->recs.p,
-                       (const int32_t *)c->recs_sorted.p, (const uint32_t *)off, nbk, (const int64_t *)bsum,
+                       (const int32_t *)c->recs_sorted.p, (const uint32_t *)off, nbk, (const unsigned long long *)bsum,
                        (const uint8_t *)c->pool.p, ctr, (uint8_t *)c->image.p);
     HIP_TRY(hipGetLastError());
     return GQ_OK;
@@ -2391,17 +2414,16 @@
     HIP_TRY(c->recs.ensure(cap_rec * sizeof(CallRec)));
     HIP_TRY(c->cplx.ensure(og.total(1) * sizeof(ComplexItem)));
     HIP_TRY(c->pool.ensure(pool_cap));
-    HIP_TRY(c->counters.ensure(sizeof(Counters)));
+    HIP_TRY(c->counters.ensure(fin_off + 4 * fin_words));
     HIP_TRY(c->keys.ensure((cap_rec + 1) * 8));
-    HIP_TRY(c->keys_sorted.ensure((cap_rec + 1) * 4 + 8 * (kImgBlocks + 2) + 16));
+    HIP_TRY(c->keys_sorted.ensure((cap_rec + 1) * 4));
     HIP_TRY(c->idx.ensure((cap_rec + 1) * 8));
     HIP_TRY(c->idx_sorted.ensure((cap_rec + 1) * 4));
     HIP_TRY(c->recs_sorted.ensure((cap_rec + 1) * 4));
-    HIP_TRY(c->bkt.ensure(sizeof(uint32_t) * (size_t)(3 * (nbk + 1))));
     HIP_TRY(c->sort_tmp.ensure(std::max<size_t>(scan_tmp, 16)));
     HIP_TRY(c->image.ensure(calls_layout((int64_t)cap_rec, (int64_t)pool_cap).bytes));
     Counters *ctr = (Counters *)c->counters.p;
-    HIP_TRY(hipMemsetAsync(ctr, 0, sizeof(Counters), c->stream));
+    HIP_TRY(hipMemsetAsync(ctr, 0, fin_off + 4 * fin_words, c->stream));
     if (attempt == 0) HIP_TRY(hipEventRecord(c->ev[1], c->stream));
     st = launch_germline(c, pl.n_tiles, rd->d, p, (CallRec *)c->recs.p, (ComplexItem *)c->cplx.p, og, ctr, direct);
     if (st) {
@@ -2444,7 +2466,6 @@
       free(res);
       return st;
     }
-    hipLaunchKernelGGL(part_scan, dim3(1), dim3(1024), 0, c->stream, ctr, 0, og);
     {
 #ifndef GQ_EXPAND_BLOCKS
 #define GQ_EXPAND_BLOCKS 1024
@@ -2454,13 +2475,14 @@
       HIP_TRY(hipGetLastError());
     }
     HIP_TRY(hipEventRecord(c->ev[3], c->stream));
-    st = finalize(ctr, cap_rec);
+    st = finalize(ctr, cap_rec, true);
     if (st) {
       free(res);
       return st;
     }
     HIP_TRY(hipEventRecord(c->ev[4], c->stream));
     st = read_counters(ctr);
+    if (!st) st = validation_settled(rd);
     if (st) {
       free(res);
       return st;
@@ -2543,7 +2565,7 @@
         retry = true;
       }
       if (!retry) {
-        st = finalize(ctr, cap_rec);
+        st = finalize(ctr, cap_rec, false);
         if (!st) {
           HIP_TRY(hipEventRecord(c->ev[4], c->stream));
           st = read_counters(ctr);
@@ -2716,6 +2738,10 @@
 gq_status gq_pileup_counts(gq_ctx *c, const gq_dev_reads *rd, const gq_loci *loci, gq_counts **out) {
   if (!c || !rd || !loci || !out) return set_err(GQ_E_ARG, "gq_pileup_counts: null argument");
   HIP_TRY(hipSetDevice(c->device));
+  {
+    const gq_status vs = gq::validation_wait(rd);
+    if (vs) return vs;
+  }
   Plan pl;
   gq_status st = ensure_columns(c, rd);
   if (st) return st;
@@ -2812,6 +2838,10 @@
   if (!c || !rd || !loci || !p || !out) return set_err(GQ_E_ARG, "gq_vaf_histogram: null argument");
   if (p->bins < 1 || p->bins > 100) return set_err(GQ_E_ASSERT, "assumption failed: Bins should be between 1 and 100");
   HIP_TRY(hipSetDevice(c->device));
+  {
+    const gq_status vs = gq::validation_wait(rd);
+    if (vs) return vs;
+  }
   memset(out, 0, sizeof(*out));
   Plan pl;
   gq_status st = ensure_columns(c, rd);
diff --git a/guacamole_amd/csrc/gq_somatic.hip b/guacamole_amd/csrc/gq_somatic.hip
--- a/guacamole_amd/csrc/gq_somatic.hip
+++ b/guacamole_amd/csrc/gq_somatic.hip
@@ -1349,6 +1349,10 @@
     return set_err(GQ_E_ARG, "tumor and normal read sets must share the contig list (%d vs %d contigs)",
                    t->d.n_contigs, n->d.n_contigs);
   const int dbg = getenv("GQ_DBG") ? atoi(getenv("GQ_DBG")) : 0;
+  for (const gq_dev_reads *s : {t, n}) {
+    const gq_status vs = gq::validation_wait(s);
+    if (vs) return vs;
+  }
   RefView rv{nullptr, nullptr};
   std::vector<int32_t> lc;
   std::vector<int64_t> ls, le, lt;
@@ -1708,6 +1712,10 @@
 gq_status gq_variant_support(gq_ctx *c, const gq_dev_reads *rd, const gq_loci *loci, gq_allele_counts **out) {
   if (!c || !rd || !loci || !out) return set_err(GQ_E_ARG, "gq_variant_support: null argument");
   HIP_TRY(hipSetDevice(c->device));
+  {
+    const gq_status vs = gq::validation_wait(rd);
+    if (vs) return vs;
+  }
   const auto h0 = std::chrono::steady_clock::now();
   c->timings = gq_timings{};
   HIP_TRY(hipEventRecord(c->ev[0], c->stream));
@@ -1886,6 +1894,10 @@
                                gq_somatic_calls **out) {
   if (!c || !rd || !loci || !p || !out) return set_err(GQ_E_ARG, "gq_germline_standard: null argument");
   HIP_TRY(hipSetDevice(c->device));
+  {
+    const gq_status vs = gq::validation_wait(rd);
+    if (vs) return vs;
+  }
   const auto h0 = std::chrono::steady_clock::now();
   c->timings = gq_timings{};
   HIP_TRY(hipEventRecord(c->ev[0], c->stream));
@@ -2075,6 +2087,10 @@
                              const gq_allele_evidence_params *p, gq_allele_evidence_rows **out) {
   if (!c || !rd || !loci || !p || !out) return set_err(GQ_E_ARG, "gq_allele_evidence: null argument");
   HIP_TRY(hipSetDevice(c->device));
+  {
+    const gq_status vs = gq::validation_wait(rd);
+    if (vs) return vs;
+  }
   const auto h0 = std::chrono::steady_clock::now();
   c->timings = gq_timings{};
   HIP_TRY(hipEventRecord(c->ev[0], c->stream));
```

Measured after the change: 37.20 billion loci/s, median of 6. 2.8% higher.
